# mit-han-lab/pvcnn

Hardware: AMD Instinct MI355X
Metric: point-clouds/sec fwd+bwd, PVCNN S3DIS N=4096 R=32 (higher is better)
Workload: dtype f32 (fp32 tensors, fp32 accumulate; Conv3d fwd / bwd-data / bwd-weight and the large SharedMLP fwd / bwd-data / bwd-weight products as power-of-two scaled fp16 hi+lo splits, 3 partial products on fp16 MFMA, max rel err vs fp64 1e-6 <= the fp32-MFMA kernels'; PVCNN_CONV_MATH=fp32 PVCNN_PW_MATH=fp32 s

## Files before the change

include/pvcnn_hip.h:

```cpp
#ifndef PVCNN_HIP_H_
#define PVCNN_HIP_H_

#include <stddef.h>
#include <stdint.h>

#ifdef __cplusplus
extern "C" {
#endif

#if defined(__GNUC__)
#define PVCNN_API __attribute__((visibility("default")))
#else
#define PVCNN_API
#endif

#define PVCNN_ABI_VERSION 12
#define PVCNN_OK 0
#define PVCNN_ERR_INVALID_ARGUMENT (-1)

PVCNN_API int pvcnn_version(void);
PVCNN_API const char *pvcnn_last_error_string(void);

PVCNN_API int pvcnn_voxel_coords(const float *coords, int B, int N, int R, int normalize, float eps, float *norm_coords,
                       int32_t *vox_coords, void *stream);

PVCNN_API int pvcnn_voxel_coords_tail(const float *coords, long coords_batch_stride, const float *mean, const float *radius,
                            int B, int N, int R, float eps, float *norm_coords, int32_t *vox_coords, void *stream);

PVCNN_API size_t pvcnn_avg_voxelize_fwd_workspace_bytes(int B, int C, int N, int R);
PVCNN_API int pvcnn_avg_voxelize_fwd(const float *feat, const int32_t *coords, int B, int C, int N, int R,
                           float *out, int32_t *ind, int32_t *cnt, void *workspace,
                           size_t workspace_bytes, void *stream);
PVCNN_API int pvcnn_avg_voxelize_bwd(const float *grad_y, const int32_t *ind, const int32_t *cnt, int B,
                           int C, int N, int S, float *grad_x, void *stream);

PVCNN_API int pvcnn_trilinear_devox_fwd(const float *coords, const float *feat, int B, int C, int N, int R,
                              int is_training, int32_t *inds, float *wgts, float *outs,
                              void *stream);
PVCNN_API size_t pvcnn_trilinear_devox_bwd_workspace_bytes(int B, int C, int N, int R);
PVCNN_API int pvcnn_trilinear_devox_bwd(const float *grad_y, const int32_t *inds, const float *wgts, int B,
                              int C, int N, int R, float *grad_x, void *workspace,
                              size_t workspace_bytes, void *stream);

PVCNN_API size_t pvcnn_avg_voxelize_plan_bytes(int B, int N, int R);
PVCNN_API size_t pvcnn_avg_voxelize_plan_scratch_bytes(int B, int N, int R);
PVCNN_API int pvcnn_avg_voxelize_plan(const int32_t *coords, int B, int N, int R, int32_t *ind, int32_t *cnt, void *plan,
                            size_t plan_bytes, void *scratch, size_t scratch_bytes, void *stream);
PVCNN_API size_t pvcnn_pvconv_plans_scratch_bytes(int B, int N, int R);
PVCNN_API int pvcnn_pvconv_plans(const int32_t *vox_coords, const float *norm_coords, int B, int N, int R, int32_t *ind, int32_t *cnt,
                                 void *vox_plan, size_t vox_plan_bytes, void *devox_bwd_plan, size_t devox_bwd_plan_bytes,
                                 void *scratch, size_t scratch_bytes, void *stream);
PVCNN_API int pvcnn_avg_voxelize_apply(const float *feat, const void *plan, size_t plan_bytes, int B, int C, int N, int R,
                             float *out, void *stream);
PVCNN_API size_t pvcnn_trilinear_devox_bwd_plan_bytes(int B, int N, int R);
PVCNN_API size_t pvcnn_trilinear_devox_bwd_plan_scratch_bytes(int B, int N, int R);
PVCNN_API int pvcnn_trilinear_devox_bwd_plan(const int32_t *inds, const float *wgts, int B, int N, int R, void *plan,
                                   size_t plan_bytes, void *scratch, size_t scratch_bytes, void *stream);
PVCNN_API int pvcnn_trilinear_devox_bwd_apply(const float *grad_y, long grad_y_batch_stride, const void *plan, size_t plan_bytes,
                                    int B, int C, int N, int R, float *grad_x, void *stream);

PVCNN_API int pvcnn_ball_query(const float *centers, const float *points, int B, int N, int M, float radius,
                     int U, int32_t *out, void *stream);

PVCNN_API int pvcnn_grouping_fwd(const float *features, const int32_t *indices, int B, int C, int N, int M,
                       int U, float *out, void *stream);
PVCNN_API size_t pvcnn_grouping_bwd_workspace_bytes(int B, int C, int N, int M, int U);
PVCNN_API int pvcnn_grouping_bwd(const float *grad_y, const int32_t *indices, int B, int C, int N, int M,
                       int U, float *grad_x, void *workspace, size_t workspace_bytes, void *stream);
PVCNN_API int pvcnn_gather_fwd(const float *features, const int32_t *indices, int B, int C, int N, int M,
                     float *out, void *stream);
PVCNN_API size_t pvcnn_gather_bwd_workspace_bytes(int B, int C, int N, int M);
PVCNN_API int pvcnn_gather_bwd(const float *grad_y, const int32_t *indices, int B, int C, int N, int M,
                     float *grad_x, void *workspace, size_t workspace_bytes, void *stream);

#define PVCNN_FPS_MAX_RESIDENT_POINTS 16384
PVCNN_API int pvcnn_fps(const float *coords, int B, int N, int M, float *distances, int32_t *indices,
              void *stream);

PVCNN_API int pvcnn_mask_select(const uint8_t *mask, int B, int N, int M, const int32_t *choices, const int64_t *seed,
                      int32_t *selected, int32_t *count, void *stream);

PVCNN_API int pvcnn_three_nn_interp_fwd(const float *points_coords, const float *centers_coords,
                              const float *centers_features, int B, int C, int M, int N,
                              int32_t *indices, float *weights, float *out, void *stream);
PVCNN_API size_t pvcnn_three_nn_interp_bwd_workspace_bytes(int B, int C, int N, int M);
PVCNN_API int pvcnn_three_nn_interp_bwd(const float *grad_y, const int32_t *indices, const float *weights,
                              int B, int C, int N, int M, float *grad_x, void *workspace,
                              size_t workspace_bytes, void *stream);

PVCNN_API int pvcnn_conv3d_weight_transform(const float *w, int Co, int Ci, int for_bwd_data, float *wt,
                                            void *stream);
PVCNN_API int pvcnn_conv3d_fwd(const float *x, const float *wt, const float *bias, int B, int Ci, int Co,
                               int R, float *y, void *stream);
PVCNN_API size_t pvcnn_conv3d_bwd_weight_workspace_bytes(int B, int Ci, int Co, int R);
PVCNN_API int pvcnn_conv3d_bwd_weight(const float *x, const float *grad_y, int B, int Ci, int Co, int R,
                                      float *grad_w, float *grad_bias, void *workspace, size_t workspace_bytes,
                                      void *stream);

PVCNN_API size_t pvcnn_conv3d_weight_split_bytes(int Co, int Ci, int for_bwd_data, int nsplit);
PVCNN_API int pvcnn_conv3d_weight_split(const float *w, int Co, int Ci, int for_bwd_data, int nsplit, void *wts, void *stream);
PVCNN_API int pvcnn_conv3d_weight_split_pair(const float *w, int Co, int Ci, void *wts_fwd, void *wts_bwd, void *stream);
PVCNN_API size_t pvcnn_conv3d_fwd_split_stats_parts(int B, int Co, int R, int nsplit);
PVCNN_API int pvcnn_conv3d_fwd_split_route(int B, int Ci, int Co, int R, int nsplit);
PVCNN_API int pvcnn_absmax_bits(const float *x, size_t n, void *out, void *stream);
PVCNN_API size_t pvcnn_absmax_tiles_count(int B, long L, int seg);
#define PVCNN_TABLE_ONLY ((void *)1)
PVCNN_API int pvcnn_absmax_tiles(const float *x, int B, int C, long L, int seg, void *out, void *ticket, void *stream);
PVCNN_API int pvcnn_conv3d_fwd_split(const float *x, const void *wts, const float *bias, int B, int Ci, int Co, int R, int nsplit,
                           const void *x_absmax, int amax_seg , float *y, float *stats_part, void *stream);

PVCNN_API size_t pvcnn_conv3d_bwd_weight_f16_workspace_bytes(int B, int Ci, int Co, int R);
PVCNN_API int pvcnn_conv3d_bwd_weight_f16(const float *x, const float *grad_y, const void *x_absmax, int x_amax_seg, const void *gy_absmax,
                                int gy_amax_seg, int B, int Ci, int Co, int R, float *grad_w, float *grad_bias, void *workspace,
                                size_t workspace_bytes, void *stream);

PVCNN_API int pvcnn_pwconv_transpose(const float *w, int M, int K, float *wt, void *stream);
PVCNN_API int pvcnn_pwconv_fwd(const float *x, const float *wt, int wt_rows, const float *bias, int B, int K, int M,
                     int N, float *y, void *stream);
PVCNN_API size_t pvcnn_pwconv_bwd_weight_workspace_bytes(int B, int K, int M, int N);
PVCNN_API int pvcnn_pwconv_bwd_weight(const float *x, const float *grad_y, int B, int K, int M, int N,
                            float *grad_w, float *grad_bias, void *workspace, size_t workspace_bytes,
                            void *stream);

PVCNN_API size_t pvcnn_pwconv_weight_split_bytes(int Co, int Ci, int for_bwd_data, int nsplit);
PVCNN_API int pvcnn_pwconv_weight_split(const float *w, int Co, int Ci, int for_bwd_data, int nsplit, void *wts, void *stream);
PVCNN_API int pvcnn_pwconv_weight_split_pair(const float *w, int Co, int Ci, void *wts_fwd, void *wts_bwd, void *stream);
PVCNN_API size_t pvcnn_pwconv_fwd_split_stats_parts(int B, int N);
PVCNN_API int pvcnn_pwconv_fwd_split(const float *x, const void *wts, const float *bias, int B, int K, int M, int N, int nsplit,
                           const void *x_absmax, int amax_seg , float *y, float *stats_part, void *stream);
PVCNN_API size_t pvcnn_pwconv_bwd_weight_f16_workspace_bytes(int B, int K, int M, int N);
PVCNN_API int pvcnn_pwconv_bwd_weight_f16(const float *x, const float *grad_y, const void *x_absmax, int x_amax_seg, const void *gy_absmax,
                                int gy_amax_seg, int B, int K, int M, int N, float *grad_w, float *grad_bias, void *workspace,
                                size_t workspace_bytes, void *stream);

PVCNN_API int pvcnn_dropout_keep_mask(const void *drop_seed, float drop_p, long numel, unsigned char *keep, void *stream);
PVCNN_API size_t pvcnn_bnact_workspace_bytes(int B, int C, int S);
PVCNN_API int pvcnn_bnact_fwd(const float *x, const float *gamma, const float *beta, float *running_mean,
                              float *running_var, int B, int C, int S, float eps, float momentum, float slope,
                              int training, float *mean, float *rstd, float *y, void *y_amax, int amax_seg, int amax_zeroed,
                              void *workspace, size_t workspace_bytes, const void *drop_seed, float drop_p, void *stream);
PVCNN_API size_t pvcnn_conv3d_fwd_stats_parts(int B, int Co, int R);
PVCNN_API int pvcnn_conv3d_fwd_stats(const float *x, const float *wt, const float *bias, int B, int Ci, int Co, int R,
                           float *y, float *stats_part, void *stream);
PVCNN_API size_t pvcnn_pwconv_fwd_stats_parts(int B, int N);
PVCNN_API int pvcnn_pwconv_fwd_stats(const float *x, const float *wt, int wt_rows, const float *bias, int B, int K, int M,
                           int N, float *y, float *stats_part, void *stream);
PVCNN_API int pvcnn_bn_finalize(const float *part, int C, long nparts, double count, float eps, float momentum, const float *shift,
                      float *running_mean, float *running_var, float *mean, float *rstd,
                      void *zero_words , long zero_count ,
                      void *num_batches_tracked , void *stream);
PVCNN_API int pvcnn_bn_stats(const float *x, float *running_mean, float *running_var, int B, int C, int S,
                   float eps, float momentum, float *mean, float *rstd, void *workspace,
                   size_t workspace_bytes, void *stream);
PVCNN_API int pvcnn_trilinear_devox_bnact_fwd(const float *coords, const float *feat, const float *gamma,
                                    const float *beta, const float *mean, const float *rstd, float slope,
                                    int B, int C, int N, int R, int is_training, int32_t *inds, float *wgts,
                                    const float *addend, const float *se_scale, float *outs, void *stream);
PVCNN_API int pvcnn_bnact_bwd(const float *x, const float *grad_y, const float *gamma, const float *beta,
                              const float *mean, const float *rstd, int B, int C, int S, float slope, int training,
                              float *grad_x, float *grad_gamma, float *grad_beta, void *workspace,
                              size_t workspace_bytes, void *stream);
PVCNN_API int pvcnn_bnact_bwd_strided(const float *x, const float *grad_y, long grad_y_batch_stride, const float *gamma,
                            const float *beta, const float *mean, const float *rstd, int B, int C, int S,
                            float slope, int training, float *grad_x, float *grad_gamma, float *grad_beta,
                            void *gx_amax, int amax_seg, void *workspace, size_t workspace_bytes, const void *drop_seed,
                            float drop_p, void *tickets, void *stream);
PVCNN_API int pvcnn_bnact_slices(int S);
PVCNN_API long pvcnn_conv3d_weight_split_pair_entry(const float *w, int Co, int Ci, void *wts_fwd, void *wts_bwd, long long *entry);
PVCNN_API int pvcnn_conv3d_weight_split_pair_batch(const void *table, int n, long total_rows, void *stream);
PVCNN_API long pvcnn_pwconv_weight_split_pair_entry(const float *w, int Co, int Ci, void *wts_fwd, void *wts_bwd, long long *entry);
PVCNN_API int pvcnn_pwconv_weight_split_pair_batch(const void *table, int n, long total_rows, void *stream);
PVCNN_API long pvcnn_conv3d_weight_split_pair_entry_bf16(const float *w, int Co, int Ci, void *wts_fwd, void *wts_bwd, long long *entry);
PVCNN_API int pvcnn_conv3d_weight_split_pair_batch_bf16(const void *table, int n, long total_rows, void *stream);
PVCNN_API long pvcnn_pwconv_weight_split_pair_entry_bf16(const float *w, int Co, int Ci, void *wts_fwd, void *wts_bwd, long long *entry);
PVCNN_API int pvcnn_pwconv_weight_split_pair_batch_bf16(const void *table, int n, long total_rows, void *stream);

PVCNN_API int pvcnn_neighbor_max_supported(int K);
PVCNN_API int pvcnn_neighbor_max_fwd(const float *x, long rows, int K, float *out, unsigned char *winners, void *stream);
PVCNN_API int pvcnn_neighbor_max_bwd(const float *grad_out, const unsigned char *winners, long rows, int K, float *grad_x, void *stream);

PVCNN_API int pvcnn_row_argmax(const float *x, long rows, int K, long long *winners, float *values, void *stream);

PVCNN_API int pvcnn_bnact_apply_rowmax(const float *x, const float *gamma, const float *beta, const float *mean, const float *rstd, int B,
                                       int C, int S, float slope, float *y, long y_batch_stride, void *y_amax, int amax_seg,
                                       void *row_keys, void *stream);
PVCNN_API int pvcnn_row_keys_decode(const void *row_keys, const float *y, long rows, int S, long long *winners, float *values,
                                    int C, long y_batch_stride, void *stream);

PVCNN_API size_t pvcnn_frustum_box_loss_grad_floats(int B, int NH, int NS);
PVCNN_API int pvcnn_frustum_box_loss(const float *center, const float *center_reg, const float *heading_scores, const float *size_scores,
                                     const float *heading_residuals_normalized, const float *size_residuals_normalized,
                                     const float *heading_residuals, const float *size_residuals, const long long *heading_bin_id,
                                     const long long *size_template_id, const float *heading_residual_t, const float *size_residual_t,
                                     const float *center_t, const float *size_templates, const float *heading_bin_centers, int B, int NH,
                                     int NS, float heading_bin_width, float w_heading_residual, float w_size_residual, float w_corners,
                                     float *loss, float *grads, void *stream);

PVCNN_API int pvcnn_se_excite_fwd(const float *part, int slices, const float *gamma, const float *beta, const float *w1, const float *w2,
                        int B, int C, int H, float inv_s, float *a_sum, float *ax_sum, float *squeezed, float *hidden, float *excite,
                        void *stream);
PVCNN_API int pvcnn_se_excite_bwd(const float *part, int slices, const float *a_sum, const float *ax_sum, const float *gamma,
                        const float *beta, const float *squeezed, const float *hidden, const float *excite, const float *w1,
                        const float *w2, int B, int C, int H, float inv_s, float *g_w1, float *g_w2, float *g_mean, float *sum_beta,
                        float *sum_gamma, float *workspace, void *stream);
PVCNN_API int pvcnn_bnact_partial_sums(const float *x, const float *grad_y, long grad_y_batch_stride, const float *gamma, const float *beta,
                             const float *mean, const float *rstd, int B, int C, int S, float slope, float *part, void *stream);
PVCNN_API int pvcnn_bnact_bwd_apply(const float *x, const float *grad_y, long grad_y_batch_stride, const float *gamma, const float *beta,
                          const float *mean, const float *rstd, const float *sum_gamma, const float *sum_beta, const float *bc_mul,
                          const float *bc_add, int B, int C, int S, float slope, int training, float *grad_x, void *gx_amax,
                          int amax_seg, void *stream);
PVCNN_API int pvcnn_trilinear_devox_bwd_strided(const float *grad_y, long grad_y_batch_stride, const int32_t *inds,
                                      const float *wgts, int B, int C, int N, int R, float *grad_x,
                                      void *workspace, size_t workspace_bytes, void *stream);

PVCNN_API int pvcnn_concat_points(const float *const *srcs, const long *bstrides, const int *channels, const int *pstrides,
                        const void *const *src_amax ,
                        int nsrc, int B, int N, float *out, void *out_amax,
                        void *ticket , void *stream);

PVCNN_API int pvcnn_dense_bn_relu_supported(int rows, int Cin, int Cout);
PVCNN_API int pvcnn_dense_bn_relu_fwd(const float *x, const float *weight, const float *bias, const float *gamma, const float *beta,
                                      float *running_mean, float *running_var, void *num_batches_tracked, int rows, int Cin, int Cout,
                                      float eps, float momentum, float *z, float *y, float *mean, float *rstd, void *stream);
PVCNN_API int pvcnn_dense_bn_relu_bwd(const float *x, const float *grad_y, const float *z, const float *mean, const float *rstd,
                                      const float *gamma, const float *beta, int rows, int Cin, int Cout, float *grad_z,
                                      float *grad_weight, float *grad_bias, float *grad_gamma, float *grad_beta, void *stream);

PVCNN_API int pvcnn_adam_step(float *p, const float *g, float *m, float *v, size_t n, float *step, const float *hyper, int inc_step,
                    void *stream);

#ifdef __cplusplus
}
#endif
#endif
```

pvcnn_amd/_lib.py:

```python
import ctypes
import functools
import os

import torch

_CSRC = os.path.join(os.path.dirname(os.path.abspath(__file__)), 'csrc')
LIB_PATH = os.path.join(_CSRC, 'libpvcnn_hip.so')
ABI_VERSION = 12

_vp, _i, _f, _sz, _l = ctypes.c_void_p, ctypes.c_int, ctypes.c_float, ctypes.c_size_t, ctypes.c_long

SIGNATURES = {
    'pvcnn_version': (_i, []),
    'pvcnn_last_error_string': (ctypes.c_char_p, []),
    'pvcnn_voxel_coords': (_i, [_vp, _i, _i, _i, _i, _f, _vp, _vp, _vp]),
    'pvcnn_voxel_coords_tail': (_i, [_vp, ctypes.c_long, _vp, _vp, _i, _i, _i, _f, _vp, _vp, _vp]),
    'pvcnn_avg_voxelize_fwd_workspace_bytes': (_sz, [_i, _i, _i, _i]),
    'pvcnn_avg_voxelize_fwd': (_i, [_vp, _vp, _i, _i, _i, _i, _vp, _vp, _vp, _vp, _sz, _vp]),
    'pvcnn_avg_voxelize_bwd': (_i, [_vp, _vp, _vp, _i, _i, _i, _i, _vp, _vp]),
    'pvcnn_trilinear_devox_fwd': (_i, [_vp, _vp, _i, _i, _i, _i, _i, _vp, _vp, _vp, _vp]),
    'pvcnn_trilinear_devox_bwd_workspace_bytes': (_sz, [_i, _i, _i, _i]),
    'pvcnn_trilinear_devox_bwd': (_i, [_vp, _vp, _vp, _i, _i, _i, _i, _vp, _vp, _sz, _vp]),
    'pvcnn_avg_voxelize_plan_bytes': (_sz, [_i, _i, _i]),
    'pvcnn_avg_voxelize_plan_scratch_bytes': (_sz, [_i, _i, _i]),
    'pvcnn_avg_voxelize_plan': (_i, [_vp, _i, _i, _i, _vp, _vp, _vp, _sz, _vp, _sz, _vp]),
    'pvcnn_avg_voxelize_apply': (_i, [_vp, _vp, _sz, _i, _i, _i, _i, _vp, _vp]),
    'pvcnn_pvconv_plans_scratch_bytes': (_sz, [_i, _i, _i]),
    'pvcnn_pvconv_plans': (_i, [_vp, _vp, _i, _i, _i, _vp, _vp, _vp, _sz, _vp, _sz, _vp, _sz, _vp]),
    'pvcnn_trilinear_devox_bwd_plan_bytes': (_sz, [_i, _i, _i]),
    'pvcnn_trilinear_devox_bwd_plan_scratch_bytes': (_sz, [_i, _i, _i]),
    'pvcnn_trilinear_devox_bwd_plan': (_i, [_vp, _vp, _i, _i, _i, _vp, _sz, _vp, _sz, _vp]),
    'pvcnn_trilinear_devox_bwd_apply': (_i, [_vp, ctypes.c_long, _vp, _sz, _i, _i, _i, _i, _vp, _vp]),
    'pvcnn_ball_query': (_i, [_vp, _vp, _i, _i, _i, _f, _i, _vp, _vp]),
    'pvcnn_grouping_fwd': (_i, [_vp, _vp, _i, _i, _i, _i, _i, _vp, _vp]),
    'pvcnn_grouping_bwd_workspace_bytes': (_sz, [_i, _i, _i, _i, _i]),
    'pvcnn_grouping_bwd': (_i, [_vp, _vp, _i, _i, _i, _i, _i, _vp, _vp, _sz, _vp]),
    'pvcnn_gather_fwd': (_i, [_vp, _vp, _i, _i, _i, _i, _vp, _vp]),
    'pvcnn_gather_bwd_workspace_bytes': (_sz, [_i, _i, _i, _i]),
    'pvcnn_gather_bwd': (_i, [_vp, _vp, _i, _i, _i, _i, _vp, _vp, _sz, _vp]),
    'pvcnn_fps': (_i, [_vp, _i, _i, _i, _vp, _vp, _vp]),
    'pvcnn_mask_select': (_i, [_vp, _i, _i, _i, _vp, _vp, _vp, _vp, _vp]),
    'pvcnn_three_nn_interp_fwd': (_i, [_vp, _vp, _vp, _i, _i, _i, _i, _vp, _vp, _vp, _vp]),
    'pvcnn_three_nn_interp_bwd_workspace_bytes': (_sz, [_i, _i, _i, _i]),
    'pvcnn_three_nn_interp_bwd': (_i, [_vp, _vp, _vp, _i, _i, _i, _i, _vp, _vp, _sz, _vp]),
    'pvcnn_conv3d_weight_transform': (_i, [_vp, _i, _i, _i, _vp, _vp]),
    'pvcnn_conv3d_fwd': (_i, [_vp, _vp, _vp, _i, _i, _i, _i, _vp, _vp]),
    'pvcnn_conv3d_bwd_weight_workspace_bytes': (_sz, [_i, _i, _i, _i]),
    'pvcnn_conv3d_bwd_weight': (_i, [_vp, _vp, _i, _i, _i, _i, _vp, _vp, _vp, _sz, _vp]),
    'pvcnn_conv3d_weight_split_bytes': (_sz, [_i, _i, _i, _i]),
    'pvcnn_conv3d_weight_split': (_i, [_vp, _i, _i, _i, _i, _vp, _vp]),
    'pvcnn_conv3d_weight_split_pair': (_i, [_vp, _i, _i, _vp, _vp, _vp]),
    'pvcnn_conv3d_fwd_split_stats_parts': (_sz, [_i, _i, _i, _i]),
    'pvcnn_conv3d_fwd_split_route': (_i, [_i, _i, _i, _i, _i]),
    'pvcnn_absmax_bits': (_i, [_vp, _sz, _vp, _vp]),
    'pvcnn_absmax_tiles_count': (_sz, [_i, ctypes.c_long, _i]),
    'pvcnn_absmax_tiles': (_i, [_vp, _i, _i, ctypes.c_long, _i, _vp, _vp, _vp]),
    'pvcnn_conv3d_bwd_weight_f16_workspace_bytes': (_sz, [_i, _i, _i, _i]),
    'pvcnn_conv3d_bwd_weight_f16': (_i, [_vp, _vp, _vp, _i, _vp, _i, _i, _i, _i, _i, _vp, _vp, _vp, _sz, _vp]),
    'pvcnn_conv3d_fwd_split': (_i, [_vp, _vp, _vp, _i, _i, _i, _i, _i, _vp, _i, _vp, _vp, _vp]),
    'pvcnn_pwconv_transpose': (_i, [_vp, _i, _i, _vp, _vp]),
    'pvcnn_pwconv_fwd': (_i, [_vp, _vp, _i, _vp, _i, _i, _i, _i, _vp, _vp]),
    'pvcnn_pwconv_weight_split_bytes': (_sz, [_i, _i, _i, _i]),
    'pvcnn_pwconv_weight_split': (_i, [_vp, _i, _i, _i, _i, _vp, _vp]),
    'pvcnn_pwconv_weight_split_pair': (_i, [_vp, _i, _i, _vp, _vp, _vp]),
    'pvcnn_pwconv_fwd_split_stats_parts': (_sz, [_i, _i]),
    'pvcnn_pwconv_fwd_split': (_i, [_vp, _vp, _vp, _i, _i, _i, _i, _i, _vp, _i, _vp, _vp, _vp]),
    'pvcnn_pwconv_bwd_weight_f16_workspace_bytes': (_sz, [_i, _i, _i, _i]),
    'pvcnn_pwconv_bwd_weight_f16': (_i, [_vp, _vp, _vp, _i, _vp, _i, _i, _i, _i, _i, _vp, _vp, _vp, _sz, _vp]),
    'pvcnn_pwconv_bwd_weight_workspace_bytes': (_sz, [_i, _i, _i, _i]),
    'pvcnn_pwconv_bwd_weight': (_i, [_vp, _vp, _i, _i, _i, _i, _vp, _vp, _vp, _sz, _vp]),
    'pvcnn_bnact_workspace_bytes': (_sz, [_i, _i, _i]),
    'pvcnn_bnact_fwd': (_i, [_vp, _vp, _vp, _vp, _vp, _i, _i, _i, _f, _f, _f, _i, _vp, _vp, _vp, _vp, _i, _i, _vp, _sz, _vp, _f, _vp]),
    'pvcnn_dropout_keep_mask': (_i, [_vp, _f, _l, _vp, _vp]),
    'pvcnn_conv3d_fwd_stats_parts': (_sz, [_i, _i, _i]),
    'pvcnn_conv3d_fwd_stats': (_i, [_vp, _vp, _vp, _i, _i, _i, _i, _vp, _vp, _vp]),
    'pvcnn_pwconv_fwd_stats_parts': (_sz, [_i, _i]),
    'pvcnn_pwconv_fwd_stats': (_i, [_vp, _vp, _i, _vp, _i, _i, _i, _i, _vp, _vp, _vp]),
    'pvcnn_bn_finalize': (_i, [_vp, _i, ctypes.c_long, ctypes.c_double, _f, _f, _vp, _vp, _vp, _vp, _vp, _vp, ctypes.c_long, _vp, _vp]),
    'pvcnn_bn_stats': (_i, [_vp, _vp, _vp, _i, _i, _i, _f, _f, _vp, _vp, _vp, _sz, _vp]),
    'pvcnn_trilinear_devox_bnact_fwd': (_i, [_vp, _vp, _vp, _vp, _vp, _vp, _f, _i, _i, _i, _i, _i, _vp, _vp, _vp, _vp, _vp, _vp]),
    'pvcnn_bnact_slices': (_i, [_i]),
    'pvcnn_conv3d_weight_split_pair_entry': (_l, [_vp, _i, _i, _vp, _vp, _vp]),
    'pvcnn_conv3d_weight_split_pair_batch': (_i, [_vp, _i, _l, _vp]),
    'pvcnn_pwconv_weight_split_pair_entry': (_l, [_vp, _i, _i, _vp, _vp, _vp]),
    'pvcnn_pwconv_weight_split_pair_batch': (_i, [_vp, _i, _l, _vp]),
    'pvcnn_conv3d_weight_split_pair_entry_bf16': (_l, [_vp, _i, _i, _vp, _vp, _vp]),
    'pvcnn_conv3d_weight_split_pair_batch_bf16': (_i, [_vp, _i, _l, _vp]),
    'pvcnn_pwconv_weight_split_pair_entry_bf16': (_l, [_vp, _i, _i, _vp, _vp, _vp]),
    'pvcnn_pwconv_weight_split_pair_batch_bf16': (_i, [_vp, _i, _l, _vp]),
    'pvcnn_neighbor_max_supported': (_i, [_i]),
    'pvcnn_neighbor_max_fwd': (_i, [_vp, _l, _i, _vp, _vp, _vp]),
    'pvcnn_neighbor_max_bwd': (_i, [_vp, _vp, _l, _i, _vp, _vp]),
    'pvcnn_row_argmax': (_i, [_vp, _l, _i, _vp, _vp, _vp]),
    'pvcnn_bnact_apply_rowmax': (_i, [_vp, _vp, _vp, _vp, _vp, _i, _i, _i, _f, _vp, _l, _vp, _i, _vp, _vp]),
    'pvcnn_row_keys_decode': (_i, [_vp, _vp, _l, _i, _vp, _vp, _i, _l, _vp]),
    'pvcnn_frustum_box_loss_grad_floats': (_sz, [_i, _i, _i]),
    'pvcnn_frustum_box_loss': (_i, [_vp] * 15 + [_i, _i, _i, _f, _f, _f, _f, _vp, _vp, _vp]),
    'pvcnn_se_excite_fwd': (_i, [_vp, _i, _vp, _vp, _vp, _vp, _i, _i, _i, _f, _vp, _vp, _vp, _vp, _vp, _vp]),
    'pvcnn_se_excite_bwd': (_i, [_vp, _i] + [_vp] * 9 + [_i, _i, _i, _f] + [_vp] * 7),
    'pvcnn_bnact_partial_sums': (_i, [_vp, _vp, ctypes.c_long, _vp, _vp, _vp, _vp, _i, _i, _i, _f, _vp, _vp]),
    'pvcnn_bnact_bwd_apply': (_i, [_vp, _vp, ctypes.c_long, _vp, _vp, _vp, _vp, _vp, _vp, _vp, _vp, _i, _i, _i, _f, _i, _vp, _vp, _i, _vp]),
    'pvcnn_bnact_bwd': (_i, [_vp, _vp, _vp, _vp, _vp, _vp, _i, _i, _i, _f, _i, _vp, _vp, _vp, _vp, _sz, _vp]),
    'pvcnn_bnact_bwd_strided': (_i, [_vp, _vp, ctypes.c_long, _vp, _vp, _vp, _vp, _i, _i, _i, _f, _i, _vp, _vp, _vp, _vp, _i, _vp, _sz, _vp, _f, _vp, _vp]),
    'pvcnn_concat_points': (_i, [_vp, _vp, _vp, _vp, _vp, _i, _i, _i, _vp, _vp, _vp, _vp]),
    'pvcnn_dense_bn_relu_supported': (_i, [_i, _i, _i]),
    'pvcnn_dense_bn_relu_fwd': (_i, [_vp] * 8 + [_i, _i, _i, _f, _f, _vp, _vp, _vp, _vp, _vp]),
    'pvcnn_dense_bn_relu_bwd': (_i, [_vp] * 7 + [_i, _i, _i] + [_vp] * 6),
    'pvcnn_adam_step': (_i, [_vp, _vp, _vp, _vp, _sz, _vp, _vp, _i, _vp]),
    'pvcnn_trilinear_devox_bwd_strided': (_i, [_vp, ctypes.c_long, _vp, _vp, _i, _i, _i, _i, _vp, _vp, _sz, _vp]),
}

_lib = None


class PvcnnHipError(RuntimeError):
    pass


def load():
    global _lib
    if _lib is not None:
        return _lib
    if not os.path.exists(LIB_PATH):
        raise PvcnnHipError(
            f'{LIB_PATH} not found: build it with `python -c "import __graft_entry__ as g; g.build()"` '
            f'or `make -C {_CSRC}`.  There is no CPU fallback for the PVConv hot path.')
    lib = ctypes.CDLL(LIB_PATH)
    for name, (res, args) in SIGNATURES.items():
        fn = getattr(lib, name)
        fn.restype, fn.argtypes = res, args
    got = lib.pvcnn_version()
    if got != ABI_VERSION:
        raise PvcnnHipError(f'libpvcnn_hip.so ABI version {got}, binding expects {ABI_VERSION}: rebuild')
    for name, (res, _args) in SIGNATURES.items():
        if res is _sz:
            setattr(lib, name, functools.lru_cache(maxsize=4096)(getattr(lib, name)))
    _lib = lib
    return lib


def sources_digest():
    import glob
    import hashlib
    h = hashlib.sha1()
    names = sorted(glob.glob(os.path.join(_CSRC, '*.hip')) + glob.glob(os.path.join(_CSRC, '*.h')))
    names.append(os.path.join(os.path.dirname(os.path.dirname(os.path.abspath(__file__))), 'include', 'pvcnn_hip.h'))
    for name in names:
        h.update(os.path.basename(name).encode())
        with open(name, 'rb') as fh:
            h.update(fh.read())
    return h.hexdigest()[:12]


def check(rc, what):
    if rc != 0:
        msg = load().pvcnn_last_error_string().decode('utf-8', 'replace')
        raise PvcnnHipError(f'{what} failed (code {rc}): {msg}')
```

pvcnn_amd/csrc/bnact.hip:

```cpp
#include <algorithm>

#include "common.h"

namespace pvcnn {

constexpr int kBnThreads = 256;
constexpr int kBnSlice = 8192;

__device__ __forceinline__ float wave_sum(float v) {
#pragma unroll
  for (int d = 32; d >= 1; d >>= 1) v += __shfl_xor(v, d);
  return v;
}

__device__ __forceinline__ void block_sum2(float &a, float &b, float *sm) {
  a = wave_sum(a);
  b = wave_sum(b);
  const int wave = threadIdx.x >> 6, lane = threadIdx.x & 63;
  if (lane == 0) { sm[wave] = a; sm[8 + wave] = b; }
  __syncthreads();
  if (threadIdx.x == 0) {
    a = sm[0] + sm[1] + sm[2] + sm[3];
    b = sm[8] + sm[9] + sm[10] + sm[11];
  }
// ... 455 lines not shown
    amax_zeroed = 1;
  }
  if (y_amax != nullptr) {
    const int nseg = ceil_div(S, amax_seg), spb = amax_seg >= 256 ? 1 : 256 / amax_seg;
    const int vec = (S % 4 == 0) && (amax_seg % 4 == 0) && aligned16(x) && aligned16(y);
    uint32_t *am = static_cast<uint32_t *>(y_amax);
    const int groups = amax_zeroed ? pb_channel_groups((long)ceil_div(nseg, spb) * B, C) : 1;
    if (dropping)
      hipLaunchKernelGGL((bnact_apply_pb_kernel<false, true>), dim3(ceil_div(nseg, spb), B, groups), dim3(256), 0, s, x, nullptr, 0L, mean, rstd,
                         gamma, beta, nullptr, nullptr, slope, 0.0f, 0, C, S, amax_seg, nseg, vec, y, am, amax_zeroed ? 1 : 0, nullptr, nullptr,
                         ceil_div(C, groups), groups > 1 ? 1 : 0, drop);
    else
      hipLaunchKernelGGL(bnact_apply_pb_kernel<false>, dim3(ceil_div(nseg, spb), B, groups), dim3(256), 0, s, x, nullptr, 0L, mean, rstd, gamma,
                         beta, nullptr, nullptr, slope, 0.0f, 0, C, S, amax_seg, nseg, vec, y, am, amax_zeroed ? 1 : 0, nullptr, nullptr,
                         ceil_div(C, groups), groups > 1 ? 1 : 0);
    if (int e = check_launch("bnact_apply_pb")) return e;
    return amax_zeroed ? 0 : launch_amax_reduce(am, (long)B * nseg, s);
  }
  hipLaunchKernelGGL(bnact_apply_kernel, grid, dim3(kBnThreads), 0, s, x, mean, rstd, gamma, beta, slope, C, S, y);
  return check_launch("bnact_apply");
}

extern "C" int pvcnn_bnact_apply_rowmax(const float *x, const float *gamma, const float *beta, const float *mean, const float *rstd, int B,
                                        int C, int S, float slope, float *y, long y_batch_stride, void *y_amax, int amax_seg, void *row_keys,
                                        void *stream) {
  PVCNN_REQUIRE(B > 0 && C > 0 && S > 0 && x && y && mean && rstd && y_amax && row_keys, "bad argument");
  PVCNN_REQUIRE(y_batch_stride == 0 || (y_batch_stride >= (long)C * S && y_batch_stride % 4 == 0), "y_batch_stride: 0, or >= C * S and a multiple of 4");
  PVCNN_REQUIRE(B <= 65535 && C <= 65535, "batch or channel count > 65535");
  PVCNN_REQUIRE(amax_seg_in_range(amax_seg), kAmaxSegRange);
  PVCNN_REQUIRE(amax_seg % 4 == 0 && 256 % amax_seg == 0 && S % 256 == 0,
                "the row-maximum pass additionally needs S % 256 == 0 and amax_seg a multiple of 4 that divides 256");
  PVCNN_REQUIRE(aligned16(x) && aligned16(y) && ((uintptr_t)row_keys & 7) == 0, "x / y must be 16-byte aligned, row_keys 8-byte aligned");
  hipStream_t s = static_cast<hipStream_t>(stream);
  const int nseg = ceil_div(S, amax_seg), spb = amax_seg >= 256 ? 1 : 256 / amax_seg;
  const int groups = pb_channel_groups((long)ceil_div(nseg, spb) * B, C);
  hipLaunchKernelGGL((bnact_apply_pb_kernel<false, false, true>), dim3(ceil_div(nseg, spb), B, groups), dim3(256), 0, s, x, nullptr, 0L, mean, rstd,
                     gamma, beta, nullptr, nullptr, slope, 0.0f, 0, C, S, amax_seg, nseg, 1, y, static_cast<uint32_t *>(y_amax), 1, nullptr, nullptr,
                     ceil_div(C, groups), groups > 1 ? 1 : 0, Drop{nullptr, 0u, 1.0f}, static_cast<unsigned long long *>(row_keys), y_batch_stride);
  return check_launch("bnact_apply_rowmax");
}

extern "C" int pvcnn_row_keys_decode(const void *row_keys, const float *y, long rows, int S, long long *winners, float *values, int C,
                                     long y_batch_stride, void *stream) {
  PVCNN_REQUIRE(rows >= 0 && S > 0, "negative size");
  if (rows == 0) return 0;
  PVCNN_REQUIRE(row_keys && y && winners, "null pointer");
  if (C <= 0 || y_batch_stride <= 0) { C = 1; y_batch_stride = S; }
  hipLaunchKernelGGL(row_keys_decode_kernel, dim3((unsigned)((rows + 255) / 256)), dim3(256), 0, static_cast<hipStream_t>(stream),
                     static_cast<const unsigned long long *>(row_keys), y, rows, S, winners, values, C, y_batch_stride);
  return check_launch("row_keys_decode");
}

extern "C" int pvcnn_bn_finalize(const float *part, int C, long nparts, double count, float eps, float momentum, const float *shift,
                                 float *running_mean, float *running_var, float *mean, float *rstd, void *zero_words, long zero_count,
                                 void *num_batches_tracked, void *stream) {
  PVCNN_REQUIRE(C > 0 && nparts > 0 && nparts <= 0x7fffffffL && count > 0 && part && mean && rstd, "bad argument");
  hipLaunchKernelGGL(bn_finalize_kernel, dim3(C), dim3(64), 0, static_cast<hipStream_t>(stream),
                     reinterpret_cast<const float2 *>(part), (int)nparts, count, eps, momentum, shift, mean, rstd, running_mean,
                     running_var, static_cast<uint32_t *>(zero_words), zero_words ? zero_count : 0L,
                     static_cast<long long *>(num_batches_tracked));
  return check_launch("bn_finalize");
}

extern "C" int pvcnn_bn_stats(const float *x, float *running_mean, float *running_var, int B, int C, int S, float eps,
                              float momentum, float *mean, float *rstd, void *workspace, size_t workspace_bytes, void *stream) {
  PVCNN_REQUIRE(B > 0 && C > 0 && S > 0 && x && mean && rstd, "bad argument");
  PVCNN_REQUIRE(B <= 65535 && C <= 65535, "batch or channel count > 65535");
  PVCNN_REQUIRE(workspace && workspace_bytes >= pvcnn_bnact_workspace_bytes(B, C, S), "workspace too small");
  hipStream_t s = static_cast<hipStream_t>(stream);
  const int slices = ceil_div(S, kBnSlice);
  float2 *part = static_cast<float2 *>(workspace);
  float *shift = reinterpret_cast<float *>(part + (size_t)C * B * slices);
  hipLaunchKernelGGL(bn_stats_kernel, dim3(slices, B, C), dim3(kBnThreads), 0, s, x, C, S, slices, part, shift);
  if (int e = check_launch("bn_stats")) return e;
  hipLaunchKernelGGL(bn_finalize_kernel, dim3(C), dim3(64), 0, s, part, B * slices, (double)B * S, eps, momentum, shift, mean, rstd,
                     running_mean, running_var, static_cast<uint32_t *>(nullptr), 0L, static_cast<long long *>(nullptr));
  return check_launch("bn_finalize");
}

static int bnact_bwd_impl(const float *x, const float *grad_y, long gy_bstride, const float *gamma, const float *beta,
                          const float *mean, const float *rstd, int B, int C, int S, float slope, int training, float *grad_x,
                          float *grad_gamma, float *grad_beta, void *workspace, size_t workspace_bytes, void *stream,
                          void *gx_amax = nullptr, int amax_seg = 0, const void *drop_seed = nullptr, float drop_p = 0.0f,
                          void *tickets = nullptr) {
  PVCNN_REQUIRE(drop_p >= 0.0f && drop_p < 1.0f, "drop_p must be in [0, 1)");
  Drop drop{nullptr, 0u, 1.0f};
  const bool dropping = make_drop(drop_seed, drop_p, &drop);
  PVCNN_REQUIRE(!dropping || (gx_amax && (size_t)B * C * S < ((size_t)1 << 33)), "fused dropout needs the amax-emitting pass (gx_amax) and < 2^33 elements");
  PVCNN_REQUIRE(B > 0 && C > 0 && S > 0 && x && grad_y && mean && rstd && grad_x && grad_gamma && grad_beta, "bad argument");
  PVCNN_REQUIRE(B <= 65535 && C <= 65535, "batch or channel count > 65535");
  PVCNN_REQUIRE(gy_bstride >= (long)C * S, "grad_y batch stride smaller than one sample");
  PVCNN_REQUIRE(workspace && workspace_bytes >= pvcnn_bnact_workspace_bytes(B, C, S), "workspace too small");
  PVCNN_REQUIRE(!gx_amax || amax_seg_in_range(amax_seg), kAmaxSegRange);
  hipStream_t s = static_cast<hipStream_t>(stream);
  const int slices = ceil_div(S, kBnSlice);
  const dim3 grid(slices, B, C);
  float2 *part = static_cast<float2 *>(workspace);
  const long zero_count = gx_amax ? 1 + (long)B * ceil_div(S, amax_seg) : 0L;
  PVCNN_REQUIRE(!tickets || (reinterpret_cast<uintptr_t>(tickets) & 3) == 0, "tickets must be 4-byte aligned");
  const BwdFold fold{static_cast<unsigned *>(tickets), grad_gamma, grad_beta, static_cast<uint32_t *>(gx_amax), zero_count};
  if (dropping)
    hipLaunchKernelGGL(bnact_bwd_reduce_kernel<true>, grid, dim3(kBnThreads), 0, s, x, grad_y, mean, rstd, gamma, beta, slope, C, S, slices, part,
                       gy_bstride, drop, fold);
  else
    hipLaunchKernelGGL(bnact_bwd_reduce_kernel<false>, grid, dim3(kBnThreads), 0, s, x, grad_y, mean, rstd, gamma, beta, slope, C, S, slices, part,
                       gy_bstride, Drop{nullptr, 0u, 1.0f}, fold);
  if (int e = check_launch("bnact_bwd_reduce")) return e;
  if (tickets == nullptr) {
    hipLaunchKernelGGL(bnact_bwd_finalize_kernel, dim3(C), dim3(64), 0, s, part, B * slices, grad_gamma, grad_beta,
                       static_cast<uint32_t *>(gx_amax), zero_count);
    if (int e = check_launch("bnact_bwd_finalize")) return e;
  }
  const float inv_count = (float)(1.0 / ((double)B * S));
  if (gx_amax != nullptr) {
    const int nseg = ceil_div(S, amax_seg), spb = amax_seg >= 256 ? 1 : 256 / amax_seg;
    const int vec = (S % 4 == 0) && (amax_seg % 4 == 0) && (gy_bstride % 4 == 0) && aligned16(x) && aligned16(grad_y) && aligned16(grad_x);
    uint32_t *am = static_cast<uint32_t *>(gx_amax);
    const int groups = pb_channel_groups((long)ceil_div(nseg, spb) * B, C);
    if (dropping)
      hipLaunchKernelGGL((bnact_apply_pb_kernel<true, true>), dim3(ceil_div(nseg, spb), B, groups), dim3(256), 0, s, x, grad_y, gy_bstride, mean,
                         rstd, gamma, beta, grad_gamma, grad_beta, slope, inv_count, training, C, S, amax_seg, nseg, vec, grad_x, am, 1, nullptr,
                         nullptr, ceil_div(C, groups), groups > 1 ? 1 : 0, drop);
    else
      hipLaunchKernelGGL(bnact_apply_pb_kernel<true>, dim3(ceil_div(nseg, spb), B, groups), dim3(256), 0, s, x, grad_y, gy_bstride, mean, rstd,
                         gamma, beta, grad_gamma, grad_beta, slope, inv_count, training, C, S, amax_seg, nseg, vec, grad_x, am, 1, nullptr,
                         nullptr, ceil_div(C, groups), groups > 1 ? 1 : 0);
    return check_launch("bnact_bwd_apply_pb");
  }
  hipLaunchKernelGGL(bnact_bwd_apply_kernel, grid, dim3(kBnThreads), 0, s, x, grad_y, mean, rstd, gamma, beta, grad_gamma,
                     grad_beta, slope, inv_count, training, C, S, grad_x, gy_bstride);
  return check_launch("bnact_bwd_apply");
}

extern "C" int pvcnn_bnact_bwd(const float *x, const float *grad_y, const float *gamma, const float *beta, const float *mean,
                               const float *rstd, int B, int C, int S, float slope, int training, float *grad_x,
                               float *grad_gamma, float *grad_beta, void *workspace, size_t workspace_bytes, void *stream) {
  return bnact_bwd_impl(x, grad_y, (long)C * S, gamma, beta, mean, rstd, B, C, S, slope, training, grad_x, grad_gamma, grad_beta,
                        workspace, workspace_bytes, stream);
}

extern "C" int pvcnn_bnact_bwd_strided(const float *x, const float *grad_y, long grad_y_batch_stride, const float *gamma,
                                       const float *beta, const float *mean, const float *rstd, int B, int C, int S, float slope,
                                       int training, float *grad_x, float *grad_gamma, float *grad_beta, void *gx_amax, int amax_seg,
                                       void *workspace, size_t workspace_bytes, const void *drop_seed, float drop_p, void *tickets,
                                       void *stream) {
  return bnact_bwd_impl(x, grad_y, grad_y_batch_stride, gamma, beta, mean, rstd, B, C, S, slope, training, grad_x, grad_gamma,
                        grad_beta, workspace, workspace_bytes, stream, gx_amax, amax_seg, drop_seed, drop_p, tickets);
}

extern "C" int pvcnn_bnact_slices(int S) { return S > 0 ? ceil_div(S, kBnSlice) : 0; }

extern "C" int pvcnn_bnact_partial_sums(const float *x, const float *grad_y, long grad_y_batch_stride, const float *gamma, const float *beta,
                                        const float *mean, const float *rstd, int B, int C, int S, float slope, float *part, void *stream) {
  PVCNN_REQUIRE(B > 0 && C > 0 && S > 0 && x && mean && rstd && part, "bad argument");
  PVCNN_REQUIRE(B <= 65535 && C <= 65535, "batch or channel count > 65535");
  PVCNN_REQUIRE(!grad_y || grad_y_batch_stride >= (long)C * S, "grad_y batch stride smaller than one sample");
  PVCNN_REQUIRE((reinterpret_cast<uintptr_t>(part) & 7) == 0, "part must be 8-byte aligned");
  const int slices = ceil_div(S, kBnSlice);
  hipLaunchKernelGGL(bnact_bwd_reduce_kernel<false>, dim3(slices, B, C), dim3(kBnThreads), 0, static_cast<hipStream_t>(stream), x, grad_y, mean,
                     rstd, gamma, beta, slope, C, S, slices, reinterpret_cast<float2 *>(part), grad_y ? grad_y_batch_stride : (long)C * S);
  return check_launch("bnact_partial_sums");
}

extern "C" int pvcnn_bnact_bwd_apply(const float *x, const float *grad_y, long grad_y_batch_stride, const float *gamma, const float *beta,
                                     const float *mean, const float *rstd, const float *sum_gamma, const float *sum_beta, const float *bc_mul,
                                     const float *bc_add, int B, int C, int S, float slope, int training, float *grad_x, void *gx_amax,
                                     int amax_seg, void *stream) {
  PVCNN_REQUIRE(B > 0 && C > 0 && S > 0 && x && grad_y && mean && rstd && grad_x, "bad argument");
  PVCNN_REQUIRE(!training || (sum_gamma && sum_beta), "training mode needs the two per-channel sums");
  PVCNN_REQUIRE(B <= 65535 && C <= 65535, "batch or channel count > 65535");
  PVCNN_REQUIRE(grad_y_batch_stride >= (long)C * S, "grad_y batch stride smaller than one sample");
  PVCNN_REQUIRE(!gx_amax || amax_seg_in_range(amax_seg), kAmaxSegRange);
  hipStream_t s = static_cast<hipStream_t>(stream);
  PVCNN_REQUIRE(gx_amax, "pvcnn_bnact_bwd_apply needs an amax buffer (pvcnn_absmax_tiles_count words)");
  const int nseg = ceil_div(S, amax_seg), spb = amax_seg >= 256 ? 1 : 256 / amax_seg;
  const int vec = (S % 4 == 0) && (amax_seg % 4 == 0) && (grad_y_batch_stride % 4 == 0) && aligned16(x) && aligned16(grad_y) && aligned16(grad_x);
  uint32_t *am = static_cast<uint32_t *>(gx_amax);
  hipLaunchKernelGGL(bnact_apply_pb_kernel<true>, dim3(ceil_div(nseg, spb), B), dim3(256), 0, s, x, grad_y, grad_y_batch_stride, mean, rstd, gamma,
                     beta, sum_gamma, sum_beta, slope, (float)(1.0 / ((double)B * S)), training, C, S, amax_seg, nseg, vec, grad_x, am, 0, bc_mul,
                     bc_add);
  if (int e = check_launch("bnact_bwd_apply_pb")) return e;
  return launch_amax_reduce(am, (long)B * nseg, s);
}

namespace pvcnn {
constexpr int kCatMaxSrc = 8;
struct CatSources {
  const float *p[kCatMaxSrc];
  long bstride[kCatMaxSrc];
  int c0[kCatMaxSrc + 1];
  int pstride[kCatMaxSrc];
  const uint32_t *pre[kCatMaxSrc];
  int n;
};

__global__ __launch_bounds__(256) void concat_points_kernel(CatSources src, int N, int vec, float *__restrict__ out,
                                                            uint32_t *__restrict__ amax, unsigned *__restrict__ ticket) {
  __shared__ uint32_t wave_max[4];
  const int b = blockIdx.y, p0 = blockIdx.x * 256;
  const int tid = threadIdx.x, wave = __builtin_amdgcn_readfirstlane(tid >> 6), lane = tid & 63, pos = p0 + 4 * lane;
  const int Ctot = src.c0[src.n];
  const int cgroup = ceil_div(Ctot, (int)gridDim.z), gbeg = (int)blockIdx.z * cgroup, gend = min(Ctot, gbeg + cgroup);
  float *ob = out + (size_t)b * Ctot * N;
  uint32_t m = 0;
  using v4f = __attribute__((ext_vector_type(4))) float;
  for (int s = 0; s < src.n; ++s) {
    const int cb = src.c0[s], lo = max(gbeg, cb) - cb, cn = min(gend, src.c0[s + 1]) - cb;
    if (lo >= cn) continue;
    if (src.pre[s] != nullptr) {
      if (tid == 0 && amax != nullptr) m = max(m, src.pre[s][1 + (size_t)b * gridDim.x + blockIdx.x]);
      continue;
    }
    const float *sp = src.p[s] + (size_t)b * src.bstride[s];
    if (src.pstride[s] == 0) {
      for (int c = lo + wave; c < cn; c += 4) {
        const float v = sp[c];
        m = max(m, __float_as_uint(fabsf(v)));
        if (vec && pos < N) { v4f o = {v, v, v, v}; __builtin_nontemporal_store(o, reinterpret_cast<v4f *>(ob + (size_t)(cb + c) * N + pos)); }
        else for (int i = 0; i < 4; ++i) if (pos + i < N) ob[(size_t)(cb + c) * N + pos + i] = v;
      }
    } else if (vec) {
      if (pos < N)
        for (int c0 = lo + wave; c0 < cn; c0 += 32) {
          float4 v[8];
#pragma unroll
          for (int u = 0; u < 8; ++u)
            if (c0 + 4 * u < cn) v[u] = *reinterpret_cast<const float4 *>(sp + (size_t)(c0 + 4 * u) * N + pos);
#pragma unroll
          for (int u = 0; u < 8; ++u)
            if (c0 + 4 * u < cn) {
// ... 74 lines not shown
```

pvcnn_amd/csrc/csr.h:

```cpp
#pragma once
#include <algorithm>

#include "slab.h"

namespace pvcnn {

constexpr int kCsrThreads = 1024;
constexpr int kCsrMaxTargets = 1 << 20;
constexpr int kCsrMaxRange = 14336;

__host__ __device__ __forceinline__ int pad32(int v) { return v + (v >> 5); }
__host__ __device__ __forceinline__ int start_stride(int L) { return (L + 1 + 3) & ~3; }

constexpr int kTileTargets = 4096;
constexpr int kTileThreads = 1024;
__host__ __device__ inline int order_stride(int L) { return ceil_div(L, kTileTargets) * kTileTargets; }

constexpr int kGroupSlack = 256;
__host__ __device__ inline long entw_range_base(int start_t0, int r) { return 2L * start_t0 + (long)r * (kTileTargets / kWave) * kGroupSlack; }
__host__ __device__ inline long entw_stride(int L, long E) { return 2L * E + (long)ceil_div(L, kTileTargets) * (kTileTargets / kWave) * kGroupSlack; }

struct CsrPlan {
  int32_t *start;
  int2 *ent;
// ... 462 lines not shown
  int2 sg[kSlots];
#pragma unroll
  for (int k = 0; k < kSlots; ++k) {
    const int pos = k * kTileThreads + tid;
    sg[k] = l_seg[pos];
    out[pos] = l_lt[pos];
    sout[pos] = sg[k];
    int m = sg[k].y - sg[k].x, sum = m;
#pragma unroll
    for (int d = 32; d >= 1; d >>= 1) { m = max(m, __shfl_xor(m, d)); sum += __shfl_xor(sum, d); }
    if (lane == 0) gsz[pos >> 6] = (m > 0 && 64L * m <= 2L * sum + kGroupSlack) ? 64 * m : 0;
  }
  __syncthreads();
  if (tid < kGroups) {
    const int sz = gsz[tid];
    int inc = sz;
#pragma unroll
    for (int d = 1; d < kWave; d <<= 1) {
      const int up = __shfl_up(inc, d);
      if (lane >= d) inc += up;
    }
    const long base = entw_range_base(st[0], r) + (inc - sz);
    const int ofs = sz > 0 ? (int)base : -1;
    gsz[tid] = ofs;
    gofs[(size_t)b * (order_stride(L) / kWave) + (size_t)r * kGroups + tid] = ofs;
  }
}

static __global__ __launch_bounds__(kTileThreads) void csr_order_kernel(const int32_t *__restrict__ start, const int2 *__restrict__ ent,
                                                                        int L, int E, uint16_t *__restrict__ order,
                                                                        int2 *__restrict__ seg, int32_t *__restrict__ gofs,
                                                                        int2 *__restrict__ entw) {
  csr_order_body(start, ent, L, E, order, seg, gofs, entw, (int)blockIdx.x, (int)blockIdx.y);
}

struct CsrPlanRef {
  const int32_t *start;
  const int2 *ent;
  uint16_t *order;
  int2 *seg;
  int32_t *gofs;
  int2 *entw;
  int E;
};

[[maybe_unused]] static __global__ __launch_bounds__(kTileThreads) void csr_order_pair_kernel(CsrPlanRef a, CsrPlanRef c, int L, int nr) {
  const int r = (int)blockIdx.x;
  const bool f = r < nr;
  csr_order_body(f ? a.start : c.start, f ? a.ent : c.ent, L, f ? a.E : c.E, f ? a.order : c.order, f ? a.seg : c.seg,
                 f ? a.gofs : c.gofs, f ? a.entw : c.entw, f ? r : r - nr, (int)blockIdx.y);
}

static __device__ __forceinline__ void csr_interleave_body(const int2 *__restrict__ ent, const int2 *__restrict__ seg,
                                                           const int32_t *__restrict__ gofs, int L, int E, int2 *__restrict__ entw,
                                                           int blk, int b) {
  const int pos = blk * 256 + threadIdx.x, lane = threadIdx.x & 63;
  const int ofs = gofs[(size_t)b * (order_stride(L) / kWave) + (pos >> 6)];
  if (ofs < 0) return;
  const int2 sg = seg[(size_t)b * order_stride(L) + pos];
  const int2 *en = ent + (size_t)b * E + sg.x;
  int2 *ew = entw + (size_t)b * entw_stride(L, E) + ofs + lane;
  const int n = sg.y - sg.x;
  int i = 0;
  for (; i + 4 <= n; i += 4) {
    const int2 a = en[i], c = en[i + 1], d = en[i + 2], f = en[i + 3];
    ew[(size_t)i * 64] = a; ew[(size_t)(i + 1) * 64] = c; ew[(size_t)(i + 2) * 64] = d; ew[(size_t)(i + 3) * 64] = f;
  }
  for (; i < n; ++i) ew[(size_t)i * 64] = en[i];
}

static __global__ __launch_bounds__(256) void csr_interleave_kernel(const int2 *__restrict__ ent, const int2 *__restrict__ seg,
                                                                    const int32_t *__restrict__ gofs, int L, int E,
                                                                    int2 *__restrict__ entw) {
  csr_interleave_body(ent, seg, gofs, L, E, entw, (int)blockIdx.x, (int)blockIdx.y);
}

[[maybe_unused]] static __global__ __launch_bounds__(256) void csr_interleave_pair_kernel(CsrPlanRef a, CsrPlanRef c, int L, int nblk) {
  const int k = (int)blockIdx.x;
  const bool f = k < nblk;
  csr_interleave_body(f ? a.ent : c.ent, f ? a.seg : c.seg, f ? a.gofs : c.gofs, L, f ? a.E : c.E, f ? a.entw : c.entw, f ? k : k - nblk,
                      (int)blockIdx.y);
}

template <int G>
__global__ __launch_bounds__(kTileThreads) void segsum_tile_kernel(const float *__restrict__ src, const int2 *__restrict__ seg,
                                                                   const int2 *__restrict__ ent, const uint16_t *__restrict__ order,
                                                                   const int32_t *__restrict__ gofs, const int2 *__restrict__ entw,
                                                                   float *__restrict__ dst, int C, int L, int J, int E,
                                                                   long src_bstride, int nsplit, int JP) {
  extern __shared__ __attribute__((aligned(16))) float lds[];
  using vecG = __attribute__((ext_vector_type(G))) float;
  const int b = blockIdx.z, split = blockIdx.y, c0 = blockIdx.x * G, tid = threadIdx.x;
  const int g = min(G, C - c0);
  float *srcI = lds;
  float *tile = lds + (size_t)JP * G;
  const float *rows = src + (size_t)b * src_bstride + (size_t)c0 * J;
  if ((J & 3) == 0 && aligned16(rows) && ((src_bstride & 3) == 0)) {
    for (int j0 = tid * 4; j0 < J; j0 += kTileThreads * 4) {
      float4 v[G];
#pragma unroll
      for (int c = 0; c < G; ++c) v[c] = ld4(rows + (size_t)min(c, g - 1) * J + j0);
#pragma unroll
      for (int u = 0; u < 4; ++u) {
        vecG o;
#pragma unroll
        for (int c = 0; c < G; ++c) o[c] = (u == 0) ? v[c].x : (u == 1) ? v[c].y : (u == 2) ? v[c].z : v[c].w;
        *reinterpret_cast<vecG *>(srcI + (size_t)(j0 + u) * G) = o;
      }
    }
  } else {
    for (int j = tid; j < J; j += kTileThreads) {
      vecG o;
#pragma unroll
      for (int c = 0; c < G; ++c) o[c] = rows[(size_t)min(c, g - 1) * J + j];
      *reinterpret_cast<vecG *>(srcI + (size_t)j * G) = o;
    }
  }
  __syncthreads();
  const int2 *en = ent + (size_t)b * E;
  const int2 *ew = entw + (size_t)b * entw_stride(L, E) + (tid & 63);
  const uint16_t *ord = order + (size_t)b * order_stride(L);
  const int2 *sg = seg + (size_t)b * order_stride(L);
  const int32_t *go = gofs + (size_t)b * (order_stride(L) / kWave);
  const int nr = ceil_div(L, kTileTargets);
  constexpr int kSlots = kTileTargets / kTileThreads;
  int lt[kSlots], gb[kSlots];
  int2 sq[kSlots];
  auto fetch = [&](int r) {
#pragma unroll
    for (int k = 0; k < kSlots; ++k) {
      const int pos = r * kTileTargets + k * kTileThreads + tid;
      lt[k] = ord[pos];
      sq[k] = sg[pos];
      gb[k] = go[pos >> 6];
    }
  };
  if (split < nr) fetch(split);
  for (int r = split; r < nr; r += nsplit) {
    const int t0 = r * kTileTargets, nt = min(kTileTargets, L - t0);
    int clt[kSlots], cgb[kSlots];
    int2 csq[kSlots];
#pragma unroll
    for (int k = 0; k < kSlots; ++k) { clt[k] = lt[k]; csq[k] = sq[k]; cgb[k] = gb[k]; }
    if (r + nsplit < nr) fetch(r + nsplit);
#pragma unroll
    for (int k = 0; k < kSlots; ++k) {
      if (clt[k] == 0xFFFF) continue;
      const int n = csq[k].y - csq[k].x;
      const int2 *ep = cgb[k] >= 0 ? ew + cgb[k] : en + csq[k].x;
      const int estep = cgb[k] >= 0 ? 64 : 1;
      vecG acc;
#pragma unroll
      for (int c = 0; c < G; ++c) acc[c] = 0.0f;
      int i = 0;
      for (; i + 8 <= n; i += 8) {
        int2 t[8];
        vecG x[8];
#pragma unroll
        for (int u = 0; u < 8; ++u) t[u] = ep[(size_t)(i + u) * estep];
#pragma unroll
        for (int u = 0; u < 8; ++u) x[u] = *reinterpret_cast<const vecG *>(srcI + (size_t)t[u].x * G);
#pragma unroll
        for (int u = 0; u < 8; ++u) {
          const float w = __int_as_float(t[u].y);
#pragma unroll
          for (int c = 0; c < G; ++c) acc[c] = acc[c] + w * x[u][c];
        }
      }
#define PVCNN_TAIL(U)                                                                              \
      if ((n - i) & U) {                                                                           \
        int2 t[U];                                                                                 \
        vecG x[U];                                                                                 \
        _Pragma("unroll") for (int u = 0; u < U; ++u) t[u] = ep[(size_t)(i + u) * estep];          \
        _Pragma("unroll") for (int u = 0; u < U; ++u) x[u] = *reinterpret_cast<const vecG *>(srcI + (size_t)t[u].x * G); \
        _Pragma("unroll") for (int u = 0; u < U; ++u) {                                            \
          const float w = __int_as_float(t[u].y);                                                  \
          _Pragma("unroll") for (int c = 0; c < G; ++c) acc[c] = acc[c] + w * x[u][c];             \
        }                                                                                          \
        i += U;                                                                                    \
      }
      PVCNN_TAIL(4)
      PVCNN_TAIL(2)
      PVCNN_TAIL(1)
#undef PVCNN_TAIL
#pragma unroll
      for (int c = 0; c < G; ++c) tile[c * kTileTargets + clt[k]] = acc[c];
    }
    lds_barrier();
    float *out = dst + ((size_t)b * C + c0) * L + t0;
    if ((L & 3) == 0 && aligned16(dst)) {
      const int q_per_row = nt >> 2;
      for (int q = tid; q < g * q_per_row; q += kTileThreads) {
        const int c = q / q_per_row, i = (q - c * q_per_row) * 4;
        const float4 v = *reinterpret_cast<const float4 *>(tile + c * kTileTargets + i);
        using v4f = __attribute__((ext_vector_type(4))) float;
        v4f o = {v.x, v.y, v.z, v.w};
        __builtin_nontemporal_store(o, reinterpret_cast<v4f *>(out + (size_t)c * L + i));
      }
    } else {
      for (int q = tid; q < g * nt; q += kTileThreads) {
        const int c = q / nt, i = q - c * nt;
        out[(size_t)c * L + i] = tile[c * kTileTargets + i];
      }
    }
    lds_barrier();
  }
}

inline bool csr_supported(int L, long E) { return L <= kCsrMaxTargets && E <= 0x7fffffffL / 8; }

template <int G, bool STAGE>
int launch_segsum_g(const float *src, const CsrPlan &ws, float *dst, int B, int C, int L, int J, int E,
                    bool vec, int threads, hipStream_t s, const char *what, long src_bstride) {
  const size_t lds = STAGE ? (size_t)G * J * sizeof(float) : 0;
  const dim3 grid(ceil_div(C, G), B);
#define PVCNN_SEGSUM(VEC, T)                                                                          \
  do {                                                                                                \
    auto k = segsum_kernel<G, VEC, T, STAGE>;                                                         \
    if (int e = enable_big_lds(k, lds)) { set_error("%s: LDS attribute: %d", what, e); return e; }    \
    hipLaunchKernelGGL(k, grid, dim3(T), lds, s, src, ws.start, ws.ent, dst, C, L, J, E, src_bstride); \
  } while (0)
  if (threads == 1024) { if (vec) PVCNN_SEGSUM(4, 1024); else PVCNN_SEGSUM(1, 1024); }
  else                 { if (vec) PVCNN_SEGSUM(4, 256);  else PVCNN_SEGSUM(1, 256); }
#undef PVCNN_SEGSUM
  return check_launch(what);
}

template <class EP>
int launch_csr_prep(const EP &ep, int B, int L, long E_, int32_t *cnt_out, void *plan, size_t plan_bytes, void *scratch,
                    size_t scratch_bytes, hipStream_t s, const char *what) {
  const int E = (int)E_;
  if (B == 0) return 0;
  if (!plan || plan_bytes < CsrPlan::bytes(B, L, E) || !aligned16(plan) || !scratch || !aligned16(scratch) ||
      scratch_bytes < csr_prep_scratch_bytes(B, E)) {
    set_error("%s: plan / scratch missing, misaligned or too small (%zu + %zu bytes needed)", what, CsrPlan::bytes(B, L, E),
              csr_prep_scratch_bytes(B, E));
    return PVCNN_ERR_INVALID_ARGUMENT;
  }
  CsrPlan pl;
  pl.carve(plan, B, L, E);
  const CsrSplit sp = csr_split(B, L, E);
  const size_t prep_lds = ((size_t)kCsrCoarse * 2 + 4 + 32 + 4 + 3 * kCsrList + sp.HP) * sizeof(int);
  auto k = csr_prep_kernel<EP>;
  if (int e = enable_big_lds(k, prep_lds)) { set_error("%s: LDS attribute: %d", what, e); return e; }
  hipLaunchKernelGGL(k, dim3(sp.P, B), dim3(kCsrThreads), prep_lds, s, ep, E, L, sp, cnt_out, pl.start,
                     static_cast<int32_t *>(scratch), pl.ent);
  if (int e = check_launch(what)) return e;
  hipLaunchKernelGGL(csr_order_kernel, dim3(ceil_div(L, kTileTargets), B), dim3(kTileThreads), 0, s, pl.start, pl.ent, L, E, pl.order, pl.seg,
                     pl.gofs, pl.entw);
  if (int e = check_launch(what)) return e;
  hipLaunchKernelGGL(csr_interleave_kernel, dim3(order_stride(L) / 256, B), dim3(256), 0, s, pl.ent, pl.seg, pl.gofs, L, E, pl.entw);
  return check_launch(what);
}

template <class EP1, class EP2>
int launch_csr_prep_pair(const EP1 &ep1, long E1_, int32_t *cnt1, void *plan1, size_t plan1_bytes, const EP2 &ep2, long E2_, void *plan2,
                         size_t plan2_bytes, int B, int L, void *scratch, size_t scratch_bytes, hipStream_t s, const char *what) {
  const int E1 = (int)E1_, E2 = (int)E2_;
  if (B == 0) return 0;
  const size_t s1 = csr_prep_scratch_bytes(B, E1), s2 = csr_prep_scratch_bytes(B, E2);
  if (!plan1 || !plan2 || plan1_bytes < CsrPlan::bytes(B, L, E1) || plan2_bytes < CsrPlan::bytes(B, L, E2) || !aligned16(plan1) ||
      !aligned16(plan2) || !scratch || !aligned16(scratch) || scratch_bytes < s1 + s2) {
    set_error("%s: plans / scratch missing, misaligned or too small (%zu, %zu, %zu bytes needed)", what, CsrPlan::bytes(B, L, E1),
              CsrPlan::bytes(B, L, E2), s1 + s2);
    return PVCNN_ERR_INVALID_ARGUMENT;
  }
  CsrPlan p1, p2;
  p1.carve(plan1, B, L, E1);
  p2.carve(plan2, B, L, E2);
  const int total = std::max(2, std::min(16, kNumCU / std::max(B, 1)));
  const int cap1 = std::max(1, total / 4);
  const CsrSplit sp1 = csr_split(B, L, E1, cap1), sp2 = csr_split(B, L, E2, std::max(1, total - cap1));
  const size_t prep_lds = ((size_t)kCsrCoarse * 2 + 4 + 32 + 4 + 3 * kCsrList + std::max(sp1.HP, sp2.HP)) * sizeof(int);
  auto k = csr_prep_pair_kernel<EP1, EP2>;
  if (int e = enable_big_lds(k, prep_lds)) { set_error("%s: LDS attribute: %d", what, e); return e; }
  char *sc = static_cast<char *>(scratch);
  hipLaunchKernelGGL(k, dim3(sp1.P + sp2.P, B), dim3(kCsrThreads), prep_lds, s, ep1, E1, sp1, cnt1, p1.start, reinterpret_cast<int32_t *>(sc),
                     p1.ent, ep2, E2, sp2, p2.start, reinterpret_cast<int32_t *>(sc + s1), p2.ent, L);
  if (int e = check_launch(what)) return e;
  const CsrPlanRef r1{p1.start, p1.ent, p1.order, p1.seg, p1.gofs, p1.entw, E1}, r2{p2.start, p2.ent, p2.order, p2.seg, p2.gofs, p2.entw, E2};
  const int nr = ceil_div(L, kTileTargets), nblk = order_stride(L) / 256;
  hipLaunchKernelGGL(csr_order_pair_kernel, dim3(2 * nr, B), dim3(kTileThreads), 0, s, r1, r2, L, nr);
  if (int e = check_launch(what)) return e;
  hipLaunchKernelGGL(csr_interleave_pair_kernel, dim3(2 * nblk, B), dim3(256), 0, s, r1, r2, L, nblk);
  return check_launch(what);
}

inline int launch_csr_apply(const float *src, const void *plan, size_t plan_bytes, float *dst, int B, int C, int L, int J, long E_,
                            hipStream_t s, const char *what, long src_bstride = 0) {
  if (src_bstride <= 0) src_bstride = (long)C * J;
  const int E = (int)E_;
  if (B == 0 || C == 0) return 0;
  if (!plan || plan_bytes < CsrPlan::bytes(B, L, E) || !aligned16(plan)) {
    set_error("%s: plan missing, misaligned or too small (%zu bytes needed)", what, CsrPlan::bytes(B, L, E));
    return PVCNN_ERR_INVALID_ARGUMENT;
  }
  CsrPlan pl;
  pl.carve(const_cast<void *>(plan), B, L, E);
  const int JP = (J + 3) & ~3;
  int G = 0;
  for (int cand = 4; cand >= 1; cand >>= 1)
    if ((size_t)cand * (JP + kTileTargets) * sizeof(float) <= (size_t)kLdsBytesPerCU) { G = cand; break; }
  const size_t row = (size_t)J * sizeof(float);
  int GS = 1;
  if (row > 0 && row <= 64 * 1024) {
    GS = (int)std::min<size_t>(8, (64 * 1024) / row);
    while (GS > 1 && (long)B * ceil_div(C, GS) < 2L * kNumCU) GS >>= 1;
    if (GS >= 8) GS = 8; else if (GS >= 4) GS = 4; else if (GS >= 2) GS = 2; else GS = 1;
  }
  const bool very_sparse = (long)E * 4 <= (long)L && row > 0 && row <= (size_t)kLdsBytesPerCU && (long)B * ceil_div(C, GS) >= kNumCU;
  if (G > 0 && J > 0 && !very_sparse) {
    while (G > 1 && G / 2 >= C) G >>= 1;
    const int nr = ceil_div(L, kTileTargets), slabs = ceil_div(C, G);
    int nsplit = 1;
    while (nsplit < nr && (long)B * slabs * nsplit < kNumCU) nsplit <<= 1;
    nsplit = std::min(nsplit, nr);
    const size_t lds = (size_t)G * (JP + kTileTargets) * sizeof(float);
    const dim3 grid(slabs, nsplit, B);
#define PVCNN_TILE(GV)                                                                                                   \
  do {                                                                                                                   \
    auto k = segsum_tile_kernel<GV>;                                                                                     \
    if (int e = enable_big_lds(k, lds)) { set_error("%s: LDS attribute: %d", what, e); return e; }                       \
    hipLaunchKernelGGL(k, grid, dim3(kTileThreads), lds, s, src, pl.seg, pl.ent, pl.order, pl.gofs, pl.entw, dst, C, L, J, E,  \
                       src_bstride, nsplit, JP);                                                                                      \
  } while (0)
    if (G == 4) PVCNN_TILE(4); else if (G == 2) PVCNN_TILE(2); else PVCNN_TILE(1);
#undef PVCNN_TILE
    return check_launch(what);
  }
  const bool stage = row > 0 && row <= (size_t)kLdsBytesPerCU;
  const bool vec = (L % 4 == 0) && aligned16(dst);
  const int threads = (L >= 8192 || (size_t)GS * row > 48 * 1024) ? 1024 : 256;
  if (!stage) return launch_segsum_g<1, false>(src, pl, dst, B, C, L, J, E, vec, threads, s, what, src_bstride);
  switch (GS) {
    case 8: return launch_segsum_g<8, true>(src, pl, dst, B, C, L, J, E, vec, threads, s, what, src_bstride);
    case 4: return launch_segsum_g<4, true>(src, pl, dst, B, C, L, J, E, vec, threads, s, what, src_bstride);
    case 2: return launch_segsum_g<2, true>(src, pl, dst, B, C, L, J, E, vec, threads, s, what, src_bstride);
    default: return launch_segsum_g<1, true>(src, pl, dst, B, C, L, J, E, vec, threads, s, what, src_bstride);
  }
}

template <class EP>
int launch_csr_scatter(const EP &ep, const float *src, float *dst, int B, int C, int L, int J, long E,
                       int32_t *cnt_out, void *workspace, size_t workspace_bytes, hipStream_t s, const char *what,
                       long src_bstride = 0) {
  if (B == 0) return 0;
  const size_t pb = CsrPlan::bytes(B, L, E);
  if (!workspace || workspace_bytes < pb + csr_prep_scratch_bytes(B, E) || !aligned16(workspace)) {
    set_error("%s: workspace missing, misaligned or too small (%zu bytes needed)", what, pb + csr_prep_scratch_bytes(B, E));
    return PVCNN_ERR_INVALID_ARGUMENT;
  }
  char *w = static_cast<char *>(workspace);
  if (int e = launch_csr_prep(ep, B, L, E, cnt_out, w, pb, w + pb, workspace_bytes - pb, s, what)) return e;
  return launch_csr_apply(src, w, pb, dst, B, C, L, J, E, s, what, src_bstride);
}

}
```

pvcnn_amd/csrc/devoxelize.hip:

```cpp
#include "csr.h"

using namespace pvcnn;

__global__ __launch_bounds__(256) void trilinear_taps_only_kernel(TrilinearFromCoords p, int N) {
  const int b = blockIdx.y, j = blockIdx.x * 256 + threadIdx.x;
  if (j >= N) return;
  Taps<8> t;
  p.load1(b, j, t);
  p.post1(b, j, t);
}

extern "C" int pvcnn_trilinear_devox_fwd(const float *coords, const float *feat, int B, int C, int N, int R,
                                         int is_training, int32_t *inds, float *wgts, float *outs,
                                         void *stream) {
  PVCNN_REQUIRE(B >= 0 && C >= 0 && N >= 0 && R > 0, "negative size");
  PVCNN_REQUIRE((long)R * R * R <= 0x7fffffffL / 4, "resolution too large");
  if (B == 0 || N == 0) return 0;
  PVCNN_REQUIRE(coords && (outs || C == 0) && (feat || C == 0), "null pointer");
  PVCNN_REQUIRE(!is_training || (inds && wgts), "training mode needs inds and wgts");
  PVCNN_REQUIRE(B <= 65535, "batch > 65535");
  hipStream_t s = static_cast<hipStream_t>(stream);
  TrilinearFromCoords p{coords, is_training ? inds : nullptr, is_training ? wgts : nullptr, N, R, R * R};
  bool vec = (N % 4 == 0) && aligned16(coords) && aligned16(outs);
  if (is_training) vec = vec && aligned16(inds) && aligned16(wgts);
  if (C == 0) {
    if (!is_training) return 0;
    hipLaunchKernelGGL(trilinear_taps_only_kernel, dim3(ceil_div(N, 256), B), dim3(256), 0, s, p, N);
    return check_launch("trilinear_taps_only");
  }
  return launch_gather(p, feat, outs, B, C, R * R * R, N, vec, s, "trilinear_devox_fwd", XfNone{}, grid_pad_shift(R));
}

extern "C" int pvcnn_trilinear_devox_bnact_fwd(const float *coords, const float *feat, const float *gamma,
                                               const float *beta, const float *mean, const float *rstd, float slope, int B,
                                               int C, int N, int R, int is_training, int32_t *inds, float *wgts,
                                               const float *addend, const float *se_scale, float *outs, void *stream) {
  PVCNN_REQUIRE(B >= 0 && C > 0 && N >= 0 && R > 0, "bad size");
  PVCNN_REQUIRE((long)R * R * R * sizeof(float) <= (size_t)kLdsBytesPerCU, "grid row does not fit LDS: use bnact_fwd + trilinear_devox_fwd");
  if (B == 0 || N == 0) return 0;
  PVCNN_REQUIRE(coords && outs && feat && mean && rstd, "null pointer");
  PVCNN_REQUIRE(!is_training || (inds && wgts), "training mode needs inds and wgts");
  PVCNN_REQUIRE(B <= 65535, "batch > 65535");
  hipStream_t s = static_cast<hipStream_t>(stream);
  TrilinearFromCoords p{coords, is_training ? inds : nullptr, is_training ? wgts : nullptr, N, R, R * R};
  bool vec = (N % 4 == 0) && aligned16(coords) && aligned16(outs) && (!addend || aligned16(addend));
  if (is_training) vec = vec && aligned16(inds) && aligned16(wgts);
  const XfBnAct xf{gamma, beta, mean, rstd, slope, se_scale};
  return launch_gather(p, feat, outs, B, C, R * R * R, N, vec, s, "trilinear_devox_bnact_fwd", xf, grid_pad_shift(R), addend);
}

extern "C" size_t pvcnn_trilinear_devox_bwd_workspace_bytes(int B, int C, int N, int R) {
  if (B <= 0 || C < 0 || N < 0 || R <= 0) return 0;
  const long S = (long)R * R * R;
  if (S > 0x7fffffffL || !csr_supported((int)S, 8L * N)) return 16;
  return CsrWorkspace::bytes(B, C, (int)S, N, 8L * N);
}

static int devox_bwd_impl(const float *grad_y, long gy_bstride, const int32_t *inds, const float *wgts, int B, int C, int N,
                          int R, float *grad_x, void *workspace, size_t workspace_bytes, void *stream) {
  PVCNN_REQUIRE(B >= 0 && C >= 0 && N >= 0 && R > 0, "negative size");
  PVCNN_REQUIRE((long)R * R * R <= 0x7fffffffL / 4, "resolution too large");
  if (B == 0 || C == 0) return 0;
  PVCNN_REQUIRE(grad_x && (N == 0 || (grad_y && inds && wgts)), "null pointer");
  PVCNN_REQUIRE(B <= 65535, "batch > 65535");
  PVCNN_REQUIRE(gy_bstride >= (long)C * N, "grad_y batch stride smaller than one cloud");
  const int S = R * R * R;
  hipStream_t s = static_cast<hipStream_t>(stream);
  if (!csr_supported(S, 8L * N)) {
    PVCNN_REQUIRE(gy_bstride == (long)C * N, "the atomic fallback needs a contiguous grad_y");
    SavedTaps<8> p{inds, wgts, N};
    return launch_scatter_direct(p, grad_y, grad_x, B, C, S, N, s, "trilinear_devox_bwd(atomic)");
  }
  TapEntries<8> ep{inds, wgts, N, S};
  return launch_csr_scatter(ep, grad_y, grad_x, B, C, S, N, 8L * N, nullptr, workspace,
                            workspace_bytes, s, "trilinear_devox_bwd", gy_bstride);
}

extern "C" int pvcnn_trilinear_devox_bwd(const float *grad_y, const int32_t *inds, const float *wgts, int B,
                                         int C, int N, int R, float *grad_x, void *workspace,
                                         size_t workspace_bytes, void *stream) {
  return devox_bwd_impl(grad_y, (long)C * N, inds, wgts, B, C, N, R, grad_x, workspace, workspace_bytes, stream);
}

extern "C" int pvcnn_trilinear_devox_bwd_strided(const float *grad_y, long grad_y_batch_stride, const int32_t *inds,
                                                 const float *wgts, int B, int C, int N, int R, float *grad_x,
                                                 void *workspace, size_t workspace_bytes, void *stream) {
  return devox_bwd_impl(grad_y, grad_y_batch_stride, inds, wgts, B, C, N, R, grad_x, workspace, workspace_bytes, stream);
}

extern "C" size_t pvcnn_trilinear_devox_bwd_plan_bytes(int B, int N, int R) {
  if (B <= 0 || N < 0 || R <= 0) return 0;
  const long S = (long)R * R * R;
  if (S > 0x7fffffffL / 4 || !csr_supported((int)S, 8L * N)) return 0;
  return CsrPlan::bytes(B, (int)S, 8L * N);
}

extern "C" size_t pvcnn_trilinear_devox_bwd_plan_scratch_bytes(int B, int N, int R) {
  if (B <= 0 || N < 0 || R <= 0) return 0;
  return csr_prep_scratch_bytes(B, 8L * N);
}

extern "C" int pvcnn_trilinear_devox_bwd_plan(const int32_t *inds, const float *wgts, int B, int N, int R, void *plan,
                                              size_t plan_bytes, void *scratch, size_t scratch_bytes, void *stream) {
  PVCNN_REQUIRE(B >= 0 && N >= 0 && R > 0, "negative size");
  PVCNN_REQUIRE((long)R * R * R <= 0x7fffffffL / 4, "resolution too large");
  if (B == 0) return 0;
  const int S = R * R * R;
  PVCNN_REQUIRE(csr_supported(S, 8L * N), "grid too large for a plan: use pvcnn_trilinear_devox_bwd");
  PVCNN_REQUIRE(N == 0 || (inds && wgts), "null pointer");
  PVCNN_REQUIRE(B <= 65535, "batch > 65535");
  TapEntries<8> ep{inds, wgts, N, S};
  return launch_csr_prep(ep, B, S, 8L * N, nullptr, plan, plan_bytes, scratch, scratch_bytes,
                         static_cast<hipStream_t>(stream), "trilinear_devox_bwd_plan");
}

extern "C" int pvcnn_trilinear_devox_bwd_apply(const float *grad_y, long grad_y_batch_stride, const void *plan, size_t plan_bytes,
                                               int B, int C, int N, int R, float *grad_x, void *stream) {
  PVCNN_REQUIRE(B >= 0 && C >= 0 && N >= 0 && R > 0, "negative size");
  PVCNN_REQUIRE((long)R * R * R <= 0x7fffffffL / 4, "resolution too large");
  if (B == 0 || C == 0) return 0;
  PVCNN_REQUIRE(grad_x && (N == 0 || grad_y), "null pointer");
  PVCNN_REQUIRE(B <= 65535, "batch > 65535");
  PVCNN_REQUIRE(grad_y_batch_stride >= (long)C * N, "grad_y batch stride smaller than one cloud");
  const int S = R * R * R;
  return launch_csr_apply(grad_y, plan, plan_bytes, grad_x, B, C, S, N, 8L * N, static_cast<hipStream_t>(stream),
                          "trilinear_devox_bwd_apply", grad_y_batch_stride);
}
```

pvcnn_amd/csrc/slab.h:

```cpp
#pragma once
#include <algorithm>
#include <stdlib.h>

#include "common.h"

namespace pvcnn {

template <int NC>
struct Taps {
  int32_t idx[NC];
  float w[NC];
};

__device__ __forceinline__ float4 ld4(const float *p) { return *reinterpret_cast<const float4 *>(p); }
__device__ __forceinline__ int4 ld4(const int32_t *p) { return *reinterpret_cast<const int4 *>(p); }
__device__ __forceinline__ void st4(float *p, float a, float b, float c, float d) {
  *reinterpret_cast<float4 *>(p) = make_float4(a, b, c, d);
}
__device__ __forceinline__ void st4(int32_t *p, int a, int b, int c, int d) {
  *reinterpret_cast<int4 *>(p) = make_int4(a, b, c, d);
}

template <int NC, bool MAY_SKIP, bool PAD = false>
__device__ __forceinline__ float combine(const Taps<NC> &t, const float *row, int pshift = 0) {
// ... 139 lines not shown
  __device__ __forceinline__ void post4(int, int, const Taps<1> (&)[4]) const {}
};

struct VoxelMean {
  static constexpr int NC = 1;
  static constexpr bool kMaySkip = true;
  static constexpr bool kGridRows = false;
  const int32_t *ind;
  const int32_t *cnt;
  int N, S;
  __device__ __forceinline__ void one(int b, int pos, Taps<1> &t) const {
    const int c = cnt[(size_t)b * S + pos];
    t.idx[0] = (c > 0) ? pos : -1;
    t.w[0] = (c > 0) ? (float)(1.0 / (double)(float)c) : 0.0f;
  }
  __device__ __forceinline__ void load1(int b, int j, Taps<1> &t) const { one(b, ind[(size_t)b * N + j], t); }
  __device__ __forceinline__ void load4(int b, int j0, Taps<1> (&t)[4]) const {
    const int4 p = ld4(ind + (size_t)b * N + j0);
    one(b, p.x, t[0]); one(b, p.y, t[1]); one(b, p.z, t[2]); one(b, p.w, t[3]);
  }
  using Packed = Taps<NC>;
  __device__ __forceinline__ void pack1(int b, int j, Packed &pk) const { load1(b, j, pk); }
  __device__ __forceinline__ void pack4(int b, int j0, Packed (&pk)[4]) const { load4(b, j0, pk); }
  __device__ __forceinline__ void unpack(const Packed &pk, Taps<NC> &t) const { t = pk; }
  __device__ __forceinline__ void post1(int, int, const Taps<1> &) const {}
  __device__ __forceinline__ void post4(int, int, const Taps<1> (&)[4]) const {}
};

template <int THREADS>
__device__ __forceinline__ void slab_copy(float *dst, const float *src, int total) {
  if (((reinterpret_cast<uintptr_t>(src) | reinterpret_cast<uintptr_t>(dst)) & 15) == 0 && (total & 3) == 0) {
    constexpr int kB = 8;
    const int nq = total >> 2;
    const float4 *s4 = reinterpret_cast<const float4 *>(src);
    float4 *d4 = reinterpret_cast<float4 *>(dst);
    for (int q0 = threadIdx.x; q0 < nq; q0 += THREADS * kB) {
      float4 v[kB];
#pragma unroll
      for (int u = 0; u < kB; ++u) v[u] = s4[min(q0 + u * THREADS, nq - 1)];
#pragma unroll
      for (int u = 0; u < kB; ++u)
        if (q0 + u * THREADS < nq) d4[q0 + u * THREADS] = v[u];
    }
  } else {
    for (int i = threadIdx.x; i < total; i += THREADS) dst[i] = src[i];
  }
}

struct XfNone {
  static constexpr bool kIdentity = true;
  static constexpr int kRaw = 1;
  __device__ __forceinline__ XfNone at(int) const { return *this; }
};
struct XfBnAct {
  static constexpr bool kIdentity = false;
  static constexpr int kRaw = 5;
  const float *gamma, *beta, *mean, *rstd;
  float slope;
  const float *se = nullptr;
  __device__ __forceinline__ XfBnAct at(int b_times_C) const {
    XfBnAct x = *this;
    if (x.se) x.se += b_times_C;
    return x;
  }
  __device__ __forceinline__ void params(int c, float &scale, float &shift) const {
    scale = (gamma ? gamma[c] : 1.0f) * rstd[c];
    shift = (beta ? beta[c] : 0.0f) - mean[c] * scale;
  }
  __device__ __forceinline__ float mul(int c) const { return se ? se[c] : 1.0f; }
  __device__ __forceinline__ float apply(float v, float scale, float shift, float m = 1.0f) const {
    v = fmaf(v, scale, shift);
    v = v > 0.f ? v : v * slope;
    return se ? v * m : v;
  }
  __device__ __forceinline__ void fetch(int c, float (&raw)[5]) const {
    raw[0] = gamma ? gamma[c] : 1.0f; raw[1] = rstd[c]; raw[2] = beta ? beta[c] : 0.0f; raw[3] = mean[c]; raw[4] = mul(c);
  }
  __device__ __forceinline__ void combine(const float (&raw)[5], float &scale, float &shift) const {
    scale = raw[0] * raw[1];
    shift = raw[2] - raw[3] * scale;
  }
};

template <int THREADS, class XF>
__device__ __forceinline__ void slab_copy_row_xf(float *dst, const float *src, int len, const XF &xf, int c) {
  float scale, shift;
  xf.params(c, scale, shift);
  const float m = xf.mul(c);
  if (((reinterpret_cast<uintptr_t>(src) | reinterpret_cast<uintptr_t>(dst)) & 15) == 0 && (len & 3) == 0) {
    constexpr int kB = 8;
    const int nq = len >> 2;
    const float4 *s4 = reinterpret_cast<const float4 *>(src);
    float4 *d4 = reinterpret_cast<float4 *>(dst);
    for (int q0 = threadIdx.x; q0 < nq; q0 += THREADS * kB) {
      float4 v[kB];
#pragma unroll
      for (int u = 0; u < kB; ++u) v[u] = s4[min(q0 + u * THREADS, nq - 1)];
#pragma unroll
      for (int u = 0; u < kB; ++u)
        if (q0 + u * THREADS < nq)
          d4[q0 + u * THREADS] = make_float4(xf.apply(v[u].x, scale, shift, m), xf.apply(v[u].y, scale, shift, m),
                                             xf.apply(v[u].z, scale, shift, m), xf.apply(v[u].w, scale, shift, m));
    }
  } else {
    for (int i = threadIdx.x; i < len; i += THREADS) dst[i] = xf.apply(src[i], scale, shift, m);
  }
}

template <int THREADS, class XF>
__device__ __forceinline__ void slab_copy_row_padded(float *dst, const float *src, int len, int pshift, const XF &xf, int c) {
  float scale = 1.0f, shift = 0.0f;
  [[maybe_unused]] float m = 1.0f;
  if constexpr (!XF::kIdentity) { xf.params(c, scale, shift); m = xf.mul(c); }
  auto f = [&](float v) {
    if constexpr (XF::kIdentity) return v; else return xf.apply(v, scale, shift, m);
  };
  if ((reinterpret_cast<uintptr_t>(src) & 15) == 0 && (len & 3) == 0) {
    constexpr int kB = 8;
    const int nq = len >> 2;
    const float4 *s4 = reinterpret_cast<const float4 *>(src);
    for (int q0 = threadIdx.x; q0 < nq; q0 += THREADS * kB) {
      float4 v[kB];
#pragma unroll
      for (int u = 0; u < kB; ++u) v[u] = s4[min(q0 + u * THREADS, nq - 1)];
#pragma unroll
      for (int u = 0; u < kB; ++u)
        if (q0 + u * THREADS < nq) {
          const int i = (q0 + u * THREADS) * 4;
          float *d = dst + i + (i >> pshift);
          d[0] = f(v[u].x); d[1] = f(v[u].y); d[2] = f(v[u].z); d[3] = f(v[u].w);
        }
    }
  } else {
    for (int i = threadIdx.x; i < len; i += THREADS) dst[i + (i >> pshift)] = f(src[i]);
  }
}

template <int THREADS, bool PAD, class XF>
__device__ __forceinline__ void slab_stage(float *lds, const float *src, int g, int L, int Lp, int pshift, const XF &xf, int c0) {
  if constexpr (PAD) {
    for (int c = 0; c < g; ++c) slab_copy_row_padded<THREADS>(lds + c * Lp, src + (size_t)c * L, L, pshift, xf, c0 + c);
  } else if constexpr (XF::kIdentity) {
    slab_copy<THREADS>(lds, src, g * L);
  } else {
    for (int c = 0; c < g; ++c) slab_copy_row_xf<THREADS>(lds + c * L, src + (size_t)c * L, L, xf, c0 + c);
  }
}

template <class P, int VEC, int THREADS, bool RESIDENT, class XF, bool PAD>
__global__ __launch_bounds__(THREADS) void gather_lds_kernel(P p, XF xf, const float *__restrict__ src,
                                                             float *__restrict__ dst, int C, int L,
                                                             int J, int G, int SEQ, int pshift,
                                                             const float *__restrict__ addend = nullptr) {
  extern __shared__ __attribute__((aligned(16))) float lds[];
  constexpr int NC = P::NC;
  const int b = blockIdx.y;
  const XF xfb = xf.at(b * C);
  const bool side = (blockIdx.x == 0);
  constexpr bool resident = RESIDENT;
  const int jf = threadIdx.x * VEC;
  typename P::Packed pk[VEC];
  if (resident && jf < J) {
    if constexpr (VEC == 4) p.pack4(b, jf, pk); else p.pack1(b, jf, pk[0]);
    if (side) {
      Taps<NC> t[VEC];
#pragma unroll
      for (int v = 0; v < VEC; ++v) p.unpack(pk[v], t[v]);
      if constexpr (VEC == 4) p.post4(b, jf, t); else p.post1(b, jf, t[0]);
    }
  }
  for (int sq = 0; sq < SEQ; ++sq) {
    const int c0 = (blockIdx.x * SEQ + sq) * G;
    if (c0 >= C) break;
    const int g = min(G, C - c0);
    if (sq > 0) lds_barrier();
    const int Lp = PAD ? L + (L >> pshift) : L;
    slab_stage<THREADS, PAD>(lds, src + ((size_t)b * C + c0) * L, g, L, Lp, pshift, xfb, c0);
    __syncthreads();
    float *out = dst + ((size_t)b * C + c0) * J;
    const float *add = addend ? addend + ((size_t)b * C + c0) * J : nullptr;
    for (int j0 = jf; j0 < J; j0 += THREADS * VEC) {
      Taps<NC> t[VEC];
      if constexpr (resident) {
#pragma unroll
        for (int v = 0; v < VEC; ++v) p.unpack(pk[v], t[v]);
      } else if constexpr (VEC == 4) {
        p.load4(b, j0, t);
        if (side && sq == 0) p.post4(b, j0, t);
      } else {
        p.load1(b, j0, t[0]);
        if (side && sq == 0) p.post1(b, j0, t[0]);
      }
      for (int c = 0; c < g; ++c) {
        const float *row = lds + c * Lp;
        if constexpr (VEC == 4) {
          const float r0 = combine<NC, P::kMaySkip, PAD>(t[0], row, pshift), r1 = combine<NC, P::kMaySkip, PAD>(t[1], row, pshift);
          float r2 = combine<NC, P::kMaySkip, PAD>(t[2], row, pshift), r3 = combine<NC, P::kMaySkip, PAD>(t[3], row, pshift);
          float q0 = r0, q1 = r1;
          if (add) { const float4 a = ld4(add + (size_t)c * J + j0); q0 = q0 + a.x; q1 = q1 + a.y; r2 = r2 + a.z; r3 = r3 + a.w; }
          st4(out + (size_t)c * J + j0, q0, q1, r2, r3);
        } else {
          float r = combine<NC, P::kMaySkip, PAD>(t[0], row, pshift);
          if (add) r = r + add[(size_t)c * J + j0];
          out[(size_t)c * J + j0] = r;
        }
      }
    }
  }
}

template <class P, class XF>
__global__ __launch_bounds__(1024) void gather_lds_pipe_kernel(P p, XF xf, const float *__restrict__ src, float *__restrict__ dst,
                                                               int C, int L, int J, int SEQ, int pshift,
                                                               const float *__restrict__ addend = nullptr) {
  extern __shared__ __attribute__((aligned(16))) float lds[];
  constexpr int NC = P::NC, THREADS = 1024, kB = 8;
  const int b = blockIdx.y;
  const XF xfb = xf.at(b * C);
  const int jf = threadIdx.x * 4;
  const bool has = jf < J;
  const int nq = L >> 2;
  float4 v[kB];
  typedef unsigned int u32x4 __attribute__((ext_vector_type(4)));
  const int voff = (int)threadIdx.x * 16;
  auto row_descriptor = [&](const float *base, size_t off, int bytes) {
    const uintptr_t rowp = reinterpret_cast<uintptr_t>(base + off);
    const uint32_t lo = __builtin_amdgcn_readfirstlane((uint32_t)rowp), hi = __builtin_amdgcn_readfirstlane((uint32_t)(rowp >> 32));
    return __builtin_amdgcn_make_buffer_rsrc(reinterpret_cast<void *>(((uintptr_t)hi << 32) | lo),  0,
                                              __builtin_amdgcn_readfirstlane(bytes), 0x00020000);
  };
  auto load = [&](const __amdgpu_buffer_rsrc_t &rsrc, int u) {
    const u32x4 raw = __builtin_amdgcn_raw_buffer_load_b128(rsrc, voff, u * THREADS * 16, 0);
    v[u] = make_float4(__uint_as_float(raw.x), __uint_as_float(raw.y), __uint_as_float(raw.z), __uint_as_float(raw.w));
  };
  const int first = blockIdx.x * SEQ;
  [[maybe_unused]] float raw[XF::kRaw];
  auto commit = [&](bool refill, int cnext) {
    float scale = 1.0f, shift = 0.0f;
    [[maybe_unused]] float m = 1.0f;
    if constexpr (!XF::kIdentity) { xfb.combine(raw, scale, shift); m = raw[XF::kRaw - 1]; }
    auto f = [&](float x) {
      if constexpr (XF::kIdentity) return x; else return xfb.apply(x, scale, shift, m);
    };
    const int cn = refill ? cnext : first;
    const __amdgpu_buffer_rsrc_t next = row_descriptor(src, ((size_t)b * C + cn) * L, refill ? L * 4 : 0);
    if constexpr (!XF::kIdentity) xfb.fetch(cn, raw);
#pragma unroll
    for (int u = 0; u < kB; ++u) {
      const int q = (int)threadIdx.x + u * THREADS;
      if (q < nq) {
        const int i = q * 4;
        float *d = lds + i + (i >> pshift);
        d[0] = f(v[u].x); d[1] = f(v[u].y); d[2] = f(v[u].z); d[3] = f(v[u].w);
      }
      load(next, u);
      __builtin_amdgcn_sched_barrier(0);
    }
  };
  {
    const bool any = first < C;
    if constexpr (!XF::kIdentity) xfb.fetch(any ? first : 0, raw);
    const __amdgpu_buffer_rsrc_t rsrc = row_descriptor(src, ((size_t)b * C + (any ? first : 0)) * L, any ? L * 4 : 0);
#pragma unroll
    for (int u = 0; u < kB; ++u) load(rsrc, u);
  }
  typename P::Packed pk[4] = {};
  if (has) p.pack4(b, jf, pk);
  for (int sq = 0; sq < SEQ; ++sq) {
    const int c = first + sq;
    if (c >= C) break;
    const size_t rowoff = ((size_t)b * C + c) * J;
    const __amdgpu_buffer_rsrc_t arsrc = row_descriptor(addend ? addend : dst, rowoff, addend ? J * 4 : 0);
    const u32x4 add = __builtin_amdgcn_raw_buffer_load_b128(arsrc, voff, 0, 0);
    __builtin_amdgcn_sched_barrier(0);
    if (sq > 0) lds_barrier();
    commit(sq + 1 < SEQ && c + 1 < C, c + 1);
    lds_barrier();
    float r[4];
#pragma unroll
    for (int h = 0; h < 4; ++h) {
      if constexpr (sizeof(typename P::Packed) == 16) {
        uint4 &raw4 = reinterpret_cast<uint4 &>(pk[h]);
        asm volatile("" : "+v"(raw4.x), "+v"(raw4.y), "+v"(raw4.z), "+v"(raw4.w));
      }
      Taps<NC> t;
      p.unpack(pk[h], t);
      r[h] = combine<NC, P::kMaySkip, true>(t, lds, pshift);
    }
    if (addend) {
      r[0] = r[0] + __uint_as_float(add.x); r[1] = r[1] + __uint_as_float(add.y);
      r[2] = r[2] + __uint_as_float(add.z); r[3] = r[3] + __uint_as_float(add.w);
    }
    const __amdgpu_buffer_rsrc_t drsrc = row_descriptor(dst, rowoff, J * 4);
    u32x4 o;
    o.x = __float_as_uint(r[0]); o.y = __float_as_uint(r[1]); o.z = __float_as_uint(r[2]); o.w = __float_as_uint(r[3]);
    __builtin_amdgcn_raw_buffer_store_b128(o, drsrc, voff, 0, 0);
  }
  if (has && blockIdx.x == 0) {
    Taps<NC> t[4];
#pragma unroll
    for (int v = 0; v < 4; ++v) p.unpack(pk[v], t[v]);
    p.post4(b, jf, t);
  }
}

template <class P, class XF, int G>
__global__ __launch_bounds__(1024) void gather_lds_pipe_rows_kernel(P p, XF xf, const float *__restrict__ src, float *__restrict__ dst,
                                                                int C, int L, int J, int SEQ, int pshift,
                                                                const float *__restrict__ addend = nullptr) {
  extern __shared__ __attribute__((aligned(16))) float lds[];
  constexpr int NC = P::NC, THREADS = 1024;
  const int b = blockIdx.y;
  const XF xfb = xf.at(b * C);
  const int jf = threadIdx.x * 4;
  const bool has = jf < J;
  const int Lp = L + (L >> pshift);
  typedef unsigned int u32x4 __attribute__((ext_vector_type(4)));
  const int voff = (int)threadIdx.x * 16;
  float4 v[G];
  auto issue_sized = [&](int c0, int bytes) {
    const uintptr_t rowp = reinterpret_cast<uintptr_t>(src + ((size_t)b * C + c0) * L);
    const uint32_t lo = __builtin_amdgcn_readfirstlane((uint32_t)rowp), hi = __builtin_amdgcn_readfirstlane((uint32_t)(rowp >> 32));
    const __amdgpu_buffer_rsrc_t rsrc = __builtin_amdgcn_make_buffer_rsrc(
        reinterpret_cast<void *>(((uintptr_t)hi << 32) | lo),  0,  __builtin_amdgcn_readfirstlane(bytes), 0x00020000);
#pragma unroll
    for (int u = 0; u < G; ++u) {
      const u32x4 raw = __builtin_amdgcn_raw_buffer_load_b128(rsrc, voff, u * THREADS * 16, 0);
      v[u] = make_float4(__uint_as_float(raw.x), __uint_as_float(raw.y), __uint_as_float(raw.z), __uint_as_float(raw.w));
    }
  };
  auto issue = [&](int c0) { issue_sized(c0, min(G, C - c0) * L * 4); };
  auto issue_none = [&]() { issue_sized(0, 0); };
  [[maybe_unused]] float raw[G][XF::kRaw];
#pragma unroll
  for (int u = 0; u < G; ++u)
#pragma unroll
    for (int i = 0; i < XF::kRaw; ++i) raw[u][i] = (i < 2 || i == 4) ? 1.0f : 0.0f;
  auto fetch = [&](int c0) {
    if constexpr (!XF::kIdentity) {
#pragma unroll
      for (int u = 0; u < G; ++u)
        if (c0 + u < C) xfb.fetch(c0 + u, raw[u]);
    }
  };
  auto commit = [&]() {
    const int i = (int)threadIdx.x * 4;
#pragma unroll
    for (int u = 0; u < G; ++u) {
      float scale = 1.0f, shift = 0.0f;
      if constexpr (!XF::kIdentity) xfb.combine(raw[u], scale, shift);
      auto f = [&](float x) {
        if constexpr (XF::kIdentity) return x; else return xfb.apply(x, scale, shift, raw[u][XF::kRaw - 1]);
      };
      float *d = lds + u * Lp + i + (i >> pshift);
      d[0] = f(v[u].x); d[1] = f(v[u].y); d[2] = f(v[u].z); d[3] = f(v[u].w);
    }
  };
  const int first = blockIdx.x * SEQ * G;
  auto row_descriptor = [&](const float *base, size_t off, int bytes) {
    const uintptr_t rowp = reinterpret_cast<uintptr_t>(base + off);
    const uint32_t lo = __builtin_amdgcn_readfirstlane((uint32_t)rowp), hi = __builtin_amdgcn_readfirstlane((uint32_t)(rowp >> 32));
    return __builtin_amdgcn_make_buffer_rsrc(reinterpret_cast<void *>(((uintptr_t)hi << 32) | lo), 0, __builtin_amdgcn_readfirstlane(bytes), 0x00020000);
  };
  {
    fetch(min(first, max(C - 1, 0)));
    if (first < C) issue(first); else issue_none();
  }
  typename P::Packed pk[4] = {};
  if (has) p.pack4(b, jf, pk);
  for (int sq = 0; sq < SEQ; ++sq) {
    const int c0 = first + sq * G;
    if (c0 >= C) break;
    const int rows = min(G, C - c0);
    const size_t rowoff = ((size_t)b * C + c0) * J;
    const __amdgpu_buffer_rsrc_t arsrc = row_descriptor(addend ? addend : dst, rowoff, addend ? rows * J * 4 : 0);
    u32x4 add[G];
#pragma unroll
    for (int u = 0; u < G; ++u) add[u] = __builtin_amdgcn_raw_buffer_load_b128(arsrc, voff, u * J * 4, 0);
    __builtin_amdgcn_sched_barrier(0);
    if (sq > 0) lds_barrier();
    commit();
    lds_barrier();
    {
      const bool more = sq + 1 < SEQ && c0 + G < C;
      fetch(more ? c0 + G : c0);
      if (more) issue(c0 + G); else issue_none();
    }
    __builtin_amdgcn_sched_barrier(0);
    float r[G][4];
#pragma unroll
    for (int h = 0; h < 4; ++h) {
      if constexpr (sizeof(typename P::Packed) == 16) {
        uint4 &rw = reinterpret_cast<uint4 &>(pk[h]);
        asm volatile("" : "+v"(rw.x), "+v"(rw.y), "+v"(rw.z), "+v"(rw.w));
      }
      Taps<NC> t;
      p.unpack(pk[h], t);
#pragma unroll
      for (int u = 0; u < G; ++u) r[u][h] = combine<NC, P::kMaySkip, true>(t, lds + u * Lp, pshift);
    }
    const __amdgpu_buffer_rsrc_t drsrc = row_descriptor(dst, rowoff, rows * J * 4);
#pragma unroll
    for (int u = 0; u < G; ++u) {
      if (addend) {
        r[u][0] = r[u][0] + __uint_as_float(add[u].x); r[u][1] = r[u][1] + __uint_as_float(add[u].y);
        r[u][2] = r[u][2] + __uint_as_float(add[u].z); r[u][3] = r[u][3] + __uint_as_float(add[u].w);
      }
      u32x4 o;
      o.x = __float_as_uint(r[u][0]); o.y = __float_as_uint(r[u][1]); o.z = __float_as_uint(r[u][2]); o.w = __float_as_uint(r[u][3]);
      __builtin_amdgcn_raw_buffer_store_b128(o, drsrc, has ? voff : 0x7ffffff0, u * J * 4, 0);
    }
  }
  if (has && blockIdx.x == 0) {
    Taps<NC> t[4];
#pragma unroll
    for (int h = 0; h < 4; ++h) p.unpack(pk[h], t[h]);
    p.post4(b, jf, t);
  }
}

template <class P>
__global__ __launch_bounds__(256) void gather_direct_kernel(P p, const float *__restrict__ src,
                                                            float *__restrict__ dst, int C, int L,
                                                            int J, int CT) {
  constexpr int NC = P::NC;
  const int b = blockIdx.z;
  const int j = blockIdx.x * 256 + threadIdx.x;
  if (j >= J) return;
  Taps<NC> t;
  p.load1(b, j, t);
  if (blockIdx.y == 0) p.post1(b, j, t);
  const int c0 = blockIdx.y * CT, c1 = min(C, c0 + CT);
  for (int c = c0; c < c1; ++c)
    dst[((size_t)b * C + c) * J + j] = combine<NC, P::kMaySkip>(t, src + ((size_t)b * C + c) * L);
}

template <class P>
__global__ __launch_bounds__(256) void scatter_direct_kernel(P p, const float *__restrict__ src,
                                                             float *__restrict__ dst, int C, int L,
                                                             int J, int CT) {
  constexpr int NC = P::NC;
  const int b = blockIdx.z;
  const int j = blockIdx.x * 256 + threadIdx.x;
  if (j >= J) return;
  Taps<NC> t;
  p.load1(b, j, t);
  const int c0 = blockIdx.y * CT, c1 = min(C, c0 + CT);
  for (int c = c0; c < c1; ++c) {
    const float gv = src[((size_t)b * C + c) * J + j];
    float *row = dst + ((size_t)b * C + c) * L;
#pragma unroll
    for (int k = 0; k < NC; ++k) atomicAdd(row + t.idx[k], t.w[k] * gv);
  }
}

struct SlabPlan {
  bool lds;
  int G;
  int seq;
  int threads;
  size_t bytes;
};

inline SlabPlan plan_slab(int B, int C, int L, int pshift = 0) {
  SlabPlan pl{};
  const size_t row = (size_t)(pshift ? L + (L >> pshift) : L) * sizeof(float);
  pl.lds = row <= (size_t)kLdsBytesPerCU;
  if (!pl.lds) return pl;
  int G = 1;
  if (row <= 64 * 1024) {
    G = (int)((64 * 1024) / row);
    if (G > C) G = C;
    while (G > 1 && (long)B * ceil_div(C, G) < 3L * kNumCU) G = (G + 1) / 2;
  }
  pl.G = G;
  pl.bytes = (size_t)G * row;
  pl.threads = (pl.bytes > 48 * 1024) ? 1024 : 256;
  const long resident_wgs = (long)kNumCU * std::max<long>(1, (long)(kLdsBytesPerCU / pl.bytes));
  const long slabs = (long)B * ceil_div(C, G);
  pl.seq = (int)std::min<long>(8, std::max<long>(1, slabs / resident_wgs));
  return pl;
}

template <class K>
inline int enable_big_lds(K kernel, size_t bytes) {
  if (bytes > 64 * 1024)
    return (int)hipFuncSetAttribute(reinterpret_cast<const void *>(kernel),
                                    hipFuncAttributeMaxDynamicSharedMemorySize, (int)bytes);
  return 0;
}

template <class P, class XF = XfNone>
int launch_gather(const P &p, const float *src, float *dst, int B, int C, int L, int J, bool vec_ok,
                  hipStream_t s, const char *what, const XF &xf = XF{}, int pshift = 0, const float *addend = nullptr) {
  if (B == 0 || C == 0 || J == 0) return 0;
  if (pshift > 0 && (size_t)(L + (L >> pshift)) * sizeof(float) > (size_t)kLdsBytesPerCU) pshift = 0;
  SlabPlan pl = plan_slab(B, C, L, pshift);
  if constexpr (P::kGridRows) {
    static const bool pipe4 = [] { const char *e = getenv("PVCNN_GATHER_PIPE"); return !(e && e[0] == '0'); }();
    if (pipe4 && pl.lds && pshift > 0 && vec_ok && J <= 1024 * 4 && J > 1024 && (L >> 2) == 1024 && aligned16(src) && C >= 4) {
      constexpr int GR = 2;
      const int slabs = ceil_div(C, GR);
      const int seq = (int)std::min<long>(8, std::max<long>(1, (long)B * slabs / kNumCU));
      const size_t bytes = (size_t)GR * (L + (L >> pshift)) * sizeof(float);
      auto k = gather_lds_pipe_rows_kernel<P, XF, GR>;
      if (int e = enable_big_lds(k, bytes)) { set_error("%s: LDS attribute: %d", what, e); return e; }
      hipLaunchKernelGGL(k, dim3(ceil_div(slabs, seq), B), dim3(1024), bytes, s, p, xf, src, dst, C, L, J, seq, pshift, addend);
      return check_launch(what);
    }
  }
  if (!pl.lds) {
    if (!XF::kIdentity || addend) {
      set_error("%s: row does not fit LDS; the fused transform / addend needs the LDS path", what);
      return PVCNN_ERR_INVALID_ARGUMENT;
    } else if constexpr (XF::kIdentity) {
      const int CT = 16;
      hipLaunchKernelGGL((gather_direct_kernel<P>), dim3(ceil_div(J, 256), ceil_div(C, CT), B), dim3(256), 0, s,
                         p, src, dst, C, L, J, CT);
      return check_launch(what);
    }
  }
  const dim3 grid(ceil_div(ceil_div(C, pl.G), pl.seq), B);
  if constexpr (P::kGridRows) {
    static const bool pipe = [] { const char *e = getenv("PVCNN_GATHER_PIPE"); return !(e && e[0] == '0'); }();
    if (pipe && pl.threads == 1024 && pl.G == 1 && pshift > 0 && vec_ok && J <= 1024 * 4 && (L & 3) == 0 && (L >> 2) <= 1024 * 8 &&
        aligned16(src) && (((size_t)L * sizeof(float)) & 15) == 0) {
      auto k = gather_lds_pipe_kernel<P, XF>;
      if (int e = enable_big_lds(k, pl.bytes)) { set_error("%s: LDS attribute: %d", what, e); return e; }
      hipLaunchKernelGGL(k, grid, dim3(1024), pl.bytes, s, p, xf, src, dst, C, L, J, pl.seq, pshift, addend);
      return check_launch(what);
    }
  }
#define PVCNN_LAUNCH_GATHER_P(VEC, T, PADV)                                                      \
  do {                                                                                           \
    auto k = (J <= T * VEC) ? gather_lds_kernel<P, VEC, T, true, XF, PADV> : gather_lds_kernel<P, VEC, T, false, XF, PADV>; \
    if (int e = enable_big_lds(k, pl.bytes)) { set_error("%s: LDS attribute: %d", what, e); return e; } \
    hipLaunchKernelGGL(k, grid, dim3(T), pl.bytes, s, p, xf, src, dst, C, L, J, pl.G, pl.seq, pshift, addend); \
  } while (0)
#define PVCNN_LAUNCH_GATHER(VEC, T)                                                              \
  do {                                                                                           \
    if constexpr (P::kGridRows) { if (pshift > 0) PVCNN_LAUNCH_GATHER_P(VEC, T, true); else PVCNN_LAUNCH_GATHER_P(VEC, T, false); } \
    else PVCNN_LAUNCH_GATHER_P(VEC, T, false);                                                   \
  } while (0)
  if (pl.threads == 1024) { if (vec_ok) PVCNN_LAUNCH_GATHER(4, 1024); else PVCNN_LAUNCH_GATHER(1, 1024); }
  else                    { if (vec_ok) PVCNN_LAUNCH_GATHER(4, 256);  else PVCNN_LAUNCH_GATHER(1, 256); }
#undef PVCNN_LAUNCH_GATHER
#undef PVCNN_LAUNCH_GATHER_P
  return check_launch(what);
}

template <class P>
int launch_scatter_direct(const P &p, const float *src, float *dst, int B, int C, int L, int J, hipStream_t s,
                          const char *what) {
  if (B == 0 || C == 0 || L == 0) return 0;
  hipError_t e = hipMemsetAsync(dst, 0, (size_t)B * C * L * sizeof(float), s);
  if (e != hipSuccess) { set_error("%s: memset: %s", what, hipGetErrorString(e)); return (int)e; }
  if (J == 0) return 0;
  const int CT = 16;
  hipLaunchKernelGGL((scatter_direct_kernel<P>), dim3(ceil_div(J, 256), ceil_div(C, CT), B), dim3(256), 0, s,
                     p, src, dst, C, L, J, CT);
  return check_launch(what);
}

}
```

pvcnn_amd/modules/functional/backend.py:

```python
import ctypes
import os

import torch

from ... import _lib
from . import _cache

__all__ = ['_backend']


def _dev(t, name):
    if not t.is_cuda:
        raise RuntimeError(f'{name} must be a CUDA (HIP) tensor -- the PVConv hot path has no CPU implementation')


def _f32(t, name):
    _dev(t, name)
    if not t.is_contiguous():
        raise RuntimeError(f'{name} must be a contiguous tensor')
    if t.dtype != torch.float32:
        raise RuntimeError(f'{name} must be a float tensor')


def _f32_rows(t, name):
# ... 323 lines not shown
        b, c, s3 = grad_y.shape
        n = indices.shape[1]
        grad_x = torch.empty((b, c, n), dtype=torch.float32, device=grad_y.device)
        with _Launch(grad_y) as s:
            _lib.check(self.lib.pvcnn_avg_voxelize_bwd(_p(grad_y), _p(indices), _p(cnt), b, c, n, s3, _p(grad_x), s),
                       'avg_voxelize_backward')
        return grad_x


    has_scatter_plans = True

    class VoxelPlan:
        __slots__ = ('ind', 'cnt', 'plan', 'r', 'n', 'b')

    def avg_voxelize_plan(self, coords, resolution):
        _i32(coords, 'coords')
        _shape(coords.dim() == 3 and coords.shape[1] == 3, 'avg_voxelize: coords (B,3,N) expected')
        b, _, n = coords.shape
        r = int(resolution)
        nbytes = self.lib.pvcnn_avg_voxelize_plan_bytes(b, n, r)
        if nbytes == 0:
            return None
        dev = coords.device
        vp = self.VoxelPlan()
        vp.r, vp.n, vp.b = r, n, b
        vp.ind = torch.empty((b, n), dtype=torch.int32, device=dev)
        vp.cnt = torch.empty((b, r * r * r), dtype=torch.int32, device=dev)
        vp.plan = torch.empty((nbytes,), dtype=torch.uint8, device=dev)
        scratch = self._scratch(self.lib.pvcnn_avg_voxelize_plan_scratch_bytes(b, n, r), dev)
        with _Launch(coords) as s:
            _lib.check(self.lib.pvcnn_avg_voxelize_plan(_p(coords), b, n, r, _p(vp.ind), _p(vp.cnt), _p(vp.plan), vp.plan.numel(),
                                                        _p(scratch), scratch.numel(), s), 'avg_voxelize_plan')
        return vp

    has_pvconv_plans = os.environ.get('PVCNN_PAIR_PLANS', '1') != '0'

    def pvconv_plans(self, vox_coords, norm_coords, resolution):
        _i32(vox_coords, 'vox_coords'); _f32(norm_coords, 'norm_coords')
        _shape(vox_coords.dim() == 3 and vox_coords.shape[1] == 3 and tuple(norm_coords.shape) == tuple(vox_coords.shape),
               'pvconv_plans: vox_coords / norm_coords (B,3,N) expected')
        b, _, n = vox_coords.shape
        r = int(resolution)
        vbytes, dbytes = self.lib.pvcnn_avg_voxelize_plan_bytes(b, n, r), self.lib.pvcnn_trilinear_devox_bwd_plan_bytes(b, n, r)
        if vbytes == 0 or dbytes == 0 or n == 0:
            return None
        dev = vox_coords.device
        vp = self.VoxelPlan()
        vp.r, vp.n, vp.b = r, n, b
        vp.ind = torch.empty((b, n), dtype=torch.int32, device=dev)
        vp.cnt = torch.empty((b, r * r * r), dtype=torch.int32, device=dev)
        vp.plan = torch.empty((vbytes,), dtype=torch.uint8, device=dev)
        dplan = torch.empty((dbytes,), dtype=torch.uint8, device=dev)
        scratch = self._scratch(self.lib.pvcnn_pvconv_plans_scratch_bytes(b, n, r), dev)
        with _Launch(vox_coords) as s:
            _lib.check(self.lib.pvcnn_pvconv_plans(_p(vox_coords), _p(norm_coords), b, n, r, _p(vp.ind), _p(vp.cnt), _p(vp.plan), vp.plan.numel(),
                                                   _p(dplan), dplan.numel(), _p(scratch), scratch.numel(), s), 'pvconv_plans')
        return vp, dplan

    def avg_voxelize_apply(self, features, vp):
        _f32(features, 'features')
        _shape(features.dim() == 3 and features.shape[0] == vp.b and features.shape[2] == vp.n, 'avg_voxelize: features do not match the plan')
        b, c, n = features.shape
        out = torch.empty((b, c, vp.r ** 3), dtype=torch.float32, device=features.device)
        with _Launch(features) as s:
            _lib.check(self.lib.pvcnn_avg_voxelize_apply(_p(features), _p(vp.plan), vp.plan.numel(), b, c, n, vp.r, _p(out), s),
                       'avg_voxelize_apply')
        return out

    def trilinear_devoxelize_backward_plan(self, indices, weights, r):
        _i32(indices, 'indices'); _f32(weights, 'weights')
        _shape(indices.dim() == 3 and indices.shape[1] == 8 and indices.shape == weights.shape, 'inds / wgts (B,8,N) expected')
        b, _, n = indices.shape
        r = int(r)
        nbytes = self.lib.pvcnn_trilinear_devox_bwd_plan_bytes(b, n, r)
        if nbytes == 0:
            return None
        plan = torch.empty((nbytes,), dtype=torch.uint8, device=indices.device)
        scratch = self._scratch(self.lib.pvcnn_trilinear_devox_bwd_plan_scratch_bytes(b, n, r), indices.device)
        with _Launch(indices) as s:
            _lib.check(self.lib.pvcnn_trilinear_devox_bwd_plan(_p(indices), _p(weights), b, n, r, _p(plan), plan.numel(),
                                                               _p(scratch), scratch.numel(), s), 'trilinear_devoxelize_backward_plan')
        return plan

    def trilinear_devoxelize_backward_apply(self, grad_y, plan, r):
        gy_bstride = _f32_rows(grad_y, 'grad_y')
        b, c, n = grad_y.shape
        r = int(r)
        grad_x = torch.empty((b, c, r * r * r), dtype=torch.float32, device=grad_y.device)
        with _Launch(grad_y) as s:
            _lib.check(self.lib.pvcnn_trilinear_devox_bwd_apply(_p(grad_y), gy_bstride, _p(plan), plan.numel(), b, c, n, r,
                                                                _p(grad_x), s), 'trilinear_devoxelize_backward_apply')
        return grad_x

    has_conv3d = True

    def _conv_wt(self, weight, for_bwd_data):
        co, ci = weight.shape[0], weight.shape[1]
        wt = torch.empty((ci * 27 * co,), dtype=torch.float32, device=weight.device)
        with _Launch(weight) as s:
            _lib.check(self.lib.pvcnn_conv3d_weight_transform(_p(weight), co, ci, int(for_bwd_data), _p(wt), s), 'conv3d_weight_transform')
        return wt

    def conv3d_forward(self, x, weight, bias, want_stats=False):
        _f32(x, 'x'); _f32(weight, 'weight')
        _shape(x.dim() == 5 and weight.dim() == 5 and tuple(weight.shape[2:]) == (3, 3, 3) and weight.shape[1] == x.shape[1]
               and x.shape[2] == x.shape[3] == x.shape[4], 'conv3d: x (B,Ci,R,R,R), weight (Co,Ci,3,3,3) expected')
        if bias is not None:
            _f32(bias, 'bias')
        b, ci, r = x.shape[0], x.shape[1], x.shape[2]
        co = weight.shape[0]
        wt = self._conv_wt(weight, False)
        y = torch.empty((b, co, r, r, r), dtype=torch.float32, device=x.device)
        if want_stats:
            part = torch.empty((co, self.lib.pvcnn_conv3d_fwd_stats_parts(b, co, r), 2), dtype=torch.float32, device=x.device)
            with _Launch(x) as s:
                _lib.check(self.lib.pvcnn_conv3d_fwd_stats(_p(x), _p(wt), _p(bias) if bias is not None else None, b, ci, co, r,
                                                           _p(y), _p(part), s), 'conv3d_forward')
            return y, part
        with _Launch(x) as s:
            _lib.check(self.lib.pvcnn_conv3d_fwd(_p(x), _p(wt), _p(bias) if bias is not None else None, b, ci, co, r, _p(y), s), 'conv3d_forward')
        return y

    def conv3d_backward_data(self, grad_y, weight):
        _f32(grad_y, 'grad_y'); _f32(weight, 'weight')
        b, co, r = grad_y.shape[0], grad_y.shape[1], grad_y.shape[2]
        ci = weight.shape[1]
        wt = self._conv_wt(weight, True)
        gx = torch.empty((b, ci, r, r, r), dtype=torch.float32, device=grad_y.device)
        with _Launch(grad_y) as s:
            _lib.check(self.lib.pvcnn_conv3d_fwd(_p(grad_y), _p(wt), None, b, co, ci, r, _p(gx), s), 'conv3d_backward_data')
        return gx

    has_grad_out = True

    @staticmethod
    def _grad_out(dst, shape, device):
        if dst is None:
            return torch.empty(shape, dtype=torch.float32, device=device)
        _shape(tuple(dst.shape) == tuple(shape) and dst.dtype == torch.float32 and dst.is_contiguous() and dst.device == device,
               'gradient destination: contiguous float32 tensor of the gradient\'s shape expected')
        return dst

    def conv3d_backward_weight(self, x, grad_y, with_bias=False, out_w=None, out_b=None):
        _f32(x, 'x'); _f32(grad_y, 'grad_y')
        b, ci, r = x.shape[0], x.shape[1], x.shape[2]
        co = grad_y.shape[1]
        gw = self._grad_out(out_w, (co, ci, 3, 3, 3), x.device)
        gb = self._grad_out(out_b, (co,), x.device) if with_bias else None
        ws = self._scratch(self.lib.pvcnn_conv3d_bwd_weight_workspace_bytes(b, ci, co, r), x.device)
        with _Launch(x) as s:
            _lib.check(self.lib.pvcnn_conv3d_bwd_weight(_p(x), _p(grad_y), b, ci, co, r, _p(gw), _p(gb) if with_bias else None,
                                                        _p(ws), ws.numel(), s), 'conv3d_backward_weight')
        return (gw, gb) if with_bias else gw


    has_conv3d_split = True
    conv_math = os.environ.get('PVCNN_CONV_MATH', 'f16x2')
    CONV_NSPLIT = {'f16x2': 2, 'bf16x3': 3, 'fp32': 0}

    def absmax_bits(self, x):
        _f32(x, 'x')
        out = torch.empty((1,), dtype=torch.int32, device=x.device)
        with _Launch(x) as s:
            _lib.check(self.lib.pvcnn_absmax_bits(_p(x), x.numel(), _p(out), s), 'absmax_bits')
        return out

    PW_AMAX_SEG = 256
    _TABLE_ONLY = ctypes.c_void_p(1)
    amax_global = os.environ.get('PVCNN_AMAX_GLOBAL', '0') == '1'

    def absmax_tiles(self, x, seg, want_global=True):
        _f32(x, 'x')
        _shape(x.dim() == 3, 'absmax_tiles: x (B,C,L) expected')
        b, c, n = x.shape
        seg = int(seg)
# ... 263 lines not shown
        amax_seg = int(amax_seg)
        armed = y_amax is not None
        if amax_seg > 0 and not armed:
            y_amax = self.amax_buffer(b, s3, amax_seg, dev)
        with _Launch(x) as s:
            _lib.check(self.lib.pvcnn_bnact_fwd(_p(x), _p(gamma) if gamma is not None else nul, _p(beta) if beta is not None else nul,
                                                _p(running_mean) if (training and running_mean is not None) else nul,
                                                _p(running_var) if (training and running_var is not None) else nul,
                                                b, c, s3, float(eps), float(momentum), float(slope), int(bool(training)),
                                                _p(mean), _p(rstd), _p(y), _p(y_amax) if amax_seg > 0 else nul, amax_seg, int(armed),
                                                _p(ws), ws.numel(), _p(drop[0]) if drop else nul, float(drop[1]) if drop else 0.0, s),
                       'bnact_forward')
        return (y, mean, rstd, y_amax) if amax_seg > 0 else (y, mean, rstd)

    has_bnact_rowmax = True

    def amax_and_row_keys(self, b, c, n, seg, device):
        words = self.lib.pvcnn_absmax_tiles_count(int(b), int(n), int(seg))
        off = (words + 1) // 2 * 2
        whole = torch.empty((off + 2 * int(b) * int(c),), dtype=torch.int32, device=device)
        return whole, whole[:words], whole[off:]

    def bnact_apply_rowmax(self, x, gamma, beta, mean, rstd, slope, amax_seg, y_amax, row_keys, out=None):
        _f32(x, 'x')
        b, c, s3 = x.shape
        _shape(s3 % 256 == 0 and amax_seg % 4 == 0 and 0 < amax_seg <= 256 and 256 % amax_seg == 0,
               'bnact_apply_rowmax: S % 256 == 0 and an amax_seg that is a multiple of 4 and divides 256 expected')
        if out is None:
            y = torch.empty_like(x)
        else:
            y = out
            _dev(y, 'out')
            _shape(tuple(y.shape) == tuple(x.shape) and y.dtype == torch.float32 and y.stride(2) == 1 and y.stride(1) == s3
                   and y.stride(0) >= c * s3 and y.stride(0) % 4 == 0 and y.data_ptr() % 16 == 0,
                   'bnact_apply_rowmax: out must be a (B, C, S) float32 view with contiguous, 16-byte aligned rows')
        ybs = int(y.stride(0)) if b > 1 else c * s3
        winners = torch.empty((b, c), dtype=torch.int64, device=x.device)
        values = torch.empty((b, c), dtype=torch.float32, device=x.device)
        nul = ctypes.c_void_p(None)
        with _Launch(x) as s:
            _lib.check(self.lib.pvcnn_bnact_apply_rowmax(_p(x), _p(gamma) if gamma is not None else nul, _p(beta) if beta is not None else nul,
                                                         _p(mean), _p(rstd), b, c, s3, float(slope), _p(y), ybs, _p(y_amax), int(amax_seg),
                                                         _p(row_keys), s), 'bnact_apply_rowmax')
            _lib.check(self.lib.pvcnn_row_keys_decode(_p(row_keys), _p(y), b * c, s3, _p(winners), _p(values), c, ybs, s), 'row_keys_decode')
        return y, winners, values

    has_devox_bnact = True

    def amax_buffer(self, b, n, seg, device):
        return torch.empty((self.lib.pvcnn_absmax_tiles_count(int(b), int(n), int(seg)),), dtype=torch.int32, device=device)

    def bn_finalize(self, part, count, running_mean, running_var, momentum, eps, shift=None, zero_word=None, counter=None):
        c, nparts = part.shape[0], part.shape[1]
        dev = part.device
        mean = torch.empty((c,), dtype=torch.float32, device=dev)
        rstd = torch.empty((c,), dtype=torch.float32, device=dev)
        nul = ctypes.c_void_p(None)
        with _Launch(part) as s:
            _lib.check(self.lib.pvcnn_bn_finalize(_p(part), c, nparts, float(count), float(eps), float(momentum),
                                                  _p(shift) if shift is not None else nul,
                                                  _p(running_mean) if running_mean is not None else nul,
                                                  _p(running_var) if running_var is not None else nul, _p(mean), _p(rstd),
                                                  _p(zero_word) if zero_word is not None else nul,
                                                  zero_word.numel() if zero_word is not None else 0,
                                                  _p(counter) if counter is not None else nul, s),
                       'bn_finalize')
        return mean, rstd

    def bn_stats(self, x, running_mean, running_var, momentum, eps):
        _f32(x, 'x')
        b, c, s3 = x.shape
        dev = x.device
        mean = torch.empty((c,), dtype=torch.float32, device=dev)
        rstd = torch.empty((c,), dtype=torch.float32, device=dev)
        ws = self._scratch(self.lib.pvcnn_bnact_workspace_bytes(b, c, s3), dev)
        nul = ctypes.c_void_p(None)
        with _Launch(x) as s:
            _lib.check(self.lib.pvcnn_bn_stats(_p(x), _p(running_mean) if running_mean is not None else nul,
                                               _p(running_var) if running_var is not None else nul, b, c, s3, float(eps),
                                               float(momentum), _p(mean), _p(rstd), _p(ws), ws.numel(), s), 'bn_stats')
        return mean, rstd

    def trilinear_devoxelize_bnact_forward(self, r, is_training, coords, features, gamma, beta, mean, rstd, slope, addend=None,
                                           se_scale=None):
        _f32(features, 'features'); _f32(coords, 'coords')
        r = int(r)
        _shape(features.dim() == 3 and coords.dim() == 3 and coords.shape[1] == 3
               and coords.shape[0] == features.shape[0] and features.shape[2] == r * r * r,
               'trilinear_devoxelize: coords (B,3,N), features (B,C,R^3) expected')
        b, c = features.shape[:2]
        n = coords.shape[2]
        dev = features.device
        if addend is not None:
            _f32(addend, 'addend')
            _shape(tuple(addend.shape) == (b, c, n), 'trilinear_devoxelize: addend (B,C,N) expected')
        if se_scale is not None:
            _f32(se_scale, 'se_scale')
            _shape(tuple(se_scale.shape) == (b, c), 'trilinear_devoxelize: se_scale (B,C) expected')
        outs = torch.empty((b, c, n), dtype=torch.float32, device=dev)
        if is_training:
            inds = torch.empty((b, 8, n), dtype=torch.int32, device=dev)
            wgts = torch.empty((b, 8, n), dtype=torch.float32, device=dev)
        else:
            inds, wgts = _dummies(dev)
        nul = ctypes.c_void_p(None)
        with _Launch(features) as s:
            _lib.check(self.lib.pvcnn_trilinear_devox_bnact_fwd(
                _p(coords), _p(features), _p(gamma) if gamma is not None else nul, _p(beta) if beta is not None else nul,
                _p(mean), _p(rstd), float(slope), b, c, n, r, int(bool(is_training)),
                _p(inds) if is_training else None, _p(wgts) if is_training else None,
                _p(addend) if addend is not None else None, _p(se_scale) if se_scale is not None else None, _p(outs), s),
                'trilinear_devoxelize_bnact_forward')
        return [outs, inds, wgts]

    has_concat_points = True

    def concat_points(self, tensors, want_amax=True, out=None, in_place=None, want_global=True):
        _shape(0 < len(tensors) <= 8, 'concat_points: 1..8 sources')
        b, n = tensors[0].shape[0], tensors[0].shape[2]
        ptrs, bstr, chans, pstr = [], [], [], []
        for i, t in enumerate(tensors):
            _dev(t, 'source')
            _shape(t.dim() == 3 and t.dtype == torch.float32 and t.shape[0] == b and t.shape[2] == n, 'concat_points: (B, C_i, N) float sources expected')
            c = t.shape[1]
            if n > 1 and t.stride(2) == 0:
                _shape(t.stride(1) == 1 or c == 1, 'concat_points: a broadcast source must be contiguous over (B, C)')
                pstr.append(0); bstr.append(t.stride(0) if b > 1 else c)
            else:
                _shape((n == 1 or t.stride(2) == 1) and (c == 1 or t.stride(1) == n), 'concat_points: rows must be contiguous inside a cloud')
                pstr.append(1); bstr.append(t.stride(0) if (b > 1 or (in_place and i in in_place)) else c * n)
            ptrs.append(t.data_ptr()); chans.append(c)
        k = len(tensors)
        if out is None:
            out = torch.empty((b, sum(chans), n), dtype=torch.float32, device=tensors[0].device)
        else:
            _f32(out, 'out')
            _shape(tuple(out.shape) == (b, sum(chans), n), 'concat_points: out (B, sum C_i, N) expected')
        pre = [None] * k
        for i, table in (in_place or {}).items():
            _shape(want_amax and table is not None and table.dtype == torch.int32 and table.is_cuda, 'concat_points: an in-place source comes with its amax buffer')
            pre[i] = table.data_ptr()
        amax = self.amax_buffer(b, n, self.PW_AMAX_SEG, out.device) if want_amax else None
        ticket = self._tickets(1, out.device) if want_amax else None
        with _Launch(out) as s:
            _lib.check(self.lib.pvcnn_concat_points((ctypes.c_void_p * k)(*ptrs), (ctypes.c_long * k)(*bstr), (ctypes.c_int * k)(*chans),
                                                    (ctypes.c_int * k)(*pstr), (ctypes.c_void_p * k)(*pre) if in_place else None, k, b, n,
                                                    _p(out), _p(amax) if want_amax else None,
                                                    (_p(ticket) if ticket is not None else None) if want_global or self.amax_global or not want_amax else self._TABLE_ONLY,
                                                    s), 'concat_points')
        return out, amax

    has_bnact_split_bwd = True

    has_dense_bn_relu = True

    def dense_bn_relu_supported(self, rows, cin, cout):
        return bool(self.lib.pvcnn_dense_bn_relu_supported(int(rows), int(cin), int(cout)))

    def dense_bn_relu_forward(self, x, weight, bias, gamma, beta, running_mean, running_var, counter, eps, momentum):
        _f32(x, 'x'); _f32(weight, 'weight')
        _shape(x.dim() == 2 and weight.dim() == 2 and weight.shape[1] == x.shape[1], 'dense_bn_relu: x (rows, Cin), weight (Cout, Cin) expected')
        rows, cin = x.shape
        cout = weight.shape[0]
        dev = x.device
        z = torch.empty((rows, cout), dtype=torch.float32, device=dev)
        y = torch.empty((rows, cout), dtype=torch.float32, device=dev)
        mean = torch.empty((cout,), dtype=torch.float32, device=dev)
        rstd = torch.empty((cout,), dtype=torch.float32, device=dev)
        opt = lambda t: _p(t) if t is not None else ctypes.c_void_p(None)
        with _Launch(x) as s:
            _lib.check(self.lib.pvcnn_dense_bn_relu_fwd(_p(x), _p(weight), opt(bias), opt(gamma), opt(beta), opt(running_mean), opt(running_var),
                                                        opt(counter), rows, cin, cout, float(eps), float(momentum), _p(z), _p(y), _p(mean),
                                                        _p(rstd), s), 'dense_bn_relu_forward')
        return y, z, mean, rstd

    def dense_bn_relu_backward(self, x, grad_y, z, mean, rstd, gamma, beta, out_w=None, out_b=None, out_gamma=None, out_beta=None):
        _f32(x, 'x'); _f32(grad_y, 'grad_y')
        rows, cin = x.shape
        cout = z.shape[1]
        dev = x.device
        gz = torch.empty((rows, cout), dtype=torch.float32, device=dev)
        gw = self._grad_out(out_w, (cout, cin), dev)
        gb = self._grad_out(out_b, (cout,), dev)
        gg = self._grad_out(out_gamma, (cout,), dev)
        gbeta = self._grad_out(out_beta, (cout,), dev)
        opt = lambda t: _p(t) if t is not None else ctypes.c_void_p(None)
        with _Launch(x) as s:
            _lib.check(self.lib.pvcnn_dense_bn_relu_bwd(_p(x), _p(grad_y), _p(z), _p(mean), _p(rstd), opt(gamma), opt(beta), rows, cin, cout,
                                                        _p(gz), _p(gw), _p(gb), _p(gg), _p(gbeta), s), 'dense_bn_relu_backward')
        return gz, gw, gb, gg, gbeta

    has_neighbor_max = True

    def neighbor_max_supported(self, k):
# ... 44 lines not shown
               and heading_bin_id.is_contiguous() and size_template_id.is_contiguous(), 'frustum_box_loss: shapes of modules/frustum.py:57-75 expected')
        loss = torch.empty((), dtype=torch.float32, device=center.device)
        grads = torch.empty((self.lib.pvcnn_frustum_box_loss_grad_floats(b, nh, ns),), dtype=torch.float32, device=center.device)
        with _Launch(center) as s:
            _lib.check(self.lib.pvcnn_frustum_box_loss(_p(center), _p(center_reg), _p(heading_scores), _p(size_scores), _p(hrn), _p(srn), _p(hr),
                                                       _p(sr), _p(heading_bin_id), _p(size_template_id), _p(heading_residual),
                                                       _p(size_residual), _p(center_t), _p(templates), _p(bin_centers), b, nh, ns,
                                                       float(bin_width), float(w_heading), float(w_size), float(w_corners), _p(loss),
                                                       _p(grads), s), 'frustum_box_loss')
        return loss, grads

    has_se_excite = True

    def se_excite_forward(self, part, gamma, beta, w1, w2, s3):
        c, b, slices, _ = part.shape
        h = w1.shape[0]
        _shape(tuple(w1.shape) == (h, c) and tuple(w2.shape) == (c, h) and c <= 2048 and h <= 256, 'se_excite: W1 (H,C), W2 (C,H), C <= 2048, H <= 256')
        dev = part.device
        a_sum, ax_sum, squeezed, excite = (torch.empty((b, c), dtype=torch.float32, device=dev) for _ in range(4))
        hidden = torch.empty((b, h), dtype=torch.float32, device=dev)
        nul = ctypes.c_void_p(None)
        with _Launch(part) as s:
            _lib.check(self.lib.pvcnn_se_excite_fwd(_p(part), slices, _p(gamma) if gamma is not None else nul, _p(beta) if beta is not None else nul,
                                                    _p(w1), _p(w2), b, c, h, 1.0 / float(s3), _p(a_sum), _p(ax_sum), _p(squeezed), _p(hidden),
                                                    _p(excite), s), 'se_excite_fwd')
        return a_sum, ax_sum, squeezed, hidden, excite

    def se_excite_backward(self, part, a_sum, ax_sum, gamma, beta, squeezed, hidden, excite, w1, w2, s3):
        c, b, slices, _ = part.shape
        h = w1.shape[0]
        dev = part.device
        g_w1 = torch.empty((h, c), dtype=torch.float32, device=dev)
        g_w2 = torch.empty((c, h), dtype=torch.float32, device=dev)
        g_mean = torch.empty((b, c), dtype=torch.float32, device=dev)
        sum_beta = torch.empty((c,), dtype=torch.float32, device=dev)
        sum_gamma = torch.empty((c,), dtype=torch.float32, device=dev)
        ws = torch.empty((b * (3 * c + h),), dtype=torch.float32, device=dev)
        nul = ctypes.c_void_p(None)
        with _Launch(part) as s:
            _lib.check(self.lib.pvcnn_se_excite_bwd(_p(part), slices, _p(a_sum), _p(ax_sum), _p(gamma) if gamma is not None else nul,
                                                    _p(beta) if beta is not None else nul, _p(squeezed), _p(hidden), _p(excite), _p(w1), _p(w2),
                                                    b, c, h, 1.0 / float(s3), _p(g_w1), _p(g_w2), _p(g_mean), _p(sum_beta), _p(sum_gamma),
                                                    _p(ws), s), 'se_excite_bwd')
        return g_w1, g_w2, g_mean, sum_beta, sum_gamma

    def bnact_partial_sums_raw(self, x, grad_y, gamma, beta, mean, rstd, slope):
        _f32(x, 'x')
        b, c, s3 = x.shape
        gy_bstride = _f32_rows(grad_y, 'grad_y') if grad_y is not None else c * s3
        slices = self.lib.pvcnn_bnact_slices(s3)
        part = torch.empty((c, b, slices, 2), dtype=torch.float32, device=x.device)
        nul = ctypes.c_void_p(None)
        with _Launch(x) as s:
            _lib.check(self.lib.pvcnn_bnact_partial_sums(_p(x), _p(grad_y) if grad_y is not None else nul, gy_bstride,
                                                         _p(gamma) if gamma is not None else nul, _p(beta) if beta is not None else nul,
                                                         _p(mean), _p(rstd), b, c, s3, float(slope), _p(part), s), 'bnact_partial_sums')
        return part

    def bnact_partial_sums(self, x, grad_y, gamma, beta, mean, rstd, slope):
        sums = self.bnact_partial_sums_raw(x, grad_y, gamma, beta, mean, rstd, slope).sum(dim=2)
        return sums[..., 0].t().contiguous(), sums[..., 1].t().contiguous()

    def bnact_backward_apply(self, x, grad_y, gamma, beta, mean, rstd, sum_gamma, sum_beta, slope, training, bc_mul=None, bc_add=None,
                             amax_seg=256):
        _f32(x, 'x')
        gy_bstride = _f32_rows(grad_y, 'grad_y')
        b, c, s3 = x.shape
        for t, name in ((bc_mul, 'bc_mul'), (bc_add, 'bc_add')):
            if t is not None:
                _f32(t, name)
                _shape(tuple(t.shape) == (b, c), f'{name} (B,C) expected')
        gx = torch.empty_like(x)
        amax = self.amax_buffer(b, s3, amax_seg, x.device)
        nul = ctypes.c_void_p(None)
        with _Launch(x) as s:
            _lib.check(self.lib.pvcnn_bnact_bwd_apply(_p(x), _p(grad_y), gy_bstride, _p(gamma) if gamma is not None else nul,
                                                      _p(beta) if beta is not None else nul, _p(mean), _p(rstd),
                                                      _p(sum_gamma) if sum_gamma is not None else nul, _p(sum_beta) if sum_beta is not None else nul,
                                                      _p(bc_mul) if bc_mul is not None else nul, _p(bc_add) if bc_add is not None else nul,
                                                      b, c, s3, float(slope), int(bool(training)), _p(gx), _p(amax), int(amax_seg), s),
                       'bnact_backward_apply')
        return gx, amax

    def bnact_backward(self, x, grad_y, gamma, beta, mean, rstd, slope, training, amax_seg=0, drop=None, out_w=None, out_b=None):
        _f32(x, 'x')
        gy_bstride = _f32_rows(grad_y, 'grad_y')
        b, c, s3 = x.shape
        dev = x.device
        gx = torch.empty_like(x)
        gg = self._grad_out(out_w, (c,), dev)
        gb = self._grad_out(out_b, (c,), dev)
        ws = self._scratch(self.lib.pvcnn_bnact_workspace_bytes(b, c, s3), dev)
        nul = ctypes.c_void_p(None)
        amax_seg = int(amax_seg)
        gx_amax = self.amax_buffer(b, s3, amax_seg, dev) if amax_seg > 0 else None
        tickets = self._tickets(c, dev)
        with _Launch(x) as s:
            _lib.check(self.lib.pvcnn_bnact_bwd_strided(_p(x), _p(grad_y), gy_bstride, _p(gamma) if gamma is not None else nul,
                                                        _p(beta) if beta is not None else nul, _p(mean), _p(rstd), b, c, s3, float(slope),
                                                        int(bool(training)), _p(gx), _p(gg), _p(gb),
                                                        _p(gx_amax) if amax_seg > 0 else nul, amax_seg, _p(ws), ws.numel(),
                                                        _p(drop[0]) if drop else nul, float(drop[1]) if drop else 0.0,
                                                        _p(tickets) if tickets is not None else nul, s), 'bnact_backward')
        return (gx, gg, gb, gx_amax) if amax_seg > 0 else (gx, gg, gb)


class _WeightBank:

    def __init__(self, be):
        import weakref
        self.be, self._weakref = be, weakref
        self.params = []
        self.seen = set()
        self.wanted = set()
        self.entries = {}
        self.tables = {}
        self.dirty = True
        self.epoch = 0
        self.pinned = []

    @staticmethod
    def _kind_of(p):
        if p.dim() == 5 and tuple(p.shape[2:]) == (3, 3, 3):
            return 'conv'
        if p.dim() in (3, 4) and all(k == 1 for k in p.shape[2:]):
            return 'pw'
        return None

    def register(self, model):
        import torch.nn as nn
        for m in model.modules():
            if isinstance(m, (nn.Conv1d, nn.Conv2d, nn.Conv3d)) and m.weight is not None and self._kind_of(m.weight) and id(m.weight) not in self.seen:
                self.seen.add(id(m.weight))
                self.params.append(self._weakref.ref(m.weight))
                self.dirty = True

    def take(self, kind, w, nsplit=2):
        key = (kind, w.data_ptr(), (int(w.shape[0]), int(w.shape[1])), int(nsplit))
        e = self.entries.get(key)
        if e is not None and e['armed']:
            e['armed'] = False
            p = e['param']()
            if p is not None and p._version == e['version'] and p.data_ptr() == key[1] and e['epoch'] == self.epoch:
                if e['wf'].is_cuda and torch.cuda.is_current_stream_capturing():
                    self._pin(e)
                return e['wf'], e['wb']
        if key not in self.wanted:
            if len(self.wanted) >= 4096:
                self.wanted.clear()
            self.wanted.add(key)
            self.dirty = True
        return None

    def _pin(self, e):
        if not e.get('pinned'):
            e['pinned'] = True
            self.pinned.append((e['wf'], e['wb']))

    def _rebuild(self):
        lib = self.be.lib
        live, by_kind = {}, {('conv', 2): [], ('pw', 2): [], ('conv', 1): [], ('pw', 1): []}
        for ref in self.params:
            p = ref()
            if p is None or not p.is_cuda or p.dtype != torch.float32 or not p.is_contiguous():
                continue
            kind = self._kind_of(p)
            for nsplit in (2, 1):
                key = (kind, p.data_ptr(), (int(p.shape[0]), int(p.shape[1])), nsplit)
                if key not in self.wanted:
                    continue
                e = self.entries.get(key)
                if e is None or e['param']() is not p:
                    co, ci = key[2]
                    nbytes = lib.pvcnn_conv3d_weight_split_bytes if kind == 'conv' else lib.pvcnn_pwconv_weight_split_bytes
                    e = {'param': ref, 'armed': False, 'version': -1, 'epoch': -1,
                         'wf': torch.empty((nbytes(co, ci, 0, nsplit),), dtype=torch.uint8, device=p.device),
                         'wb': torch.empty((nbytes(co, ci, 1, nsplit),), dtype=torch.uint8, device=p.device)}
                live[key] = e
# ... 50 lines not shown
```

pvcnn_amd/modules/functional/bnact.py:

```python
import contextlib
import threading

import torch
import torch.nn as nn
from torch.autograd import Function

from . import _cache, _gradslots
from ._autograd import native, amp_fwd, amp_bwd
from .devoxelization import CornerTaps


def _rows(t, shape):
    from .backend import batch_strided_ok
    if t.dim() == len(shape) and t.dim() >= 3:
        try:
            v = t.view(shape[0], shape[1], -1) if t.dim() > 3 else t
            if batch_strided_ok(v):
                return v
        except RuntimeError:
            pass
    return t.contiguous().view(shape[0], shape[1], -1)


def _servable(x):
    return x.dtype == torch.float32 or (torch.is_autocast_enabled() and x.dtype in (torch.bfloat16, torch.float16))


def _amax_seg_for(shape, is_cuda):
    be = native()
    if not is_cuda:
        return 0
    cap = getattr(be, 'BNACT_AMAX_MAX_SEG', 0)
    if len(shape) == 5 and shape[2] == shape[3] == shape[4]:
        ok = getattr(be, 'has_conv3d_split', False) and getattr(be, 'conv_math', '') == 'f16x2'
        return int(shape[2]) if ok and shape[2] <= cap else 0
    if len(shape) in (3, 4):
        ok = getattr(be, 'has_pwconv_split', False) and getattr(be, 'pw_math', '') == 'f16x2'
        seg = getattr(be, 'PW_AMAX_SEG', 0)
        return seg if ok and 0 < seg <= cap else 0
    return 0


def _bnact_backward(x3, g3, w, b, mean, rstd, slope, training, shape, drop=None):
    be = native()
    seg = _amax_seg_for(shape, x3.is_cuda)
    dst = _gradslots.destinations(be, w, b)
    if seg:
        gx, gw, gb, amax = be.bnact_backward(x3, g3, w, b, mean, rstd, slope, training, amax_seg=seg, **({'drop': drop} if drop else {}), **dst)
        return _cache.tag_amax(gx.view(shape), seg, amax), gw, gb
    assert drop is None, 'the fused dropout rides on the amax-emitting passes'  
    gx, gw, gb = be.bnact_backward(x3, g3, w, b, mean, rstd, slope, training, **dst)
    return gx.view(shape), gw, gb


__all__ = ['batch_norm_act', 'batch_norm_act_devoxelize', 'batch_norm_act_se_devoxelize', 'fusable_tail', 'run_layers', 'fused_dropout_ok']


class BatchNormAct(Function):
    @staticmethod
    @amp_fwd
    def forward(ctx, x, weight, bias, running_mean, running_var, training, momentum, eps, slope, stats_part=None, stats_shift=None,
                amax_seg=0, counter=None, drop_p=0.0, drop_seed=None, row_max=False):
        shape = x.shape
        x3 = x.contiguous().view(shape[0], shape[1], -1)
        w = weight.contiguous() if weight is not None else None
        b = bias.contiguous() if bias is not None else None
        stats = armed = None
        if training and stats_part is not None:
            if amax_seg and row_max:
                whole, armed, keys = native().amax_and_row_keys(x3.shape[0], x3.shape[1], x3.shape[2], amax_seg, x3.device)
                stats = native().bn_finalize(stats_part, x3.shape[0] * x3.shape[2], running_mean, running_var, momentum, eps, stats_shift,
                                             zero_word=whole, counter=counter)
                ctx.slope, ctx.training, ctx.shape, ctx.drop = slope, training, shape, None
                dest = getattr(_ROW_MAX, 'out', None)
                if dest is not None and not (dest.is_cuda and tuple(dest.shape) == tuple(x3.shape) and dest.dtype == torch.float32):
                    dest = None
                y, winners, values = native().bnact_apply_rowmax(x3, w, b, stats[0], stats[1], slope, amax_seg, armed, keys, out=dest)
                ctx.save_for_backward(x3, w, b, stats[0], stats[1])
                ctx.mark_non_differentiable(armed, winners, values)
                ctx.set_materialize_grads(False)
                return y.view(shape), armed, winners, values
            if amax_seg:
                armed = native().amax_buffer(x3.shape[0], x3.shape[2], amax_seg, x3.device)
                stats = native().bn_finalize(stats_part, x3.shape[0] * x3.shape[2], running_mean, running_var, momentum, eps, stats_shift,
                                             zero_word=armed, counter=counter)
            else:
                stats = native().bn_finalize(stats_part, x3.shape[0] * x3.shape[2], running_mean, running_var, momentum, eps, stats_shift,
                                             counter=counter)
        ctx.slope, ctx.training, ctx.shape = slope, training, shape
        ctx.drop = (drop_seed, float(drop_p)) if (drop_p and drop_seed is not None) else None
        if amax_seg:
            y, mean, rstd, amax = native().bnact_forward(x3, w, b, running_mean, running_var, training, momentum, eps, slope, stats=stats,
                                                         amax_seg=amax_seg, y_amax=armed, **({'drop': ctx.drop} if ctx.drop else {}))
            ctx.save_for_backward(x3, w, b, mean, rstd)
            ctx.mark_non_differentiable(amax)
            ctx.set_materialize_grads(False)
            return y.view(shape), amax
        y, mean, rstd = native().bnact_forward(x3, w, b, running_mean, running_var, training, momentum, eps, slope, stats=stats)
        ctx.save_for_backward(x3, w, b, mean, rstd)
        return y.view(shape)

    @staticmethod
    @amp_bwd
    def backward(ctx, grad_y, grad_amax=None, grad_winners=None, grad_values=None):
        if grad_y is None:
            return (None,) * 16
        x3, w, b, mean, rstd = ctx.saved_tensors
        g3 = _rows(grad_y, ctx.shape)
        gx, gw, gb = _bnact_backward(x3, g3, w, b, mean, rstd, ctx.slope, ctx.training, ctx.shape, drop=ctx.drop)
        return (gx, gw if w is not None else None, gb if b is not None else None,
                None, None, None, None, None, None, None, None, None, None, None, None, None)


_ROW_MAX = threading.local()


@contextlib.contextmanager
def emit_row_max(bn, out=None):
    prev = (getattr(_ROW_MAX, 'bn', None), getattr(_ROW_MAX, 'out', None))
    _ROW_MAX.bn, _ROW_MAX.out = bn, out
    try:
        yield
    finally:
        _ROW_MAX.bn, _ROW_MAX.out = prev


def _bn_mode(bn, finalize_counts=False):
    use_batch_stats = bn.training or bn.running_mean is None
    momentum = 0.0 if bn.momentum is None else bn.momentum
    counter = None
    if bn.training and bn.track_running_stats and bn.num_batches_tracked is not None:
        nbt = bn.num_batches_tracked
        if (finalize_counts and bn.momentum is not None and nbt.is_cuda and nbt.dtype == torch.int64 and nbt.numel() == 1):
            counter = nbt
        else:
            nbt.add_(1)
            if bn.momentum is None:
                momentum = 1.0 / float(nbt)
    rm = bn.running_mean if (bn.track_running_stats or not use_batch_stats) else None
    rv = bn.running_var if (bn.track_running_stats or not use_batch_stats) else None
    return use_batch_stats, momentum, rm, rv, counter


def _split(stats):
    if stats is None:
        return None, None
    part, shift = stats
    return part, (shift.detach().contiguous() if shift is not None else None)


def fused_dropout_ok(x):
    return (x.is_cuda and x.dtype == torch.float32 and getattr(native(), 'has_bnact_dropout', False) and not torch.is_autocast_enabled()
            and _amax_seg_for(x.shape, True) > 0 and 0 < x.numel() < (1 << 33))


def batch_norm_act(x, bn, slope, stats_part=None, drop_p=0.0):
    use_batch_stats, momentum, rm, rv, counter = _bn_mode(bn, finalize_counts=stats_part is not None and bn.training)
    part, shift = _split(stats_part)
    seg = _amax_seg_for(x.shape, x.is_cuda)
    if (seg and bn is getattr(_ROW_MAX, 'bn', None) and not drop_p and use_batch_stats and part is not None and x.dim() == 3
            and x.shape[2] % 256 == 0 and seg % 4 == 0 and x.dtype == torch.float32 and x.data_ptr() % 16 == 0 and x.is_contiguous()
            and getattr(native(), 'has_bnact_rowmax', False)):
        y, amax, winners, values = BatchNormAct.apply(x, bn.weight, bn.bias, rm, rv, use_batch_stats, momentum, bn.eps, slope, part, shift,
                                                      seg, counter, 0.0, None, True)
        y._pvcnn_row_max = (winners, values, y._version)
        return _cache.tag_amax(y, seg, amax)
    if seg:
        seed = torch.randint(-(1 << 62), 1 << 62, (1,), dtype=torch.int64, device=x.device) if drop_p else None
        y, amax = BatchNormAct.apply(x, bn.weight, bn.bias, rm, rv, use_batch_stats, momentum, bn.eps, slope, part, shift, seg, counter,
                                     float(drop_p), seed)
        return _cache.tag_amax(y, seg, amax)
    assert not drop_p, 'fused dropout: see fused_dropout_ok'
    return BatchNormAct.apply(x, bn.weight, bn.bias, rm, rv, use_batch_stats, momentum, bn.eps, slope, part, shift, 0, counter)


class BatchNormActDevoxelize(Function):

    @staticmethod
    @amp_fwd
    def forward(ctx, grid, coords, weight, bias, running_mean, running_var, use_batch_stats, momentum, eps, slope,
                resolution, is_training, stats_part=None, stats_shift=None, addend=None, counter=None):
        shape = grid.shape
        x3 = grid.contiguous().view(shape[0], shape[1], -1)
        w = weight.contiguous() if weight is not None else None
        b = bias.contiguous() if bias is not None else None
        if use_batch_stats and stats_part is not None:
            mean, rstd = native().bn_finalize(stats_part, x3.shape[0] * x3.shape[2], running_mean, running_var, momentum, eps, stats_shift,
                                              counter=counter)
        elif use_batch_stats:
            mean, rstd = native().bn_stats(x3, running_mean, running_var, momentum, eps)
        else:
            mean, rstd = running_mean.contiguous(), torch.rsqrt(running_var + eps)
        r = int(resolution)
        pts = coords.contiguous()
        add = addend.contiguous() if addend is not None else None
        ctx.has_addend = add is not None
        if not is_training:
            return native().trilinear_devoxelize_bnact_forward(r, False, pts, x3, w, b, mean, rstd, slope, add)[0]
        taps = CornerTaps.of(coords, r)
        out = taps.forward(lambda emit: native().trilinear_devoxelize_bnact_forward(r, emit, pts, x3, w, b, mean, rstd, slope, add))
        ctx.save_for_backward(x3, w, b, mean, rstd, taps.inds, taps.wgts)
        ctx.taps = taps
        ctx.slope, ctx.use_batch_stats, ctx.shape = slope, use_batch_stats, shape
        return out

    @staticmethod
    @amp_bwd
    def backward(ctx, grad_out):
        x3, w, b, mean, rstd, _, _ = ctx.saved_tensors
        g_act = ctx.taps.backward(_rows(grad_out, grad_out.shape))
        gx, gw, gb = _bnact_backward(x3, g_act.view(x3.shape), w, b, mean, rstd, ctx.slope, ctx.use_batch_stats, ctx.shape)
        return (gx, None, gw if w is not None else None, gb if b is not None else None,
                None, None, None, None, None, None, None, None, None, None, grad_out if ctx.has_addend else None, None)


def batch_norm_act_devoxelize(grid, coords, bn, slope, resolution, is_training, stats_part=None, addend=None):
    use_batch_stats, momentum, rm, rv, counter = _bn_mode(bn, finalize_counts=stats_part is not None and bn.training)
    part, shift = _split(stats_part)
    return BatchNormActDevoxelize.apply(grid, coords, bn.weight, bn.bias, rm, rv, use_batch_stats, momentum, bn.eps, slope,
                                        resolution, is_training, part, shift, addend, counter)


class BatchNormActSEDevoxelize(Function):

    @staticmethod
    @amp_fwd
    def forward(ctx, grid, coords, weight, bias, running_mean, running_var, use_batch_stats, momentum, eps, slope,
                resolution, is_training, stats_part, stats_shift, addend, counter, fc1, fc2):
        be = native()
        shape = grid.shape
        x3 = grid.contiguous().view(shape[0], shape[1], -1)
        nb, nc, s3 = x3.shape
        w = weight.contiguous() if weight is not None else None
        b = bias.contiguous() if bias is not None else None
        if use_batch_stats and stats_part is not None:
            mean, rstd = be.bn_finalize(stats_part, nb * s3, running_mean, running_var, momentum, eps, stats_shift, counter=counter)
        elif use_batch_stats:
            mean, rstd = be.bn_stats(x3, running_mean, running_var, momentum, eps)
        else:
            mean, rstd = running_mean.contiguous(), torch.rsqrt(running_var + eps)
        w1, w2 = fc1.contiguous(), fc2.contiguous()
        fused_se = getattr(be, 'has_se_excite', False) and nc <= 2048 and w1.shape[0] <= 256
        if fused_se:
            part = be.bnact_partial_sums_raw(x3, None, w, b, mean, rstd, slope)
            a_sum, ax_sum, squeezed, hidden, excite = be.se_excite_forward(part, w, b, w1, w2, s3)
        else:
            a_sum, ax_sum = be.bnact_partial_sums(x3, None, w, b, mean, rstd, slope)
            gam = w if w is not None else torch.ones_like(mean)
            bet = b if b is not None else torch.zeros_like(mean)
            squeezed = (gam * ax_sum + bet * a_sum) / float(s3)
            hidden = torch.relu(squeezed @ w1.t())
            excite = torch.sigmoid(hidden @ w2.t()).contiguous()
        r = int(resolution)
        pts = coords.contiguous()
        add = addend.contiguous() if addend is not None else None
        ctx.has_addend = add is not None
        if not is_training:
            return be.trilinear_devoxelize_bnact_forward(r, False, pts, x3, w, b, mean, rstd, slope, add, se_scale=excite)[0]
        taps = CornerTaps.of(coords, r)
        out = taps.forward(lambda emit: be.trilinear_devoxelize_bnact_forward(r, emit, pts, x3, w, b, mean, rstd, slope, add, se_scale=excite))
        ctx.save_for_backward(x3, w, b, mean, rstd, a_sum, ax_sum, squeezed, hidden, excite, w1, w2, taps.inds, taps.wgts)
        ctx.taps = taps
        ctx.slope, ctx.use_batch_stats, ctx.shape = slope, use_batch_stats, shape
        return out

    @staticmethod
    @amp_bwd
    def backward(ctx, grad_out):
        be = native()
        x3, w, b, mean, rstd, a_sum, ax_sum, squeezed, hidden, excite, w1, w2, _, _ = ctx.saved_tensors
        nb, nc, s3 = x3.shape
        g_y = ctx.taps.backward(_rows(grad_out, grad_out.shape)).view(x3.shape)
        if getattr(be, 'has_se_excite', False) and nc <= 2048 and w1.shape[0] <= 256:
            part = be.bnact_partial_sums_raw(x3, g_y, w, b, mean, rstd, ctx.slope)
            g_w1, g_w2, g_mean, sum_beta, sum_gamma = be.se_excite_backward(part, a_sum, ax_sum, w, b, squeezed, hidden, excite, w1, w2, s3)
        else:
            p_sum, q_sum = be.bnact_partial_sums(x3, g_y, w, b, mean, rstd, ctx.slope)
            gam = w if w is not None else torch.ones_like(mean)
            bet = b if b is not None else torch.zeros_like(mean)
            g_excite = gam * q_sum + bet * p_sum
            g_pre2 = g_excite * excite * (1.0 - excite)
            g_w2 = g_pre2.t() @ hidden
            g_pre1 = (g_pre2 @ w2) * (hidden > 0).to(hidden.dtype)
            g_w1 = g_pre1.t() @ squeezed
            g_mean = ((g_pre1 @ w1) / float(s3)).contiguous()
            sum_beta = (excite * p_sum + g_mean * a_sum).sum(dim=0).contiguous()
            sum_gamma = (excite * q_sum + g_mean * ax_sum).sum(dim=0).contiguous()
        seg = _amax_seg_for(ctx.shape, x3.is_cuda) or 256
        gx, amax = be.bnact_backward_apply(x3, g_y, w, b, mean, rstd, sum_gamma, sum_beta, ctx.slope, ctx.use_batch_stats,
                                           bc_mul=excite, bc_add=g_mean, amax_seg=seg)
        gx = gx.view(ctx.shape)
        if _amax_seg_for(ctx.shape, x3.is_cuda):
            _cache.tag_amax(gx, seg, amax)
        return (gx, None, sum_gamma if w is not None else None, sum_beta if b is not None else None,
                None, None, None, None, None, None, None, None, None, None, grad_out if ctx.has_addend else None, None, g_w1, g_w2)


def batch_norm_act_se_devoxelize(grid, coords, bn, slope, se, resolution, is_training, stats_part=None, addend=None):
    use_batch_stats, momentum, rm, rv, counter = _bn_mode(bn, finalize_counts=stats_part is not None and bn.training)
    part, shift = _split(stats_part)
    return BatchNormActSEDevoxelize.apply(grid, coords, bn.weight, bn.bias, rm, rv, use_batch_stats, momentum, bn.eps, slope,
                                          resolution, is_training, part, shift, addend, counter, se.fc[0].weight, se.fc[2].weight)

# ... 90 lines not shown
```

pvcnn_amd/modules/functional/devoxelization.py:

```python
from torch.autograd import Function

from . import _cache
from ._autograd import native, amp_fwd, amp_bwd

__all__ = ['trilinear_devoxelize', 'CornerTaps']


class CornerTaps:
    __slots__ = ('inds', 'wgts', 'plan', 'r')

    def __init__(self, r):
        self.inds = self.wgts = self.plan = None
        self.r = int(r)

    @staticmethod
    def of(coords, r):
        if coords.is_cuda and getattr(native(), 'has_scatter_plans', False):
            return _cache.memo(coords, ('corner_taps', int(r)), lambda: CornerTaps(r))
        return CornerTaps(r)

    def forward(self, run):
        if self.inds is None:
            outs, self.inds, self.wgts = run(True)
        else:
            outs = run(False)[0]
        return outs

    def backward(self, grad_points):
        be = native()
        if getattr(be, 'has_scatter_plans', False) and grad_points.is_cuda:
            if self.plan is None:
                made = be.trilinear_devoxelize_backward_plan(self.inds, self.wgts, self.r)
                self.plan = made if made is not None else False
            if self.plan is not False:
                return be.trilinear_devoxelize_backward_apply(grad_points, self.plan, self.r)
        return be.trilinear_devoxelize_backward(grad_points, self.inds, self.wgts, self.r)


class TrilinearDevoxelization(Function):

    @staticmethod
    @amp_fwd
    def forward(ctx, features, coords, resolution, is_training=True):
        nb, nc = features.shape[0], features.shape[1]
        grid = features.contiguous().view(nb, nc, -1)
        r = int(resolution)
        if not is_training:
            return native().trilinear_devoxelize_forward(r, False, coords.contiguous(), grid)[0]
        taps = CornerTaps.of(coords, r)
        pts = coords.contiguous()
        outs = taps.forward(lambda emit: native().trilinear_devoxelize_forward(r, emit, pts, grid))
        ctx.save_for_backward(taps.inds, taps.wgts)
        ctx.taps = taps
        return outs

    @staticmethod
    @amp_bwd
    def backward(ctx, grad_points):
        r = ctx.taps.r
        grad_grid = ctx.taps.backward(grad_points.contiguous())
        return grad_grid.view(grad_points.shape[0], grad_points.shape[1], r, r, r), None, None, None


trilinear_devoxelize = TrilinearDevoxelization.apply
```

pvcnn_amd/modules/pvconv.py:

```python
import torch
import torch.nn as nn

from . import functional as F
from .functional._autograd import native
from .functional.bnact import batch_norm_act_devoxelize, batch_norm_act_se_devoxelize, fusable_tail, run_layers
from .functional.conv3d import conv_nsplit, voxel_conv3d
from .se import SE3d
from .shared_mlp import SharedMLP
from .voxelization import Voxelization

__all__ = ['PVConv']


class _VoxelConv3d(nn.Conv3d):

    def _fast(self, x):
        return (x.is_cuda and getattr(native(), 'has_conv3d', False) and self.kernel_size == (3, 3, 3)
                and self.stride == (1, 1, 1) and self.padding == (1, 1, 1) and self.dilation == (1, 1, 1)
                and self.groups == 1 and self.padding_mode == 'zeros' and x.dim() == 5
                and x.shape[2] == x.shape[3] == x.shape[4] and self.weight.dtype == torch.float32
                and (x.dtype == torch.float32 or (torch.is_autocast_enabled() and x.dtype in (torch.bfloat16, torch.float16))))

    def forward(self, x):
        if not self._fast(x):
            return super().forward(x)
        return voxel_conv3d(x, self.weight, self.bias, False, conv_nsplit())

    def forward_with_stats(self, x):
        if not self._fast(x):
            return self.forward(x)
        return voxel_conv3d(x, self.weight, self.bias, True, conv_nsplit())


class PVConv(nn.Module):
    def __init__(self, in_channels, out_channels, kernel_size, resolution, with_se=False, normalize=True, eps=0):
        super().__init__()
        self.in_channels = in_channels
        self.out_channels = out_channels
        self.kernel_size = kernel_size
        self.resolution = resolution

        self.voxelization = Voxelization(resolution, normalize=normalize, eps=eps)
        pad = kernel_size // 2
        grid_ops = []
        for cin in (in_channels, out_channels):
            grid_ops += [_VoxelConv3d(cin, out_channels, kernel_size, stride=1, padding=pad),
                         nn.BatchNorm3d(out_channels, eps=1e-4),
                         nn.LeakyReLU(0.1, True)]
        if with_se:
            grid_ops.append(SE3d(out_channels))
        self.voxel_layers = nn.Sequential(*grid_ops)
        self.point_features = SharedMLP(in_channels, out_channels)

    def forward(self, inputs):
        features, coords = inputs
        grid, grid_coords = self.voxelization(features, coords)
        tail = fusable_tail(self.voxel_layers, grid) if self.resolution ** 3 * 4 <= 160 * 1024 else None
        if tail is not None:
            bn, slope, se = tail
            ntail = 2 if se is None else 3
            grid, stats_part = run_layers(self.voxel_layers, grid, stop=len(self.voxel_layers) - ntail, tail_stats=True)
            per_point = self.point_features(features)
            if se is None:
                fused = batch_norm_act_devoxelize(grid, grid_coords, bn, slope, self.resolution, self.training, stats_part,
                                                  addend=per_point)
            else:
                fused = batch_norm_act_se_devoxelize(grid, grid_coords, bn, slope, se, self.resolution, self.training, stats_part,
                                                     addend=per_point)
            return fused, coords
        else:
            hooked = bool(self.voxel_layers._forward_hooks or self.voxel_layers._forward_pre_hooks or self.voxel_layers._backward_hooks)
            grid = self.voxel_layers(grid) if hooked else run_layers(self.voxel_layers, grid)
            per_point = self.point_features(features)
            from_voxels = F.trilinear_devoxelize(grid, grid_coords, self.resolution, self.training)
        return from_voxels + per_point, coords
```

Baseline: 2572.

## Fuse point-branch BN-act into devoxelize and fold BN backward sums into scatter

In the PVConv forward, the point branch's BatchNorm+LeakyReLU is now deferred and applied inside the trilinear devoxelize+bnact kernel, together with the residual add. This removes a separate elementwise pass over the point features. In backward, the CSR segment-sum scatter kernel also accumulates the BatchNorm reduction partial sums, so the separate bnact reduce kernel is skipped and the finalize step reads the precomputed parts. The cost is more LDS in the scatter kernel and a requirement for one workgroup per slab; when that does not hold, the code falls back to the old path.

Result: faster. 2614 (median of 6 runs) (+1.6%).

```diff
diff --git a/include/pvcnn_hip.h b/include/pvcnn_hip.h
--- a/include/pvcnn_hip.h
+++ b/include/pvcnn_hip.h
@@ -14,7 +14,7 @@
 #define PVCNN_API
 #endif
 
-#define PVCNN_ABI_VERSION 12
+#define PVCNN_ABI_VERSION 13
 #define PVCNN_OK 0
 #define PVCNN_ERR_INVALID_ARGUMENT (-1)
 
@@ -155,7 +155,17 @@
 PVCNN_API int pvcnn_trilinear_devox_bnact_fwd(const float *coords, const float *feat, const float *gamma,
                                     const float *beta, const float *mean, const float *rstd, float slope,
                                     int B, int C, int N, int R, int is_training, int32_t *inds, float *wgts,
-                                    const float *addend, const float *se_scale, float *outs, void *stream);
+                                    const float *addend, const float *se_scale, const float *add_gamma, const float *add_beta,
+                                    const float *add_mean, const float *add_rstd, float add_slope, float *outs, void *stream);
+PVCNN_API int pvcnn_trilinear_devox_bwd_bn_parts(int B, int C, int N, int R);
+PVCNN_API int pvcnn_trilinear_devox_bwd_apply_bn(const float *grad_y, long grad_y_batch_stride, const void *plan, size_t plan_bytes,
+                                                 int B, int C, int N, int R, float *grad_x, const float *x, const float *gamma,
+                                                 const float *beta, const float *mean, const float *rstd, float slope, float *part,
+                                                 void *stream);
+PVCNN_API int pvcnn_bnact_bwd_from_parts(const float *x, const float *grad_y, long grad_y_batch_stride, const float *gamma,
+                                         const float *beta, const float *mean, const float *rstd, int B, int C, int S, float slope,
+                                         int training, float *grad_x, float *grad_gamma, float *grad_beta, void *gx_amax, int amax_seg,
+                                         const float *part, int nparts, void *stream);
 PVCNN_API int pvcnn_bnact_bwd(const float *x, const float *grad_y, const float *gamma, const float *beta,
                               const float *mean, const float *rstd, int B, int C, int S, float slope, int training,
                               float *grad_x, float *grad_gamma, float *grad_beta, void *workspace,
diff --git a/pvcnn_amd/_lib.py b/pvcnn_amd/_lib.py
--- a/pvcnn_amd/_lib.py
+++ b/pvcnn_amd/_lib.py
@@ -6,7 +6,7 @@
 
 _CSRC = os.path.join(os.path.dirname(os.path.abspath(__file__)), 'csrc')
 LIB_PATH = os.path.join(_CSRC, 'libpvcnn_hip.so')
-ABI_VERSION = 12
+ABI_VERSION = 13
 
 _vp, _i, _f, _sz, _l = ctypes.c_void_p, ctypes.c_int, ctypes.c_float, ctypes.c_size_t, ctypes.c_long
 
@@ -78,8 +78,12 @@
     'pvcnn_pwconv_fwd_stats': (_i, [_vp, _vp, _i, _vp, _i, _i, _i, _i, _vp, _vp, _vp]),
     'pvcnn_bn_finalize': (_i, [_vp, _i, ctypes.c_long, ctypes.c_double, _f, _f, _vp, _vp, _vp, _vp, _vp, _vp, ctypes.c_long, _vp, _vp]),
     'pvcnn_bn_stats': (_i, [_vp, _vp, _vp, _i, _i, _i, _f, _f, _vp, _vp, _vp, _sz, _vp]),
-    'pvcnn_trilinear_devox_bnact_fwd': (_i, [_vp, _vp, _vp, _vp, _vp, _vp, _f, _i, _i, _i, _i, _i, _vp, _vp, _vp, _vp, _vp, _vp]),
+    'pvcnn_trilinear_devox_bnact_fwd': (_i, [_vp, _vp, _vp, _vp, _vp, _vp, _f, _i, _i, _i, _i, _i, _vp, _vp, _vp, _vp, _vp, _vp, _vp, _vp, _f,
+                                                _vp, _vp]),
     'pvcnn_bnact_slices': (_i, [_i]),
+    'pvcnn_trilinear_devox_bwd_bn_parts': (_i, [_i, _i, _i, _i]),
+    'pvcnn_trilinear_devox_bwd_apply_bn': (_i, [_vp, _l, _vp, _sz, _i, _i, _i, _i, _vp, _vp, _vp, _vp, _vp, _vp, _f, _vp, _vp]),
+    'pvcnn_bnact_bwd_from_parts': (_i, [_vp, _vp, _l, _vp, _vp, _vp, _vp, _i, _i, _i, _f, _i, _vp, _vp, _vp, _vp, _i, _vp, _i, _vp]),
     'pvcnn_conv3d_weight_split_pair_entry': (_l, [_vp, _i, _i, _vp, _vp, _vp]),
     'pvcnn_conv3d_weight_split_pair_batch': (_i, [_vp, _i, _l, _vp]),
     'pvcnn_pwconv_weight_split_pair_entry': (_l, [_vp, _i, _i, _vp, _vp, _vp]),
diff --git a/pvcnn_amd/csrc/bnact.hip b/pvcnn_amd/csrc/bnact.hip
--- a/pvcnn_amd/csrc/bnact.hip
+++ b/pvcnn_amd/csrc/bnact.hip
@@ -561,7 +561,7 @@
                           const float *mean, const float *rstd, int B, int C, int S, float slope, int training, float *grad_x,
                           float *grad_gamma, float *grad_beta, void *workspace, size_t workspace_bytes, void *stream,
                           void *gx_amax = nullptr, int amax_seg = 0, const void *drop_seed = nullptr, float drop_p = 0.0f,
-                          void *tickets = nullptr) {
+                          void *tickets = nullptr, const float2 *given_part = nullptr, int given_nparts = 0) {
   PVCNN_REQUIRE(drop_p >= 0.0f && drop_p < 1.0f, "drop_p must be in [0, 1)");
   Drop drop{nullptr, 0u, 1.0f};
   const bool dropping = make_drop(drop_seed, drop_p, &drop);
@@ -569,8 +569,9 @@
   PVCNN_REQUIRE(B > 0 && C > 0 && S > 0 && x && grad_y && mean && rstd && grad_x && grad_gamma && grad_beta, "bad argument");
   PVCNN_REQUIRE(B <= 65535 && C <= 65535, "batch or channel count > 65535");
   PVCNN_REQUIRE(gy_bstride >= (long)C * S, "grad_y batch stride smaller than one sample");
-  PVCNN_REQUIRE(workspace && workspace_bytes >= pvcnn_bnact_workspace_bytes(B, C, S), "workspace too small");
+  PVCNN_REQUIRE(given_part || (workspace && workspace_bytes >= pvcnn_bnact_workspace_bytes(B, C, S)), "workspace too small");
   PVCNN_REQUIRE(!gx_amax || amax_seg_in_range(amax_seg), kAmaxSegRange);
+  PVCNN_REQUIRE(!given_part || (given_nparts > 0 && !dropping && !tickets), "given partial sums: no dropout, no tickets");
   hipStream_t s = static_cast<hipStream_t>(stream);
   const int slices = ceil_div(S, kBnSlice);
   const dim3 grid(slices, B, C);
@@ -578,15 +579,19 @@
   const long zero_count = gx_amax ? 1 + (long)B * ceil_div(S, amax_seg) : 0L;
   PVCNN_REQUIRE(!tickets || (reinterpret_cast<uintptr_t>(tickets) & 3) == 0, "tickets must be 4-byte aligned");
   const BwdFold fold{static_cast<unsigned *>(tickets), grad_gamma, grad_beta, static_cast<uint32_t *>(gx_amax), zero_count};
-  if (dropping)
-    hipLaunchKernelGGL(bnact_bwd_reduce_kernel<true>, grid, dim3(kBnThreads), 0, s, x, grad_y, mean, rstd, gamma, beta, slope, C, S, slices, part,
-                       gy_bstride, drop, fold);
-  else
-    hipLaunchKernelGGL(bnact_bwd_reduce_kernel<false>, grid, dim3(kBnThreads), 0, s, x, grad_y, mean, rstd, gamma, beta, slope, C, S, slices, part,
-                       gy_bstride, Drop{nullptr, 0u, 1.0f}, fold);
-  if (int e = check_launch("bnact_bwd_reduce")) return e;
+  if (given_part) {
+    part = const_cast<float2 *>(given_part);
+  } else {
+    if (dropping)
+      hipLaunchKernelGGL(bnact_bwd_reduce_kernel<true>, grid, dim3(kBnThreads), 0, s, x, grad_y, mean, rstd, gamma, beta, slope, C, S, slices,
+                         part, gy_bstride, drop, fold);
+    else
+      hipLaunchKernelGGL(bnact_bwd_reduce_kernel<false>, grid, dim3(kBnThreads), 0, s, x, grad_y, mean, rstd, gamma, beta, slope, C, S, slices,
+                         part, gy_bstride, Drop{nullptr, 0u, 1.0f}, fold);
+    if (int e = check_launch("bnact_bwd_reduce")) return e;
+  }
   if (tickets == nullptr) {
-    hipLaunchKernelGGL(bnact_bwd_finalize_kernel, dim3(C), dim3(64), 0, s, part, B * slices, grad_gamma, grad_beta,
+    hipLaunchKernelGGL(bnact_bwd_finalize_kernel, dim3(C), dim3(64), 0, s, part, given_part ? given_nparts : B * slices, grad_gamma, grad_beta,
                        static_cast<uint32_t *>(gx_amax), zero_count);
     if (int e = check_launch("bnact_bwd_finalize")) return e;
   }
@@ -625,6 +630,16 @@
                                        void *stream) {
   return bnact_bwd_impl(x, grad_y, grad_y_batch_stride, gamma, beta, mean, rstd, B, C, S, slope, training, grad_x, grad_gamma,
                         grad_beta, workspace, workspace_bytes, stream, gx_amax, amax_seg, drop_seed, drop_p, tickets);
+}
+
+extern "C" int pvcnn_bnact_bwd_from_parts(const float *x, const float *grad_y, long grad_y_batch_stride, const float *gamma,
+                                          const float *beta, const float *mean, const float *rstd, int B, int C, int S, float slope,
+                                          int training, float *grad_x, float *grad_gamma, float *grad_beta, void *gx_amax, int amax_seg,
+                                          const float *part, int nparts, void *stream) {
+  PVCNN_REQUIRE(part && nparts > 0, "partial sums missing");
+  return bnact_bwd_impl(x, grad_y, grad_y_batch_stride, gamma, beta, mean, rstd, B, C, S, slope, training, grad_x, grad_gamma,
+                        grad_beta, nullptr, 0, stream, gx_amax, amax_seg, nullptr, 0.0f, nullptr, reinterpret_cast<const float2 *>(part),
+                        nparts);
 }
 
 extern "C" int pvcnn_bnact_slices(int S) { return S > 0 ? ceil_div(S, kBnSlice) : 0; }
diff --git a/pvcnn_amd/csrc/csr.h b/pvcnn_amd/csrc/csr.h
--- a/pvcnn_amd/csrc/csr.h
+++ b/pvcnn_amd/csrc/csr.h
@@ -568,13 +568,22 @@
                       (int)blockIdx.y);
 }
 
-template <int G>
+constexpr int kBnSumSlice = 8192;
+static_assert(kBnSumSlice == 2 * kTileTargets && kTileThreads == 4 * 256, "a slice = two tiles, one 256-thread group per channel");
+struct BnSums {
+  const float *x, *mean, *rstd, *gamma, *beta;
+  float slope;
+  float2 *part;
+};
+
+template <int G, bool BN = false>
 __global__ __launch_bounds__(kTileThreads) void segsum_tile_kernel(const float *__restrict__ src, const int2 *__restrict__ seg,
                                                                    const int2 *__restrict__ ent, const uint16_t *__restrict__ order,
                                                                    const int32_t *__restrict__ gofs, const int2 *__restrict__ entw,
                                                                    float *__restrict__ dst, int C, int L, int J, int E,
-                                                                   long src_bstride, int nsplit, int JP) {
+                                                                   long src_bstride, int nsplit, int JP, BnSums bn = BnSums{}) {
   extern __shared__ __attribute__((aligned(16))) float lds[];
+  [[maybe_unused]] float bn_s = 0.f, bn_q = 0.f;
   using vecG = __attribute__((ext_vector_type(G))) float;
   const int b = blockIdx.z, split = blockIdx.y, c0 = blockIdx.x * G, tid = threadIdx.x;
   const int g = min(G, C - c0);
@@ -689,11 +698,77 @@
         out[(size_t)c * L + i] = tile[c * kTileTargets + i];
       }
     }
+    if constexpr (BN) {
+      const int c = tid >> 8, vt = tid & 255;
+      float *bn_sm = tile + (size_t)G * kTileTargets;
+      if (c < g) {
+        const int ch = c0 + c;
+        const float m = bn.mean[ch], rs = bn.rstd[ch];
+        const float scale = (bn.gamma ? bn.gamma[ch] : 1.0f) * rs;
+        const float shift = (bn.beta ? bn.beta[ch] : 0.0f) - m * scale;
+        const float *xr = bn.x + ((size_t)b * C + ch) * L + t0;
+        const float *tr = tile + c * kTileTargets;
+        for (int i = vt * 4; i < nt; i += 256 * 4) {
+          const float4 xv = ld4(xr + i);
+          const float4 gv = *reinterpret_cast<const float4 *>(tr + i);
+          const float xs_[4] = {xv.x, xv.y, xv.z, xv.w}, gs_[4] = {gv.x, gv.y, gv.z, gv.w};
+#pragma unroll
+          for (int u = 0; u < 4; ++u) {
+            const float z = fmaf(xs_[u], scale, shift);
+            const float gg = gs_[u] * (z > 0.f ? 1.0f : bn.slope);
+            bn_s += gg;
+            bn_q += gg * ((xs_[u] - m) * rs);
+          }
+        }
+      }
+      if ((r & 1) || r + 1 == nr) {
+#pragma unroll
+        for (int d = 32; d >= 1; d >>= 1) { bn_s += __shfl_xor(bn_s, d); bn_q += __shfl_xor(bn_q, d); }
+        const int wave = (tid >> 6) & 3;
+        if ((tid & 63) == 0 && c < G) { bn_sm[c * 8 + wave] = bn_s; bn_sm[c * 8 + 4 + wave] = bn_q; }
+        __syncthreads();
+        if (vt == 0 && c < g) {
+          const float s = bn_sm[c * 8] + bn_sm[c * 8 + 1] + bn_sm[c * 8 + 2] + bn_sm[c * 8 + 3];
+          const float q = bn_sm[c * 8 + 4] + bn_sm[c * 8 + 5] + bn_sm[c * 8 + 6] + bn_sm[c * 8 + 7];
+          bn.part[((size_t)(c0 + c) * gridDim.z + b) * ceil_div(L, kBnSumSlice) + (r >> 1)] = make_float2(s, q);
+        }
+        bn_s = bn_q = 0.f;
+      }
+    }
     lds_barrier();
   }
 }
 
 inline bool csr_supported(int L, long E) { return L <= kCsrMaxTargets && E <= 0x7fffffffL / 8; }
+
+struct CsrTileChoice { int G, nsplit, GS; };
+inline CsrTileChoice csr_tile_choice(int B, int C, int L, int J, int E) {
+  const int JP = (J + 3) & ~3;
+  int G = 0;
+  for (int cand = 4; cand >= 1; cand >>= 1)
+    if ((size_t)cand * (JP + kTileTargets) * sizeof(float) <= (size_t)kLdsBytesPerCU) { G = cand; break; }
+  const size_t row = (size_t)J * sizeof(float);
+  int GS = 1;
+  if (row > 0 && row <= 64 * 1024) {
+    GS = (int)std::min<size_t>(8, (64 * 1024) / row);
+    while (GS > 1 && (long)B * ceil_div(C, GS) < 2L * kNumCU) GS >>= 1;
+    if (GS >= 8) GS = 8; else if (GS >= 4) GS = 4; else if (GS >= 2) GS = 2; else GS = 1;
+  }
+  const bool very_sparse = (long)E * 4 <= (long)L && row > 0 && row <= (size_t)kLdsBytesPerCU && (long)B * ceil_div(C, GS) >= kNumCU;
+  if (G <= 0 || J <= 0 || very_sparse) return CsrTileChoice{0, 0, GS};
+  while (G > 1 && G / 2 >= C) G >>= 1;
+  const int nr = ceil_div(L, kTileTargets), slabs = ceil_div(C, G);
+  int nsplit = 1;
+  while (nsplit < nr && (long)B * slabs * nsplit < kNumCU) nsplit <<= 1;
+  return CsrTileChoice{G, std::min(nsplit, nr), GS};
+}
+
+inline bool csr_tile_bn_sums_ok(int B, int C, int L, int J, int E) {
+  const CsrTileChoice tc = csr_tile_choice(B, C, L, J, E);
+  const int JP = (J + 3) & ~3;
+  return tc.G > 0 && tc.nsplit == 1 && (L & 3) == 0 &&
+         (size_t)tc.G * (JP + kTileTargets + 2 * 4) * sizeof(float) <= (size_t)kLdsBytesPerCU;
+}
 
 template <int G, bool STAGE>
 int launch_segsum_g(const float *src, const CsrPlan &ws, float *dst, int B, int C, int L, int J, int E,
@@ -773,7 +848,7 @@
 }
 
 inline int launch_csr_apply(const float *src, const void *plan, size_t plan_bytes, float *dst, int B, int C, int L, int J, long E_,
-                            hipStream_t s, const char *what, long src_bstride = 0) {
+                            hipStream_t s, const char *what, long src_bstride = 0, const BnSums *bn = nullptr) {
   if (src_bstride <= 0) src_bstride = (long)C * J;
   const int E = (int)E_;
   if (B == 0 || C == 0) return 0;
@@ -784,35 +859,44 @@
   CsrPlan pl;
   pl.carve(const_cast<void *>(plan), B, L, E);
   const int JP = (J + 3) & ~3;
-  int G = 0;
-  for (int cand = 4; cand >= 1; cand >>= 1)
-    if ((size_t)cand * (JP + kTileTargets) * sizeof(float) <= (size_t)kLdsBytesPerCU) { G = cand; break; }
+  const CsrTileChoice tc = csr_tile_choice(B, C, L, J, E);
+  const int G = tc.G, GS = tc.GS;
   const size_t row = (size_t)J * sizeof(float);
-  int GS = 1;
-  if (row > 0 && row <= 64 * 1024) {
-    GS = (int)std::min<size_t>(8, (64 * 1024) / row);
-    while (GS > 1 && (long)B * ceil_div(C, GS) < 2L * kNumCU) GS >>= 1;
-    if (GS >= 8) GS = 8; else if (GS >= 4) GS = 4; else if (GS >= 2) GS = 2; else GS = 1;
-  }
-  const bool very_sparse = (long)E * 4 <= (long)L && row > 0 && row <= (size_t)kLdsBytesPerCU && (long)B * ceil_div(C, GS) >= kNumCU;
-  if (G > 0 && J > 0 && !very_sparse) {
-    while (G > 1 && G / 2 >= C) G >>= 1;
-    const int nr = ceil_div(L, kTileTargets), slabs = ceil_div(C, G);
-    int nsplit = 1;
-    while (nsplit < nr && (long)B * slabs * nsplit < kNumCU) nsplit <<= 1;
-    nsplit = std::min(nsplit, nr);
-    const size_t lds = (size_t)G * (JP + kTileTargets) * sizeof(float);
+  if (G > 0) {
+    const int slabs = ceil_div(C, G), nsplit = tc.nsplit;
+    size_t lds = (size_t)G * (JP + kTileTargets) * sizeof(float);
     const dim3 grid(slabs, nsplit, B);
+    if (bn) {
+      lds += 2 * G * 4 * sizeof(float);
+      if (!csr_tile_bn_sums_ok(B, C, L, J, E) || !aligned16(bn->x)) {
+        set_error("%s: BatchNorm sums need one workgroup per slab, L %% 4 == 0 and an aligned x", what);
+        return PVCNN_ERR_INVALID_ARGUMENT;
+      }
+#define PVCNN_TILE_BN(GV)                                                                                                \
+  do {                                                                                                                   \
+    auto k = segsum_tile_kernel<GV, true>;                                                                               \
+    if (int e = enable_big_lds(k, lds)) { set_error("%s: LDS attribute: %d", what, e); return e; }                       \
+    hipLaunchKernelGGL(k, grid, dim3(kTileThreads), lds, s, src, pl.seg, pl.ent, pl.order, pl.gofs, pl.entw, dst, C, L, J, E,  \
+                       src_bstride, nsplit, JP, *bn);                                                                             \
+  } while (0)
+      if (G == 4) PVCNN_TILE_BN(4); else if (G == 2) PVCNN_TILE_BN(2); else PVCNN_TILE_BN(1);
+#undef PVCNN_TILE_BN
+      return check_launch(what);
+    }
 #define PVCNN_TILE(GV)                                                                                                   \
   do {                                                                                                                   \
     auto k = segsum_tile_kernel<GV>;                                                                                     \
     if (int e = enable_big_lds(k, lds)) { set_error("%s: LDS attribute: %d", what, e); return e; }                       \
     hipLaunchKernelGGL(k, grid, dim3(kTileThreads), lds, s, src, pl.seg, pl.ent, pl.order, pl.gofs, pl.entw, dst, C, L, J, E,  \
-                       src_bstride, nsplit, JP);                                                                                      \
+                       src_bstride, nsplit, JP, BnSums{});                                                                            \
   } while (0)
     if (G == 4) PVCNN_TILE(4); else if (G == 2) PVCNN_TILE(2); else PVCNN_TILE(1);
 #undef PVCNN_TILE
     return check_launch(what);
+  }
+  if (bn) {
+    set_error("%s: BatchNorm sums need the tile kernel", what);
+    return PVCNN_ERR_INVALID_ARGUMENT;
   }
   const bool stage = row > 0 && row <= (size_t)kLdsBytesPerCU;
   const bool vec = (L % 4 == 0) && aligned16(dst);
diff --git a/pvcnn_amd/csrc/devoxelize.hip b/pvcnn_amd/csrc/devoxelize.hip
--- a/pvcnn_amd/csrc/devoxelize.hip
+++ b/pvcnn_amd/csrc/devoxelize.hip
@@ -34,18 +34,27 @@
 extern "C" int pvcnn_trilinear_devox_bnact_fwd(const float *coords, const float *feat, const float *gamma,
                                                const float *beta, const float *mean, const float *rstd, float slope, int B,
                                                int C, int N, int R, int is_training, int32_t *inds, float *wgts,
-                                               const float *addend, const float *se_scale, float *outs, void *stream) {
+                                               const float *addend, const float *se_scale, const float *add_gamma,
+                                               const float *add_beta, const float *add_mean, const float *add_rstd, float add_slope,
+                                               float *outs, void *stream) {
   PVCNN_REQUIRE(B >= 0 && C > 0 && N >= 0 && R > 0, "bad size");
   PVCNN_REQUIRE((long)R * R * R * sizeof(float) <= (size_t)kLdsBytesPerCU, "grid row does not fit LDS: use bnact_fwd + trilinear_devox_fwd");
   if (B == 0 || N == 0) return 0;
   PVCNN_REQUIRE(coords && outs && feat && mean && rstd, "null pointer");
   PVCNN_REQUIRE(!is_training || (inds && wgts), "training mode needs inds and wgts");
   PVCNN_REQUIRE(B <= 65535, "batch > 65535");
+  PVCNN_REQUIRE(!add_mean == !add_rstd, "add_mean and add_rstd: both or neither");
+  PVCNN_REQUIRE(!add_mean || addend, "an addend transform needs the addend");
   hipStream_t s = static_cast<hipStream_t>(stream);
   TrilinearFromCoords p{coords, is_training ? inds : nullptr, is_training ? wgts : nullptr, N, R, R * R};
   bool vec = (N % 4 == 0) && aligned16(coords) && aligned16(outs) && (!addend || aligned16(addend));
   if (is_training) vec = vec && aligned16(inds) && aligned16(wgts);
   const XfBnAct xf{gamma, beta, mean, rstd, slope, se_scale};
+  if (add_mean) {
+    const XfBnAct axf{add_gamma, add_beta, add_mean, add_rstd, add_slope, nullptr};
+    return launch_gather(p, feat, outs, B, C, R * R * R, N, vec, s, "trilinear_devox_bnact_fwd", xf, grid_pad_shift(R), addend,
+                         axf);
+  }
   return launch_gather(p, feat, outs, B, C, R * R * R, N, vec, s, "trilinear_devox_bnact_fwd", xf, grid_pad_shift(R), addend);
 }
 
@@ -126,3 +135,24 @@
   return launch_csr_apply(grad_y, plan, plan_bytes, grad_x, B, C, S, N, 8L * N, static_cast<hipStream_t>(stream),
                           "trilinear_devox_bwd_apply", grad_y_batch_stride);
 }
+
+extern "C" int pvcnn_trilinear_devox_bwd_bn_parts(int B, int C, int N, int R) {
+  if (B <= 0 || C <= 0 || N <= 0 || R <= 0 || B > 65535) return 0;
+  const long S = (long)R * R * R;
+  if (S > 0x7fffffffL / 4 || !csr_supported((int)S, 8L * N)) return 0;
+  return csr_tile_bn_sums_ok(B, C, (int)S, N, 8 * N) ? B * ceil_div((int)S, kBnSumSlice) : 0;
+}
+
+extern "C" int pvcnn_trilinear_devox_bwd_apply_bn(const float *grad_y, long grad_y_batch_stride, const void *plan, size_t plan_bytes,
+                                                  int B, int C, int N, int R, float *grad_x, const float *x, const float *gamma,
+                                                  const float *beta, const float *mean, const float *rstd, float slope, float *part,
+                                                  void *stream) {
+  PVCNN_REQUIRE(pvcnn_trilinear_devox_bwd_bn_parts(B, C, N, R) > 0, "no BatchNorm sums for this problem (pvcnn_trilinear_devox_bwd_bn_parts)");
+  PVCNN_REQUIRE(grad_x && grad_y && x && mean && rstd && part, "null pointer");
+  PVCNN_REQUIRE(aligned16(x) && aligned16(grad_x), "x / grad_x must be 16-byte aligned");
+  PVCNN_REQUIRE(grad_y_batch_stride >= (long)C * N, "grad_y batch stride smaller than one cloud");
+  const int S = R * R * R;
+  const BnSums bn{x, mean, rstd, gamma, beta, slope, reinterpret_cast<float2 *>(part)};
+  return launch_csr_apply(grad_y, plan, plan_bytes, grad_x, B, C, S, N, 8L * N, static_cast<hipStream_t>(stream),
+                          "trilinear_devox_bwd_apply_bn", grad_y_batch_stride, &bn);
+}
diff --git a/pvcnn_amd/csrc/slab.h b/pvcnn_amd/csrc/slab.h
--- a/pvcnn_amd/csrc/slab.h
+++ b/pvcnn_amd/csrc/slab.h
@@ -245,6 +245,18 @@
   }
 };
 
+template <class AXF>
+struct AddendXf {
+  float scale = 1.0f, shift = 0.0f;
+  const AXF &xf;
+  __device__ __forceinline__ AddendXf(const AXF &x, int c) : xf(x) {
+    if constexpr (!AXF::kIdentity) xf.params(c, scale, shift);
+  }
+  __device__ __forceinline__ float operator()(float v) const {
+    if constexpr (AXF::kIdentity) return v; else return xf.apply(v, scale, shift);
+  }
+};
+
 template <int THREADS, class XF>
 __device__ __forceinline__ void slab_copy_row_xf(float *dst, const float *src, int len, const XF &xf, int c) {
   float scale, shift;
@@ -310,11 +322,11 @@
   }
 }
 
-template <class P, int VEC, int THREADS, bool RESIDENT, class XF, bool PAD>
+template <class P, int VEC, int THREADS, bool RESIDENT, class XF, bool PAD, class AXF = XfNone>
 __global__ __launch_bounds__(THREADS) void gather_lds_kernel(P p, XF xf, const float *__restrict__ src,
                                                              float *__restrict__ dst, int C, int L,
                                                              int J, int G, int SEQ, int pshift,
-                                                             const float *__restrict__ addend = nullptr) {
+                                                             const float *__restrict__ addend = nullptr, AXF axf = AXF{}) {
   extern __shared__ __attribute__((aligned(16))) float lds[];
   constexpr int NC = P::NC;
   const int b = blockIdx.y;
@@ -356,15 +368,19 @@
       }
       for (int c = 0; c < g; ++c) {
         const float *row = lds + c * Lp;
+        const AddendXf<AXF> fa(axf, c0 + c);
         if constexpr (VEC == 4) {
           const float r0 = combine<NC, P::kMaySkip, PAD>(t[0], row, pshift), r1 = combine<NC, P::kMaySkip, PAD>(t[1], row, pshift);
           float r2 = combine<NC, P::kMaySkip, PAD>(t[2], row, pshift), r3 = combine<NC, P::kMaySkip, PAD>(t[3], row, pshift);
           float q0 = r0, q1 = r1;
-          if (add) { const float4 a = ld4(add + (size_t)c * J + j0); q0 = q0 + a.x; q1 = q1 + a.y; r2 = r2 + a.z; r3 = r3 + a.w; }
+          if (add) {
+            const float4 a = ld4(add + (size_t)c * J + j0);
+            q0 = q0 + fa(a.x); q1 = q1 + fa(a.y); r2 = r2 + fa(a.z); r3 = r3 + fa(a.w);
+          }
           st4(out + (size_t)c * J + j0, q0, q1, r2, r3);
         } else {
           float r = combine<NC, P::kMaySkip, PAD>(t[0], row, pshift);
-          if (add) r = r + add[(size_t)c * J + j0];
+          if (add) r = r + fa(add[(size_t)c * J + j0]);
           out[(size_t)c * J + j0] = r;
         }
       }
@@ -372,10 +388,10 @@
   }
 }
 
-template <class P, class XF>
+template <class P, class XF, class AXF = XfNone>
 __global__ __launch_bounds__(1024) void gather_lds_pipe_kernel(P p, XF xf, const float *__restrict__ src, float *__restrict__ dst,
                                                                int C, int L, int J, int SEQ, int pshift,
-                                                               const float *__restrict__ addend = nullptr) {
+                                                               const float *__restrict__ addend = nullptr, AXF axf = AXF{}) {
   extern __shared__ __attribute__((aligned(16))) float lds[];
   constexpr int NC = P::NC, THREADS = 1024, kB = 8;
   const int b = blockIdx.y;
@@ -451,8 +467,9 @@
       r[h] = combine<NC, P::kMaySkip, true>(t, lds, pshift);
     }
     if (addend) {
-      r[0] = r[0] + __uint_as_float(add.x); r[1] = r[1] + __uint_as_float(add.y);
-      r[2] = r[2] + __uint_as_float(add.z); r[3] = r[3] + __uint_as_float(add.w);
+      const AddendXf<AXF> fa(axf, c);
+      r[0] = r[0] + fa(__uint_as_float(add.x)); r[1] = r[1] + fa(__uint_as_float(add.y));
+      r[2] = r[2] + fa(__uint_as_float(add.z)); r[3] = r[3] + fa(__uint_as_float(add.w));
     }
     const __amdgpu_buffer_rsrc_t drsrc = row_descriptor(dst, rowoff, J * 4);
     u32x4 o;
@@ -467,10 +484,10 @@
   }
 }
 
-template <class P, class XF, int G>
+template <class P, class XF, int G, class AXF = XfNone>
 __global__ __launch_bounds__(1024) void gather_lds_pipe_rows_kernel(P p, XF xf, const float *__restrict__ src, float *__restrict__ dst,
                                                                 int C, int L, int J, int SEQ, int pshift,
-                                                                const float *__restrict__ addend = nullptr) {
+                                                                const float *__restrict__ addend = nullptr, AXF axf = AXF{}) {
   extern __shared__ __attribute__((aligned(16))) float lds[];
   constexpr int NC = P::NC, THREADS = 1024;
   const int b = blockIdx.y;
@@ -566,8 +583,9 @@
 #pragma unroll
     for (int u = 0; u < G; ++u) {
       if (addend) {
-        r[u][0] = r[u][0] + __uint_as_float(add[u].x); r[u][1] = r[u][1] + __uint_as_float(add[u].y);
-        r[u][2] = r[u][2] + __uint_as_float(add[u].z); r[u][3] = r[u][3] + __uint_as_float(add[u].w);
+        const AddendXf<AXF> fa(axf, min(c0 + u, C - 1));
+        r[u][0] = r[u][0] + fa(__uint_as_float(add[u].x)); r[u][1] = r[u][1] + fa(__uint_as_float(add[u].y));
+        r[u][2] = r[u][2] + fa(__uint_as_float(add[u].z)); r[u][3] = r[u][3] + fa(__uint_as_float(add[u].w));
       }
       u32x4 o;
       o.x = __float_as_uint(r[u][0]); o.y = __float_as_uint(r[u][1]); o.z = __float_as_uint(r[u][2]); o.w = __float_as_uint(r[u][3]);
@@ -653,9 +671,10 @@
   return 0;
 }
 
-template <class P, class XF = XfNone>
+template <class P, class XF = XfNone, class AXF = XfNone>
 int launch_gather(const P &p, const float *src, float *dst, int B, int C, int L, int J, bool vec_ok,
-                  hipStream_t s, const char *what, const XF &xf = XF{}, int pshift = 0, const float *addend = nullptr) {
+                  hipStream_t s, const char *what, const XF &xf = XF{}, int pshift = 0, const float *addend = nullptr,
+                  const AXF &axf = AXF{}) {
   if (B == 0 || C == 0 || J == 0) return 0;
   if (pshift > 0 && (size_t)(L + (L >> pshift)) * sizeof(float) > (size_t)kLdsBytesPerCU) pshift = 0;
   SlabPlan pl = plan_slab(B, C, L, pshift);
@@ -666,17 +685,17 @@
       const int slabs = ceil_div(C, GR);
       const int seq = (int)std::min<long>(8, std::max<long>(1, (long)B * slabs / kNumCU));
       const size_t bytes = (size_t)GR * (L + (L >> pshift)) * sizeof(float);
-      auto k = gather_lds_pipe_rows_kernel<P, XF, GR>;
+      auto k = gather_lds_pipe_rows_kernel<P, XF, GR, AXF>;
       if (int e = enable_big_lds(k, bytes)) { set_error("%s: LDS attribute: %d", what, e); return e; }
-      hipLaunchKernelGGL(k, dim3(ceil_div(slabs, seq), B), dim3(1024), bytes, s, p, xf, src, dst, C, L, J, seq, pshift, addend);
+      hipLaunchKernelGGL(k, dim3(ceil_div(slabs, seq), B), dim3(1024), bytes, s, p, xf, src, dst, C, L, J, seq, pshift, addend, axf);
       return check_launch(what);
     }
   }
   if (!pl.lds) {
-    if (!XF::kIdentity || addend) {
+    if (!XF::kIdentity || !AXF::kIdentity || addend) {
       set_error("%s: row does not fit LDS; the fused transform / addend needs the LDS path", what);
       return PVCNN_ERR_INVALID_ARGUMENT;
-    } else if constexpr (XF::kIdentity) {
+    } else if constexpr (XF::kIdentity && AXF::kIdentity) {
       const int CT = 16;
       hipLaunchKernelGGL((gather_direct_kernel<P>), dim3(ceil_div(J, 256), ceil_div(C, CT), B), dim3(256), 0, s,
                          p, src, dst, C, L, J, CT);
@@ -688,17 +707,17 @@
     static const bool pipe = [] { const char *e = getenv("PVCNN_GATHER_PIPE"); return !(e && e[0] == '0'); }();
     if (pipe && pl.threads == 1024 && pl.G == 1 && pshift > 0 && vec_ok && J <= 1024 * 4 && (L & 3) == 0 && (L >> 2) <= 1024 * 8 &&
         aligned16(src) && (((size_t)L * sizeof(float)) & 15) == 0) {
-      auto k = gather_lds_pipe_kernel<P, XF>;
+      auto k = gather_lds_pipe_kernel<P, XF, AXF>;
       if (int e = enable_big_lds(k, pl.bytes)) { set_error("%s: LDS attribute: %d", what, e); return e; }
-      hipLaunchKernelGGL(k, grid, dim3(1024), pl.bytes, s, p, xf, src, dst, C, L, J, pl.seq, pshift, addend);
+      hipLaunchKernelGGL(k, grid, dim3(1024), pl.bytes, s, p, xf, src, dst, C, L, J, pl.seq, pshift, addend, axf);
       return check_launch(what);
     }
   }
 #define PVCNN_LAUNCH_GATHER_P(VEC, T, PADV)                                                      \
   do {                                                                                           \
-    auto k = (J <= T * VEC) ? gather_lds_kernel<P, VEC, T, true, XF, PADV> : gather_lds_kernel<P, VEC, T, false, XF, PADV>; \
+    auto k = (J <= T * VEC) ? gather_lds_kernel<P, VEC, T, true, XF, PADV, AXF> : gather_lds_kernel<P, VEC, T, false, XF, PADV, AXF>; \
     if (int e = enable_big_lds(k, pl.bytes)) { set_error("%s: LDS attribute: %d", what, e); return e; } \
-    hipLaunchKernelGGL(k, grid, dim3(T), pl.bytes, s, p, xf, src, dst, C, L, J, pl.G, pl.seq, pshift, addend); \
+    hipLaunchKernelGGL(k, grid, dim3(T), pl.bytes, s, p, xf, src, dst, C, L, J, pl.G, pl.seq, pshift, addend, axf); \
   } while (0)
 #define PVCNN_LAUNCH_GATHER(VEC, T)                                                              \
   do {                                                                                           \
diff --git a/pvcnn_amd/modules/functional/backend.py b/pvcnn_amd/modules/functional/backend.py
--- a/pvcnn_amd/modules/functional/backend.py
+++ b/pvcnn_amd/modules/functional/backend.py
@@ -429,15 +429,32 @@
                                                                _p(scratch), scratch.numel(), s), 'trilinear_devoxelize_backward_plan')
         return plan
 
-    def trilinear_devoxelize_backward_apply(self, grad_y, plan, r):
+    def trilinear_devoxelize_backward_apply(self, grad_y, plan, r, bn=None):
         gy_bstride = _f32_rows(grad_y, 'grad_y')
         b, c, n = grad_y.shape
         r = int(r)
         grad_x = torch.empty((b, c, r * r * r), dtype=torch.float32, device=grad_y.device)
+        if bn is not None:
+            x, gamma, beta, mean, rstd, slope = bn
+            _f32(x, 'x'); _f32(mean, 'mean'); _f32(rstd, 'rstd')
+            _shape(tuple(x.shape) == (b, c, r * r * r), 'trilinear_devoxelize_backward_apply: x (B,C,R^3) expected')
+            nparts = self.trilinear_devoxelize_backward_bn_parts(b, c, n, r)
+            _shape(nparts > 0, 'trilinear_devoxelize_backward_apply: no BatchNorm sums for this problem')
+            part = torch.empty((c, nparts, 2), dtype=torch.float32, device=grad_y.device)
+            nul = ctypes.c_void_p(None)
+            with _Launch(grad_y) as s:
+                _lib.check(self.lib.pvcnn_trilinear_devox_bwd_apply_bn(
+                    _p(grad_y), gy_bstride, _p(plan), plan.numel(), b, c, n, r, _p(grad_x), _p(x),
+                    _p(gamma) if gamma is not None else nul, _p(beta) if beta is not None else nul, _p(mean), _p(rstd), float(slope),
+                    _p(part), s), 'trilinear_devoxelize_backward_apply_bn')
+            return grad_x, part
         with _Launch(grad_y) as s:
             _lib.check(self.lib.pvcnn_trilinear_devox_bwd_apply(_p(grad_y), gy_bstride, _p(plan), plan.numel(), b, c, n, r,
                                                                 _p(grad_x), s), 'trilinear_devoxelize_backward_apply')
         return grad_x
+
+    def trilinear_devoxelize_backward_bn_parts(self, b, c, n, r):
+        return int(self.lib.pvcnn_trilinear_devox_bwd_bn_parts(int(b), int(c), int(n), int(r)))
 
     has_conv3d = True
 
@@ -867,7 +884,7 @@
         return mean, rstd
 
     def trilinear_devoxelize_bnact_forward(self, r, is_training, coords, features, gamma, beta, mean, rstd, slope, addend=None,
-                                           se_scale=None):
+                                           se_scale=None, addend_bn=None):
         _f32(features, 'features'); _f32(coords, 'coords')
         r = int(r)
         _shape(features.dim() == 3 and coords.dim() == 3 and coords.shape[1] == 3
@@ -882,6 +899,16 @@
         if se_scale is not None:
             _f32(se_scale, 'se_scale')
             _shape(tuple(se_scale.shape) == (b, c), 'trilinear_devoxelize: se_scale (B,C) expected')
+        a_gamma = a_beta = a_mean = a_rstd = None
+        a_slope = 0.0
+        if addend_bn is not None:
+            _shape(addend is not None, 'trilinear_devoxelize: addend_bn needs the addend')
+            a_gamma, a_beta, a_mean, a_rstd, a_slope = addend_bn
+            for t, what in ((a_gamma, 'addend gamma'), (a_beta, 'addend beta'), (a_mean, 'addend mean'), (a_rstd, 'addend rstd')):
+                if t is not None:
+                    _f32(t, what)
+                    _shape(t.dim() == 1 and t.numel() == c and t.is_contiguous(), 'trilinear_devoxelize: addend statistics (C,) expected')
+            _shape(a_mean is not None and a_rstd is not None, 'trilinear_devoxelize: addend_bn needs mean and rstd')
         outs = torch.empty((b, c, n), dtype=torch.float32, device=dev)
         if is_training:
             inds = torch.empty((b, 8, n), dtype=torch.int32, device=dev)
@@ -894,7 +921,9 @@
                 _p(coords), _p(features), _p(gamma) if gamma is not None else nul, _p(beta) if beta is not None else nul,
                 _p(mean), _p(rstd), float(slope), b, c, n, r, int(bool(is_training)),
                 _p(inds) if is_training else None, _p(wgts) if is_training else None,
-                _p(addend) if addend is not None else None, _p(se_scale) if se_scale is not None else None, _p(outs), s),
+                _p(addend) if addend is not None else None, _p(se_scale) if se_scale is not None else None,
+                _p(a_gamma) if a_gamma is not None else nul, _p(a_beta) if a_beta is not None else nul,
+                _p(a_mean) if a_mean is not None else nul, _p(a_rstd) if a_rstd is not None else nul, float(a_slope), _p(outs), s),
                 'trilinear_devoxelize_bnact_forward')
         return [outs, inds, wgts]
 
@@ -1105,7 +1134,8 @@
                        'bnact_backward_apply')
         return gx, amax
 
-    def bnact_backward(self, x, grad_y, gamma, beta, mean, rstd, slope, training, amax_seg=0, drop=None, out_w=None, out_b=None):
+    def bnact_backward(self, x, grad_y, gamma, beta, mean, rstd, slope, training, amax_seg=0, drop=None, out_w=None, out_b=None,
+                       parts=None):
         _f32(x, 'x')
         gy_bstride = _f32_rows(grad_y, 'grad_y')
         b, c, s3 = x.shape
@@ -1113,10 +1143,20 @@
         gx = torch.empty_like(x)
         gg = self._grad_out(out_w, (c,), dev)
         gb = self._grad_out(out_b, (c,), dev)
-        ws = self._scratch(self.lib.pvcnn_bnact_workspace_bytes(b, c, s3), dev)
         nul = ctypes.c_void_p(None)
         amax_seg = int(amax_seg)
         gx_amax = self.amax_buffer(b, s3, amax_seg, dev) if amax_seg > 0 else None
+        if parts is not None:
+            _f32(parts, 'parts')
+            _shape(drop is None and parts.dim() == 3 and parts.shape[0] == c and parts.shape[2] == 2, 'bnact_backward: parts (C, nparts, 2)')
+            with _Launch(x) as s:
+                _lib.check(self.lib.pvcnn_bnact_bwd_from_parts(_p(x), _p(grad_y), gy_bstride, _p(gamma) if gamma is not None else nul,
+                                                               _p(beta) if beta is not None else nul, _p(mean), _p(rstd), b, c, s3,
+                                                               float(slope), int(bool(training)), _p(gx), _p(gg), _p(gb),
+                                                               _p(gx_amax) if amax_seg > 0 else nul, amax_seg, _p(parts), parts.shape[1], s),
+                           'bnact_backward_from_parts')
+            return (gx, gg, gb, gx_amax) if amax_seg > 0 else (gx, gg, gb)
+        ws = self._scratch(self.lib.pvcnn_bnact_workspace_bytes(b, c, s3), dev)
         tickets = self._tickets(c, dev)
         with _Launch(x) as s:
             _lib.check(self.lib.pvcnn_bnact_bwd_strided(_p(x), _p(grad_y), gy_bstride, _p(gamma) if gamma is not None else nul,
diff --git a/pvcnn_amd/modules/functional/bnact.py b/pvcnn_amd/modules/functional/bnact.py
--- a/pvcnn_amd/modules/functional/bnact.py
+++ b/pvcnn_amd/modules/functional/bnact.py
@@ -1,4 +1,5 @@
 import contextlib
+import os
 import threading
 
 import torch
@@ -41,19 +42,23 @@
     return 0
 
 
-def _bnact_backward(x3, g3, w, b, mean, rstd, slope, training, shape, drop=None):
+def _bnact_backward(x3, g3, w, b, mean, rstd, slope, training, shape, drop=None, parts=None):
     be = native()
     seg = _amax_seg_for(shape, x3.is_cuda)
     dst = _gradslots.destinations(be, w, b)
     if seg:
-        gx, gw, gb, amax = be.bnact_backward(x3, g3, w, b, mean, rstd, slope, training, amax_seg=seg, **({'drop': drop} if drop else {}), **dst)
+        gx, gw, gb, amax = be.bnact_backward(x3, g3, w, b, mean, rstd, slope, training, amax_seg=seg, **({'drop': drop} if drop else {}),
+                                             **({'parts': parts} if parts is not None else {}), **dst)
         return _cache.tag_amax(gx.view(shape), seg, amax), gw, gb
     assert drop is None, 'the fused dropout rides on the amax-emitting passes'  
-    gx, gw, gb = be.bnact_backward(x3, g3, w, b, mean, rstd, slope, training, **dst)
+    gx, gw, gb = be.bnact_backward(x3, g3, w, b, mean, rstd, slope, training, **({'parts': parts} if parts is not None else {}), **dst)
     return gx.view(shape), gw, gb
 
 
-__all__ = ['batch_norm_act', 'batch_norm_act_devoxelize', 'batch_norm_act_se_devoxelize', 'fusable_tail', 'run_layers', 'fused_dropout_ok']
+__all__ = ['batch_norm_act', 'batch_norm_act_devoxelize', 'batch_norm_act_se_devoxelize', 'fusable_tail', 'run_layers', 'fused_dropout_ok',
+           'point_branch_deferred']
+
+_BN_FOLD = os.environ.get('PVCNN_BN_FOLD', '1') != '0'
 
 
 class BatchNormAct(Function):
@@ -179,7 +184,8 @@
     @staticmethod
     @amp_fwd
     def forward(ctx, grid, coords, weight, bias, running_mean, running_var, use_batch_stats, momentum, eps, slope,
-                resolution, is_training, stats_part=None, stats_shift=None, addend=None, counter=None):
+                resolution, is_training, stats_part=None, stats_shift=None, addend=None, counter=None,
+                add_weight=None, add_bias=None, add_mean=None, add_rstd=None, add_slope=0.0):
         shape = grid.shape
         x3 = grid.contiguous().view(shape[0], shape[1], -1)
         w = weight.contiguous() if weight is not None else None
@@ -195,11 +201,21 @@
         pts = coords.contiguous()
         add = addend.contiguous() if addend is not None else None
         ctx.has_addend = add is not None
+        add_bn = None
+        if add_mean is not None:
+            aw = add_weight.contiguous() if add_weight is not None else None
+            ab = add_bias.contiguous() if add_bias is not None else None
+            add_bn = (aw, ab, add_mean, add_rstd, add_slope)
         if not is_training:
-            return native().trilinear_devoxelize_bnact_forward(r, False, pts, x3, w, b, mean, rstd, slope, add)[0]
+            return native().trilinear_devoxelize_bnact_forward(r, False, pts, x3, w, b, mean, rstd, slope, add, addend_bn=add_bn)[0]
         taps = CornerTaps.of(coords, r)
-        out = taps.forward(lambda emit: native().trilinear_devoxelize_bnact_forward(r, emit, pts, x3, w, b, mean, rstd, slope, add))
-        ctx.save_for_backward(x3, w, b, mean, rstd, taps.inds, taps.wgts)
+        out = taps.forward(lambda emit: native().trilinear_devoxelize_bnact_forward(r, emit, pts, x3, w, b, mean, rstd, slope, add,
+                                                                                   addend_bn=add_bn))
+        if add_bn is None:
+            ctx.save_for_backward(x3, w, b, mean, rstd, taps.inds, taps.wgts)
+        else:
+            ctx.save_for_backward(x3, w, b, mean, rstd, taps.inds, taps.wgts, add, *add_bn[:4])
+        ctx.add_slope = add_slope if add_bn is not None else None
         ctx.taps = taps
         ctx.slope, ctx.use_batch_stats, ctx.shape = slope, use_batch_stats, shape
         return out
@@ -207,18 +223,56 @@
     @staticmethod
     @amp_bwd
     def backward(ctx, grad_out):
-        x3, w, b, mean, rstd, _, _ = ctx.saved_tensors
-        g_act = ctx.taps.backward(_rows(grad_out, grad_out.shape))
-        gx, gw, gb = _bnact_backward(x3, g_act.view(x3.shape), w, b, mean, rstd, ctx.slope, ctx.use_batch_stats, ctx.shape)
+        x3, w, b, mean, rstd = ctx.saved_tensors[:5]
+        g_rows = _rows(grad_out, grad_out.shape)
+        taken = None
+        if _BN_FOLD and ctx.use_batch_stats and x3.dtype == torch.float32:
+            taken = ctx.taps.backward_bn_sums(g_rows, (x3, w, b, mean, rstd, ctx.slope))
+        if taken is not None:
+            g_act, parts = taken
+            gx, gw, gb = _bnact_backward(x3, g_act.view(x3.shape), w, b, mean, rstd, ctx.slope, ctx.use_batch_stats, ctx.shape,
+                                         parts=parts)
+        else:
+            g_act = ctx.taps.backward(g_rows)
+            gx, gw, gb = _bnact_backward(x3, g_act.view(x3.shape), w, b, mean, rstd, ctx.slope, ctx.use_batch_stats, ctx.shape)
+        g_add, g_aw, g_ab = (grad_out if ctx.has_addend else None), None, None
+        if ctx.add_slope is not None:
+            add, aw, ab, amean, arstd = ctx.saved_tensors[7:]
+            g_add, g_aw, g_ab = _bnact_backward(add, _rows(grad_out, add.shape), aw, ab, amean, arstd, ctx.add_slope, True, add.shape)
+            g_aw, g_ab = (g_aw if aw is not None else None), (g_ab if ab is not None else None)
         return (gx, None, gw if w is not None else None, gb if b is not None else None,
-                None, None, None, None, None, None, None, None, None, None, grad_out if ctx.has_addend else None, None)
-
-
-def batch_norm_act_devoxelize(grid, coords, bn, slope, resolution, is_training, stats_part=None, addend=None):
+                None, None, None, None, None, None, None, None, None, None, g_add, None, g_aw, g_ab, None, None, None)
+
+
+def batch_norm_act_devoxelize(grid, coords, bn, slope, resolution, is_training, stats_part=None, addend=None, addend_bn=None):
     use_batch_stats, momentum, rm, rv, counter = _bn_mode(bn, finalize_counts=stats_part is not None and bn.training)
     part, shift = _split(stats_part)
+    if addend_bn is None:
+        return BatchNormActDevoxelize.apply(grid, coords, bn.weight, bn.bias, rm, rv, use_batch_stats, momentum, bn.eps, slope,
+                                            resolution, is_training, part, shift, addend, counter)
+    pbn, pslope, pmean, prstd = addend_bn
     return BatchNormActDevoxelize.apply(grid, coords, bn.weight, bn.bias, rm, rv, use_batch_stats, momentum, bn.eps, slope,
-                                        resolution, is_training, part, shift, addend, counter)
+                                        resolution, is_training, part, shift, addend, counter, pbn.weight, pbn.bias, pmean, prstd, pslope)
+
+
+def point_branch_deferred(mlp, x):
+    mods = list(getattr(mlp, 'layers', ()))
+    be = native()
+    if not (_BN_FOLD and x.is_cuda and x.dtype == torch.float32 and x.dim() == 3 and x.numel() > 0 and not torch.is_autocast_enabled()
+            and getattr(be, 'has_bnact', False) and getattr(be, 'has_pwconv', False) and getattr(be, 'has_devox_bnact', False)
+            and len(mods) == 3 and _is_pointwise(mods[0]) and isinstance(mods[0], nn.Conv1d) and _wants_batch_stats(mods[1])
+            and mods[1].training and _slope(mods[2]) is not None and not _has_hooks(mlp) and not _has_hooks(mlp.layers)
+            and not any(_has_hooks(m) for m in mods)
+            and _amax_seg_for((x.shape[0], mods[0].out_channels, x.shape[2]), True) > 0):
+        return mlp(x), None
+    bn, slope = mods[1], _slope(mods[2])
+    y, stats_part = run_layers(mlp.layers, x, stop=1, tail_stats=True)
+    if stats_part is None:
+        return batch_norm_act(y, bn, slope), None
+    _, momentum, rm, rv, counter = _bn_mode(bn, finalize_counts=True)
+    part, shift = _split(stats_part)
+    mean, rstd = native().bn_finalize(part, y.shape[0] * y.shape[2], rm, rv, momentum, bn.eps, shift, counter=counter)
+    return y, (bn, slope, mean, rstd)
 
 
 class BatchNormActSEDevoxelize(Function):
diff --git a/pvcnn_amd/modules/functional/devoxelization.py b/pvcnn_amd/modules/functional/devoxelization.py
--- a/pvcnn_amd/modules/functional/devoxelization.py
+++ b/pvcnn_amd/modules/functional/devoxelization.py
@@ -25,6 +25,20 @@
         else:
             outs = run(False)[0]
         return outs
+
+    def backward_bn_sums(self, grad_points, bn):
+        be = native()
+        if not (getattr(be, 'has_scatter_plans', False) and grad_points.is_cuda and hasattr(be, 'trilinear_devoxelize_backward_bn_parts')):
+            return None
+        b, c, n = grad_points.shape
+        if be.trilinear_devoxelize_backward_bn_parts(b, c, n, self.r) <= 0:
+            return None
+        if self.plan is None:
+            made = be.trilinear_devoxelize_backward_plan(self.inds, self.wgts, self.r)
+            self.plan = made if made is not None else False
+        if self.plan is False:
+            return None
+        return be.trilinear_devoxelize_backward_apply(grad_points, self.plan, self.r, bn=bn)
 
     def backward(self, grad_points):
         be = native()
diff --git a/pvcnn_amd/modules/pvconv.py b/pvcnn_amd/modules/pvconv.py
--- a/pvcnn_amd/modules/pvconv.py
+++ b/pvcnn_amd/modules/pvconv.py
@@ -3,7 +3,8 @@
 
 from . import functional as F
 from .functional._autograd import native
-from .functional.bnact import batch_norm_act_devoxelize, batch_norm_act_se_devoxelize, fusable_tail, run_layers
+from .functional.bnact import (batch_norm_act_devoxelize, batch_norm_act_se_devoxelize, fusable_tail, point_branch_deferred,
+                               run_layers)
 from .functional.conv3d import conv_nsplit, voxel_conv3d
 from .se import SE3d
 from .shared_mlp import SharedMLP
@@ -60,11 +61,12 @@
             bn, slope, se = tail
             ntail = 2 if se is None else 3
             grid, stats_part = run_layers(self.voxel_layers, grid, stop=len(self.voxel_layers) - ntail, tail_stats=True)
-            per_point = self.point_features(features)
             if se is None:
+                per_point, point_bn = point_branch_deferred(self.point_features, features)
                 fused = batch_norm_act_devoxelize(grid, grid_coords, bn, slope, self.resolution, self.training, stats_part,
-                                                  addend=per_point)
+                                                  addend=per_point, addend_bn=point_bn)
             else:
+                per_point = self.point_features(features)
                 fused = batch_norm_act_se_devoxelize(grid, grid_coords, bn, slope, se, self.resolution, self.training, stats_part,
                                                      addend=per_point)
             return fused, coords
```
